# liuyuan-pal/NeRO

Hardware: NVIDIA B200
Metric: train rays/sec (128 samples/ray) (higher is better)
Workload: dtype f32 (split-bf16 x3 tensor-core MMAs, fp32 accumulate)

## Files before the change

### include/nero_b200.h

```cpp
#ifndef NERO_B200_H_
#define NERO_B200_H_
#include <stdint.h>

#ifdef __cplusplus
extern "C" {
#endif

#define NERO_ACT_NONE 0
#define NERO_ACT_SOFTPLUS100 1
#define NERO_ACT_RELU 2
#define NERO_ACT_SIGMOID 3
#define NERO_ACT_EXPCLAMP 4
#define NERO_EPI_BIAS_ACT 0
#define NERO_EPI_MUL_DACT 1
#define NERO_EPI_TANGENT 2

int nero_version(void);

int nero_prep_weight(const float* v, const float* g, int K, int row0, int nrows, const int* kmap, float in_scale,
                     void* img_f, int rows_pad_f, void* img_t, int rows_pad_t, int t_c0, int t_ncols, float* w_eff, int ld_weff,
                     void* stream);

int nero_linear(const float* A, int lda, int k_valid, const void* wimg, int n_pad, int k_chunks, const float* bias, int n_bias,
                float* out, int ldo, int ncol_out, float oscale, int mode, int act, float act_param,
                const float* H, int ldh, float hscale, int dact, const float* V, int ldv, float* out2, int ldo2,
                const float* addend, int ldadd, int ncol_main, float* tail, int ldt,
                const int* m_ptr, int m_cap, void* stream);

typedef struct nero_chain_layer {
  const void* wimg; const float* bias;
  float* save; const float* H; const float* addend; const float* V; float* out2; float* tail;
  int n_pad, k_chunks, n_bias, ncol_out, ncol_main, kind, act;
  int ld_save, ldh, ldadd, ldv, ldo2, ldt;
  float oscale, hscale, act_param;
  int write_a, a_blocks;
  const float* csrc; int ld_csrc;
  int pad_;
} nero_chain_layer;
typedef struct nero_chain_params {
  const float* A0; int lda0; int k_valid0;
  int n_layers; const int* m_ptr; int m_cap;
  nero_chain_layer L[10];
} nero_chain_params;
int nero_chain(const void* chain_params_host, void* stream);
int nero_row_axpy(const float* a, int lda, const float* X, int ldx, float* Y, int ldy, int ncol, const int* m_ptr, int m_cap, void* stream);

int nero_wgrad(const float* dY, int ldy, int n_valid, const float* X, int ldx, int k_valid,
               const float* dY2, int ldy2, const float* X2, int ldx2,
               float* partial, int ld_partial, int rows_partial, float* bias_partial,
               int n_rows_pad, int k_pad, int P, const int* m_ptr, int m_cap, void* stream);
int nero_wgrad_finish(const float* partial, int P, int rows_partial, int ld_partial, const float* bias_partial, int K,
                      int row0, int nrows, const int* kmap, float in_scale, const float* v, const float* g,
                      float* grad_w, float* grad_g, float* grad_b, const float* extra_row, float extra_scale, void* stream);
int nero_colsum(const float* X, int ldx, int ncol, const float* w, int ldw, const int* m_ptr, int m_cap, float* out,
                void* stream);

int nero_pe(const float* x, int d, int ldx, int M, int L, float scale, float* out, int ldo, void* stream);
int nero_ide(const float* dirs, int ldd, const float* kappa_inv, int kstride, float kappa_scalar, int M, float* out, int ldo, void* stream);

int nero_set_ide_table(const float* mat17x36_host);

int nero_ray_prepare(const float* rays_o, const float* rays_d, const float* z_vals, int R, int S, int* cnt_in, int* cnt_out,
                     int* off_in, int* off_out, int* n_in, int* n_out, void* stream);
int nero_ray_fill(const float* rays_o, const float* rays_d, const float* z_vals, int R, int S, const int* off_in, const int* off_out,
                  int* slot, float* pts, int* ray_in, float* X0, int ld_x0, float* Y8, int ld_y8, float* H4, int ld_h4,
                  float* XN, int ld_xn, float* H5, int ld_h5, float* FV, int ld_fv, float* dist_out, int* ray_out, void* stream);

int nero_reg_prepare(const float* rays_o, const float* rays_d, const float* z_vals, int R, int S, float radius, int* cnt, int* cnt_dummy,
                     int* off, int* off_dummy, int* n, int* n_dummy, void* stream);
int nero_reg_fill(const float* rays_o, const float* rays_d, const float* z_vals, int R, int S, float radius, const int* off, float* pts,
                  float* X0, int ldx, float* H4, int ldh, void* stream);

int nero_points_fill(const float* pts3, int N, float* pts, int* ray_in, float* X0, int ldx, float* Y8, int ldy, float* H4, int ldh, void* stream);

int nero_dact_times_row(const float* H, int ldh, const float* row, float* V, int ldv, int ncol, const int* m_ptr, int m_cap, void* stream);
int nero_pe_grad(const float* X0, int ldx, const float* U0, int ldu, const float* US, int lds, float* G, const int* m_ptr, int m_cap, void* stream);
int nero_pe_tangent(const float* X0, int ldx, const float* DG, float* UB0, int ld0, float* UB4, int ld4, const int* m_ptr, int m_cap, void* stream);

int nero_sdf_alpha_fwd(const float* Y8, int ldy, int sdf_col, const float* G, const float* pts, const int* ray_in, const float* rays_d,
                       const float* variance, const float* car, float* alpha, float* gerr, const int* m_ptr, int m_cap, void* stream);
int nero_sdf_alpha_bwd(const float* Y8, int ldy, int sdf_col, const float* G, const float* pts, const int* ray_in, const float* rays_d,
                       const float* variance, const float* car, const float* dalpha, const float* dgerr, float* dY8, int lddy, float* DG,
                       float* d_inv_s, const int* m_ptr, int m_cap, void* stream);

int nero_nerf_post_fwd(const float* dens, int ldd, const float* rgb, int ldr, const float* dist, float* alpha, float* color,
                       const int* m_ptr, int m_cap, void* stream);
int nero_nerf_post_bwd(const float* dens, int ldd, const float* rgb, int ldr, const float* dist, const float* dalpha, const float* dcolor,
                       float* ddens, int lddd, float* drgb, int lddr, const int* m_ptr, int m_cap, void* stream);

int nero_composite_fwd(const int* slot, int R, int S, const float* a_in, const float* c_in, const float* a_out, const float* c_out,
                       float* rgb, float* weights, void* stream);
int nero_composite_bwd(const int* slot, int R, int S, const float* a_in, const float* c_in, const float* a_out, const float* c_out,
                       const float* drgb, float* da_in, float* dc_in, float* da_out, float* dc_out, void* stream);

int nero_shade_prep_fwd(const float* G, const float* pts, const int* ray_in, const float* rays_d, const float* OUTS, float* E, int lde,
                        float* GEO, const float* human_poses, float* EH, int ldeh, int pos_freq, const int* m_ptr, int m_cap, int sphere, void* stream);
int nero_shade_prep_bwd(const float* G, const float* pts, const int* ray_in, const float* rays_d, const float* OUTS, const float* GEO,
                        const float* dE_dir, int ld_dir, const float* dE_inn, int ld_inn, const float* dE_dif, int ld_dif,
                        const float* dEH, int ld_eh, const float* human_poses, const float* dNoV, float* DOUTS, float* DG,
                        const int* m_ptr, int m_cap, int sphere, void* stream);
int nero_shade_combine_fwd(const float* OUTS, const float* GEO, const float* lut, float exp_max, int human, float* color,
                           float* occ_prob, float* refl, const int* m_ptr, int m_cap, void* stream);
int nero_shade_combine_bwd(const float* OUTS, const float* GEO, const float* lut, float exp_max, int human, const float* dcolor,
                           const float* docc, float* DOUTS, float* dNoV, const int* m_ptr, int m_cap, void* stream);

int nero_sample_init(const float* rays_o, const float* rays_d, const float* near, const float* far, int R, int n, int nb,
                     const float* lin_inner, const float* bg_base, const float* bg_lower, const float* bg_upper,
                     const float* rand_inner, const float* rand_bg, float* z, int ldz, float* z_bg, int ldzb,
                     float* X0, int ldx, float* HC, int ldh, void* stream);
int nero_upsample(const float* rays_o, const float* rays_d, int R, const float* z, int ldz, const float* sdf, int lds, int n, int n_new,
                  const float* variance, float inv_s_cap, int clip, int surface_variant, float* new_z, int ldn,
                  float* X0, int ldx, float* HC, int ldh, float* wsum, void* stream);
int nero_merge_samples(const float* z, int ldz, const float* sdf, int lds, int n, const float* nz, int ldn, const float* nsdf, int ldns,
                       int m, float* oz, int ldoz, float* osdf, int ldos, int R, void* stream);
int nero_occ_init(const float* pts, const float* refl, const int* sel, const int* p_ptr, int p_cap, int sn0, const float* lin,
                  float* o_out, float* d_out, float* z, int ldz, float* X0, int ldx, float* HC, int ldh, void* stream);
int nero_occ_select(const float* pts, const float* Y8, int ldy, int sdf_col, const float* G, const int* ray_in, const float* rays_d,
                    float sdf_thresh, const int* m_ptr, int m_cap, int* sel, int* count, void* stream);
int nero_occ_loss(const float* occ_prob, const float* gt, const int* sel, const int* p_ptr, int p_cap, float* loss_sum, float* docc_sign,
                  void* stream);

int nero_bvh_build_host(const float* verts, int V, const int* tris, int T, void* nodes_out, float* tri_out, int* tri_id_out, int* n_nodes);
int nero_bvh_trace(const void* nodes, const float* tris, int n_rays, const float* org, int ldo, const float* dir, int ldd,
                   float* pos_depth, float* nrm_hit, float miss_depth, int flip, void* stream);

typedef struct nero_mc_params {
  const float* pts; const float* normals; const float* view; const float* rough;
  const float* poses;
  const float* rand_d; const float* rand_s;
  const float* tab_d; const float* tab_s;
  int P, Sd, Ss;
  int ggx_smith, sphere_dir, human;
  float* org; float* dir;
  const float* pos_depth; const float* nrm_hit;
  int* slot;
  int* blk_cnt; int* blk_off; int* counts;
  float* EO; int ldeo; float* EH; int ldeh; float* hhit; float* EI; int ldei;
  const float* OUT_O; const float* OUT_H; const float* OUT_I;
  float exp_max_o, exp_max_i;
  float* LD; float* LS; float* LSF;
  const float* dLD; const float* dLS; const float* dLSF;
  float* DPRE_O; float* DPRE_H; float* DPRE_I;
  float* dA;
  const float* dEO; const float* dEH; const float* dEI;
  float* dA2;
} nero_mc_params;
int nero_mc_sample(const nero_mc_params* q, void* stream);
int nero_mc_classify(const nero_mc_params* q, void* stream);
int nero_mc_fill(const nero_mc_params* q, void* stream);
int nero_mc_combine_fwd(const nero_mc_params* q, void* stream);
int nero_mc_combine_bwd(const nero_mc_params* q, void* stream);
int nero_mc_dir_bwd(const nero_mc_params* q, void* stream);
int nero_mat_prep(const float* pts, int M, float* X, int ldx, float* CAT, int ldc, float* Y, int ldy, void* stream);

int nero_abi_sizeof(int which);

int nero_prep_weight_batch(const void* jobs_dev, int n_jobs, int max_rows, void* stream);

int nero_wgrad_finish_batch(const void* jobs_dev, int n_jobs, int max_rows, int max_k, void* stream);

int nero_adam_flat(float* p, const float* g, float* m, float* v, long long n, float lr_over_bc1, float b1, float b2, float eps,
                   float inv_sqrt_bc2, float weight_decay, void* stream);

#ifdef __cplusplus
}
#endif
#endif
```

### nero_b200/csrc/api.cu

```cuda
#include "common.cuh"
#include "../../include/nero_b200.h"

namespace nero {
struct LinearParams {
  const float* A; int lda; int k_valid;
  const uint8_t* wimg; int n_pad; int k_chunks;
  const float* bias; int n_bias;
  float* out; int ldo; int ncol_out; float oscale;
  int mode; int act; float act_param;
  const float* H; int ldh; float hscale; int dact;
  const float* V; int ldv;
  float* out2; int ldo2;
  const float* addend; int ldadd;
  int ncol_main; float* tail; int ldt;
  const int* m_ptr; int m_cap;
};
struct WgradParams {
  const float* dY; int ldy; const float* X; int ldx;
  const float* dY2; int ldy2; const float* X2; int ldx2;
  int n0; int n_valid; int k0; int k_valid;
  float* partial; int ld_partial; int rows_partial;
  float* bias_partial;
  const int* m_ptr; int m_cap;
};
int linear_dispatch(const LinearParams& p, cudaStream_t stream);
int wgrad_dispatch(WgradParams p, int n_rows_pad, int k_pad, int P, cudaStream_t stream);
int prep_weight(const float* v, const float* g, int K, int row0, int nrows, const int* kmap, float in_scale,
                uint8_t* img_f, int rows_pad_f, uint8_t* img_t, int rows_pad_t, int t_c0, int t_ncols, float* w_eff, int ld_weff,
                cudaStream_t stream);
int wgrad_finish(const float* partial, int P, int rows_partial, int ld_partial, const float* bias_partial, int K,
                 int row0, int nrows, const int* kmap, float in_scale, const float* v, const float* g, float* grad_w,
                 float* grad_g, float* grad_b, const float* extra_row, float extra_scale, cudaStream_t stream);
int colsum(const float* X, int ldx, int ncol, const float* w, int ldw, const int* m_ptr, int m_cap, float* out, cudaStream_t stream);
int wgrad_finish_batch(const void* jobs_dev, int n_jobs, int max_rows, int max_k, cudaStream_t stream);
int prep_weight_batch(const void* jobs_dev, int n_jobs, int max_rows, cudaStream_t stream);
int adam_flat(float* p, const float* g, float* m, float* v, long n, float lr_over_bc1, float b1, float b2, float eps, float inv_sqrt_bc2,
              float wd, cudaStream_t st);
}


namespace nero {
struct IdeTable;
int set_ide_table(const float* mat17x36_host);
int ray_prepare(const float* rays_o, const float* rays_d, const float* z_vals, int R, int S, int* cnt_in, int* cnt_out,
                int* off_in, int* off_out, int* n_in, int* n_out, cudaStream_t st);
struct FillParams {
  const float* rays_o; const float* rays_d; const float* z_vals; int R; int S;
  const int* off_in; const int* off_out;
  int* slot; float* pts; int* ray_in;
  float* X0; int ld_x0; float* Y8; int ld_y8; float* H4; int ld_h4;
  float* XN; int ld_xn; float* H5; int ld_h5; float* FV; int ld_fv;
  float* dist_out; int* ray_out;
};
int ray_fill(const FillParams& q, cudaStream_t st);
int dact_times_row(const float* H, int ldh, const float* row, float* V, int ldv, int ncol, const int* m_ptr, int m_cap, cudaStream_t st);
int pe_grad(const float* X0, int ldx, const float* U0, int ldu, const float* US, int lds, float* G, const int* m_ptr, int m_cap, cudaStream_t st);
int pe_tangent_launch(const float* X0, int ldx, const float* DG, float* UB0, int ld0, float* UB4, int ld4, const int* m_ptr, int m_cap, cudaStream_t st);
int sdf_alpha_forward(const float* Y8, int ldy, int sdf_col, const float* G, const float* pts, const int* ray_in, const float* rays_d,
                      const float* variance, const float* car, float* alpha, float* gerr, const int* m_ptr, int m_cap, cudaStream_t st);
int sdf_alpha_backward(const float* Y8, int ldy, int sdf_col, const float* G, const float* pts, const int* ray_in, const float* rays_d,
                       const float* variance, const float* car, const float* dalpha, const float* dgerr, float* dY8, int lddy, float* DG,
                       float* d_inv_s, const int* m_ptr, int m_cap, cudaStream_t st);
int nerf_post_forward(const float* dens, int ldd, const float* rgb, int ldr, const float* dist, float* alpha, float* color, const int* m_ptr, int m_cap, cudaStream_t st);
int nerf_post_backward(const float* dens, int ldd, const float* rgb, int ldr, const float* dist, const float* dalpha, const float* dcolor,
                       float* ddens, int lddd, float* drgb, int lddr, const int* m_ptr, int m_cap, cudaStream_t st);
int composite_forward(const int* slot, int R, int S, const float* a_in, const float* c_in, const float* a_out, const float* c_out,
                      float* rgb, float* weights, cudaStream_t st);
int composite_backward(const int* slot, int R, int S, const float* a_in, const float* c_in, const float* a_out, const float* c_out,
                       const float* drgb, float* da_in, float* dc_in, float* da_out, float* dc_out, cudaStream_t st);
struct ShadePrepParams {
  const float* G; const float* pts; const int* ray_in; const float* rays_d;
  const float* OUTS; float* E; int lde; float* GEO;
  const float* human_poses; float* EH; int ldeh;
  int pos_freq;
  const int* m_ptr; int m_cap;
  int sphere;
};
struct ShadePrepBwdParams {
  const float* G; const float* pts; const int* ray_in; const float* rays_d; const float* OUTS; const float* GEO;
  const float* dE_dir; int ld_dir; const float* dE_inn; int ld_inn; const float* dE_dif; int ld_dif;
  const float* dEH; int ld_eh; const float* human_poses; const float* dNoV;
  float* DOUTS; float* DG;
  const int* m_ptr; int m_cap;
  int sphere;
};
struct ShadeCombineParams {
  const float* OUTS; const float* GEO; const float* lut; float exp_max; int human;
  float* color; float* occ_prob; float* refl;
  const float* dcolor; const float* docc; float* DOUTS; float* dNoV;
  const int* m_ptr; int m_cap;
};
int shade_prep_forward(const ShadePrepParams& q, cudaStream_t st);
int shade_prep_backward(const ShadePrepBwdParams& q, cudaStream_t st);
int shade_combine_forward(const ShadeCombineParams& q, cudaStream_t st);
int shade_combine_backward(const ShadeCombineParams& q, cudaStream_t st);
struct SampleInitParams {
  const float* rays_o; const float* rays_d; const float* near; const float* far; int R;
  int n; int nb;
  const float* lin_inner; const float* bg_base; const float* bg_lower; const float* bg_upper;
  const float* rand_inner; const float* rand_bg;
  float* z; int ldz; float* z_bg; int ldzb;
  float* X0; int ldx; float* HC; int ldh;
};
struct UpsampleParams {
  const float* rays_o; const float* rays_d; int R;
  const float* z; int ldz; const float* sdf; int lds; int n;
  int n_new;
  const float* variance; float inv_s_cap; int clip;
  int surface_variant;
  float* new_z; int ldn;
  float* X0; int ldx; float* HC; int ldh;
  float* wsum;
  const float* origins;
};
int sample_init(const SampleInitParams& q, cudaStream_t st);
int upsample(const UpsampleParams& q, cudaStream_t st);
int merge_samples(const float* z, int ldz, const float* sdf, int lds, int n, const float* nz, int ldn, const float* nsdf, int ldns,
                  int m, float* oz, int ldoz, float* osdf, int ldos, int R, cudaStream_t st);
int occ_init(const float* pts, const float* refl, const int* sel, const int* p_ptr, int p_cap, int sn0, const float* lin,
             float* o_out, float* d_out, float* z, int ldz, float* X0, int ldx, float* HC, int ldh, cudaStream_t st);
int occ_select(const float* pts, const float* Y8, int ldy, int sdf_col, const float* G, const int* ray_in, const float* rays_d,
               float sdf_thresh, const int* m_ptr, int m_cap, int* sel, int* count, cudaStream_t st);
int row_axpy(const float* a, int lda, const float* X, int ldx, float* Y, int ldy, int ncol, const int* m_ptr, int m_cap, cudaStream_t st);
int reg_prepare(const float* rays_o, const float* rays_d, const float* z_vals, int R, int S, float radius, int* cnt, int* cnt_dummy,
                int* off, int* off_dummy, int* n, int* n_dummy, cudaStream_t st);
int reg_fill(const float* rays_o, const float* rays_d, const float* z_vals, int R, int S, float radius, const int* off, float* pts,
             float* X0, int ldx, float* H4, int ldh, cudaStream_t st);
int points_fill(const float* pts3, int N, float* pts, int* ray_in, float* X0, int ldx, float* Y8, int ldy, float* H4, int ldh, cudaStream_t st);
struct ChainParams;
int set_ide_table_mc(const float* mat17x36_host);
int bvh_build_host(const float* verts, int V, const int* tris, int T, void* nodes_out, float* tri_out, int* tri_id_out, int* n_nodes);
struct BvhNode;
struct TraceParams {
  const BvhNode* nodes; const float4* tris; int n_rays;
  const float* org; int ldo; const float* dir; int ldd;
  float4* pos_depth; float4* nrm_hit;
  float miss_depth; int flip;
};
int bvh_trace(const TraceParams& q, cudaStream_t st);
int mc_sample(const ::nero_mc_params& q, cudaStream_t st);
int mc_classify(const ::nero_mc_params& q, cudaStream_t st);
int mc_fill(const ::nero_mc_params& q, cudaStream_t st);
int mc_combine_fwd(const ::nero_mc_params& q, cudaStream_t st);
int mc_combine_bwd(const ::nero_mc_params& q, cudaStream_t st);
int mc_dir_bwd(const ::nero_mc_params& q, cudaStream_t st);
int mat_prep(const float* pts, int M, float* X, int ldx, float* CAT, int ldc, float* Y, int ldy, cudaStream_t st);
int chain_dispatch(const ChainParams& p, cudaStream_t stream);
int pe_standalone(const float* x, int d, int ldx, int M, int L, float scale, float* out, int ldo, cudaStream_t st);
int ide_standalone(const float* dirs, int ldd, const float* kappa, int kstride, float kappa_scalar, int M, float* out, int ldo, cudaStream_t st);
int occ_loss(const float* occ_prob, const float* gt, const int* sel, const int* p_ptr, int p_cap, float* loss_sum, float* docc_sign,
             cudaStream_t st);
}

using namespace nero;

extern "C" {

int nero_version(void) { return 100; }

int nero_prep_weight(const float* v, const float* g, int K, int row0, int nrows, const int* kmap, float in_scale,
                     void* img_f, int rows_pad_f, void* img_t, int rows_pad_t, int t_c0, int t_ncols, float* w_eff, int ld_weff,
                     void* stream) {
  return prep_weight(v, g, K, row0, nrows, kmap, in_scale, (uint8_t*)img_f, rows_pad_f, (uint8_t*)img_t, rows_pad_t, t_c0, t_ncols,
                     w_eff, ld_weff, (cudaStream_t)stream);
}

int nero_linear(const float* A, int lda, int k_valid, const void* wimg, int n_pad, int k_chunks, const float* bias, int n_bias,
                float* out, int ldo, int ncol_out, float oscale, int mode, int act, float act_param,
                const float* H, int ldh, float hscale, int dact, const float* V, int ldv, float* out2, int ldo2,
                const float* addend, int ldadd, int ncol_main, float* tail, int ldt,
                const int* m_ptr, int m_cap, void* stream) {
  LinearParams p{A, lda, k_valid, (const uint8_t*)wimg, n_pad, k_chunks, bias, n_bias, out, ldo, ncol_out, oscale, mode, act, act_param,
                 H, ldh, hscale, dact, V, ldv, out2, ldo2, addend, ldadd, ncol_main, tail, ldt, m_ptr, m_cap};
  if (!A || !wimg || !out || ncol_out > n_pad) return NERO_ERR_ARG;
  return linear_dispatch(p, (cudaStream_t)stream);
}

int nero_wgrad(const float* dY, int ldy, int n_valid, const float* X, int ldx, int k_valid,
               const float* dY2, int ldy2, const float* X2, int ldx2,
               float* partial, int ld_partial, int rows_partial, float* bias_partial,
               int n_rows_pad, int k_pad, int P, const int* m_ptr, int m_cap, void* stream) {
  WgradParams p{dY, ldy, X, ldx, dY2, ldy2, X2, ldx2, 0, n_valid, 0, k_valid, partial, ld_partial, rows_partial, bias_partial,
                m_ptr, m_cap};
  if (!dY || !X || !partial || (dY2 && !X2)) return NERO_ERR_ARG;
  return wgrad_dispatch(p, n_rows_pad, k_pad, P, (cudaStream_t)stream);
}

int nero_wgrad_finish(const float* partial, int P, int rows_partial, int ld_partial, const float* bias_partial, int K,
                      int row0, int nrows, const int* kmap, float in_scale, const float* v, const float* g,
                      float* grad_w, float* grad_g, float* grad_b, const float* extra_row, float extra_scale, void* stream) {
  return wgrad_finish(partial, P, rows_partial, ld_partial, bias_partial, K, row0, nrows, kmap, in_scale, v, g, grad_w, grad_g,
                      grad_b, extra_row, extra_scale, (cudaStream_t)stream);
}

int nero_colsum(const float* X, int ldx, int ncol, const float* w, int ldw, const int* m_ptr, int m_cap, float* out,
                void* stream) {
  return colsum(X, ldx, ncol, w, ldw, m_ptr, m_cap, out, (cudaStream_t)stream);
}

int nero_set_ide_table(const float* mat17x36_host) {
  const int rc = set_ide_table(mat17x36_host);
  return rc != NERO_OK ? rc : set_ide_table_mc(mat17x36_host);
}
int nero_bvh_build_host(const float* verts, int V, const int* tris, int T, void* nodes_out, float* tri_out, int* tri_id_out, int* n_nodes) {
  if (!verts || !tris || !nodes_out || !tri_out || !tri_id_out || !n_nodes) return NERO_ERR_ARG;
  return bvh_build_host(verts, V, tris, T, nodes_out, tri_out, tri_id_out, n_nodes);
}
int nero_bvh_trace(const void* nodes, const float* tris, int n_rays, const float* org, int ldo, const float* dir, int ldd,
                   float* pos_depth, float* nrm_hit, float miss_depth, int flip, void* stream) {
  if (!nodes || !tris || (n_rays > 0 && (!org || !dir || !pos_depth || !nrm_hit))) return NERO_ERR_ARG;
  TraceParams q{reinterpret_cast<const BvhNode*>(nodes), reinterpret_cast<const float4*>(tris), n_rays, org, ldo, dir, ldd,
                reinterpret_cast<float4*>(pos_depth), reinterpret_cast<float4*>(nrm_hit), miss_depth, flip};
  return bvh_trace(q, (cudaStream_t)stream);
}
int nero_mc_sample(const nero_mc_params* q, void* stream) { return q ? mc_sample(*q, (cudaStream_t)stream) : NERO_ERR_ARG; }
int nero_mc_classify(const nero_mc_params* q, void* stream) { return q ? mc_classify(*q, (cudaStream_t)stream) : NERO_ERR_ARG; }
int nero_mc_fill(const nero_mc_params* q, void* stream) { return q ? mc_fill(*q, (cudaStream_t)stream) : NERO_ERR_ARG; }
int nero_mc_combine_fwd(const nero_mc_params* q, void* stream) { return q ? mc_combine_fwd(*q, (cudaStream_t)stream) : NERO_ERR_ARG; }
int nero_mc_combine_bwd(const nero_mc_params* q, void* stream) { return q ? mc_combine_bwd(*q, (cudaStream_t)stream) : NERO_ERR_ARG; }
int nero_mc_dir_bwd(const nero_mc_params* q, void* stream) { return q ? mc_dir_bwd(*q, (cudaStream_t)stream) : NERO_ERR_ARG; }
int nero_abi_sizeof(int which) {
  switch (which) {
    case 0: return int(sizeof(nero_chain_layer));
    case 1: return int(sizeof(nero_chain_params));
    case 2: return int(sizeof(nero_mc_params));
    case 3: return 104;
    case 4: return 88;
    default: return -1;
  }
}
int nero_prep_weight_batch(const void* jobs_dev, int n_jobs, int max_rows, void* stream) {
  return prep_weight_batch(jobs_dev, n_jobs, max_rows, (cudaStream_t)stream);
}
int nero_wgrad_finish_batch(const void* jobs_dev, int n_jobs, int max_rows, int max_k, void* stream) {
  return wgrad_finish_batch(jobs_dev, n_jobs, max_rows, max_k, (cudaStream_t)stream);
}
int nero_adam_flat(float* p, const float* g, float* m, float* v, long long n, float lr_over_bc1, float b1, float b2, float eps,
                   float inv_sqrt_bc2, float weight_decay, void* stream) {
  if (!p || !g || !m || !v) return NERO_ERR_ARG;
  return adam_flat(p, g, m, v, long(n), lr_over_bc1, b1, b2, eps, inv_sqrt_bc2, weight_decay, (cudaStream_t)stream);
}
int nero_mat_prep(const float* pts, int M, float* X, int ldx, float* CAT, int ldc, float* Y, int ldy, void* stream) {
  return mat_prep(pts, M, X, ldx, CAT, ldc, Y, ldy, (cudaStream_t)stream);
}

int nero_pe(const float* x, int d, int ldx, int M, int L, float scale, float* out, int ldo, void* stream) {
  return pe_standalone(x, d, ldx, M, L, scale, out, ldo, (cudaStream_t)stream);
}
int nero_ide(const float* dirs, int ldd, const float* kappa_inv, int kstride, float kappa_scalar, int M, float* out, int ldo, void* stream) {
  return ide_standalone(dirs, ldd, kappa_inv, kstride, kappa_scalar, M, out, ldo, (cudaStream_t)stream);
}

int nero_chain(const void* chain_params_host, void* stream) {
  if (!chain_params_host) return NERO_ERR_ARG;
  return chain_dispatch(*reinterpret_cast<const ChainParams*>(chain_params_host), (cudaStream_t)stream);
}
int nero_reg_prepare(const float* rays_o, const float* rays_d, const float* z_vals, int R, int S, float radius, int* cnt, int* cnt_dummy,
                     int* off, int* off_dummy, int* n, int* n_dummy, void* stream) {
  return reg_prepare(rays_o, rays_d, z_vals, R, S, radius, cnt, cnt_dummy, off, off_dummy, n, n_dummy, (cudaStream_t)stream);
}
int nero_reg_fill(const float* rays_o, const float* rays_d, const float* z_vals, int R, int S, float radius, const int* off, float* pts,
                  float* X0, int ldx, float* H4, int ldh, void* stream) {
  return reg_fill(rays_o, rays_d, z_vals, R, S, radius, off, pts, X0, ldx, H4, ldh, (cudaStream_t)stream);
}
int nero_points_fill(const float* pts3, int N, float* pts, int* ray_in, float* X0, int ldx, float* Y8, int ldy, float* H4, int ldh, void* stream) {
  return points_fill(pts3, N, pts, ray_in, X0, ldx, Y8, ldy, H4, ldh, (cudaStream_t)stream);
}
int nero_row_axpy(const float* a, int lda, const float* X, int ldx, float* Y, int ldy, int ncol, const int* m_ptr, int m_cap, void* stream) {
  return row_axpy(a, lda, X, ldx, Y, ldy, ncol, m_ptr, m_cap, (cudaStream_t)stream);
}

int nero_ray_prepare(const float* rays_o, const float* rays_d, const float* z_vals, int R, int S, int* cnt_in, int* cnt_out,
                     int* off_in, int* off_out, int* n_in, int* n_out, void* stream) {
  return ray_prepare(rays_o, rays_d, z_vals, R, S, cnt_in, cnt_out, off_in, off_out, n_in, n_out, (cudaStream_t)stream);
}
int nero_ray_fill(const float* rays_o, const float* rays_d, const float* z_vals, int R, int S, const int* off_in, const int* off_out,
                  int* slot, float* pts, int* ray_in, float* X0, int ld_x0, float* Y8, int ld_y8, float* H4, int ld_h4,
                  float* XN, int ld_xn, float* H5, int ld_h5, float* FV, int ld_fv, float* dist_out, int* ray_out, void* stream) {
  FillParams q{rays_o, rays_d, z_vals, R, S, off_in, off_out, slot, pts, ray_in, X0, ld_x0, Y8, ld_y8, H4, ld_h4, XN, ld_xn, H5, ld_h5,
               FV, ld_fv, dist_out, ray_out};
  return ray_fill(q, (cudaStream_t)stream);
}
int nero_dact_times_row(const float* H, int ldh, const float* row, float* V, int ldv, int ncol, const int* m_ptr, int m_cap, void* stream) {
  return dact_times_row(H, ldh, row, V, ldv, ncol, m_ptr, m_cap, (cudaStream_t)stream);
}
int nero_pe_grad(const float* X0, int ldx, const float* U0, int ldu, const float* US, int lds, float* G, const int* m_ptr, int m_cap, void* stream) {
  return pe_grad(X0, ldx, U0, ldu, US, lds, G, m_ptr, m_cap, (cudaStream_t)stream);
}
int nero_pe_tangent(const float* X0, int ldx, const float* DG, float* UB0, int ld0, float* UB4, int ld4, const int* m_ptr, int m_cap, void* stream) {
  return pe_tangent_launch(X0, ldx, DG, UB0, ld0, UB4, ld4, m_ptr, m_cap, (cudaStream_t)stream);
}
int nero_sdf_alpha_fwd(const float* Y8, int ldy, int sdf_col, const float* G, const float* pts, const int* ray_in, const float* rays_d,
                       const float* variance, const float* car, float* alpha, float* gerr, const int* m_ptr, int m_cap, void* stream) {
  return sdf_alpha_forward(Y8, ldy, sdf_col, G, pts, ray_in, rays_d, variance, car, alpha, gerr, m_ptr, m_cap, (cudaStream_t)stream);
}
int nero_sdf_alpha_bwd(const float* Y8, int ldy, int sdf_col, const float* G, const float* pts, const int* ray_in, const float* rays_d,
                       const float* variance, const float* car, const float* dalpha, const float* dgerr, float* dY8, int lddy, float* DG,
                       float* d_inv_s, const int* m_ptr, int m_cap, void* stream) {
  return sdf_alpha_backward(Y8, ldy, sdf_col, G, pts, ray_in, rays_d, variance, car, dalpha, dgerr, dY8, lddy, DG, d_inv_s, m_ptr, m_cap,
                            (cudaStream_t)stream);
}
int nero_nerf_post_fwd(const float* dens, int ldd, const float* rgb, int ldr, const float* dist, float* alpha, float* color,
                       const int* m_ptr, int m_cap, void* stream) {
  return nerf_post_forward(dens, ldd, rgb, ldr, dist, alpha, color, m_ptr, m_cap, (cudaStream_t)stream);
}
int nero_nerf_post_bwd(const float* dens, int ldd, const float* rgb, int ldr, const float* dist, const float* dalpha, const float* dcolor,
                       float* ddens, int lddd, float* drgb, int lddr, const int* m_ptr, int m_cap, void* stream) {
  return nerf_post_backward(dens, ldd, rgb, ldr, dist, dalpha, dcolor, ddens, lddd, drgb, lddr, m_ptr, m_cap, (cudaStream_t)stream);
}
int nero_composite_fwd(const int* slot, int R, int S, const float* a_in, const float* c_in, const float* a_out, const float* c_out,
                       float* rgb, float* weights, void* stream) {
  return composite_forward(slot, R, S, a_in, c_in, a_out, c_out, rgb, weights, (cudaStream_t)stream);
}
int nero_composite_bwd(const int* slot, int R, int S, const float* a_in, const float* c_in, const float* a_out, const float* c_out,
                       const float* drgb, float* da_in, float* dc_in, float* da_out, float* dc_out, void* stream) {
  return composite_backward(slot, R, S, a_in, c_in, a_out, c_out, drgb, da_in, dc_in, da_out, dc_out, (cudaStream_t)stream);
}
int nero_shade_prep_fwd(const float* G, const float* pts, const int* ray_in, const float* rays_d, const float* OUTS, float* E, int lde,
                        float* GEO, const float* human_poses, float* EH, int ldeh, int pos_freq, const int* m_ptr, int m_cap, int sphere, void* stream) {
  ShadePrepParams q{G, pts, ray_in, rays_d, OUTS, E, lde, GEO, human_poses, EH, ldeh, pos_freq, m_ptr, m_cap, sphere};
  return shade_prep_forward(q, (cudaStream_t)stream);
}
int nero_shade_prep_bwd(const float* G, const float* pts, const int* ray_in, const float* rays_d, const float* OUTS, const float* GEO,
                        const float* dE_dir, int ld_dir, const float* dE_inn, int ld_inn, const float* dE_dif, int ld_dif,
                        const float* dEH, int ld_eh, const float* human_poses, const float* dNoV, float* DOUTS, float* DG,
                        const int* m_ptr, int m_cap, int sphere, void* stream) {
  ShadePrepBwdParams q{G, pts, ray_in, rays_d, OUTS, GEO, dE_dir, ld_dir, dE_inn, ld_inn, dE_dif, ld_dif, dEH, ld_eh, human_poses, dNoV,
                       DOUTS, DG, m_ptr, m_cap, sphere};
  return shade_prep_backward(q, (cudaStream_t)stream);
}
int nero_shade_combine_fwd(const float* OUTS, const float* GEO, const float* lut, float exp_max, int human, float* color,
                           float* occ_prob, float* refl, const int* m_ptr, int m_cap, void* stream) {
  ShadeCombineParams q{OUTS, GEO, lut, exp_max, human, color, occ_prob, refl, nullptr, nullptr, nullptr, nullptr, m_ptr, m_cap};
  return shade_combine_forward(q, (cudaStream_t)stream);
}
int nero_shade_combine_bwd(const float* OUTS, const float* GEO, const float* lut, float exp_max, int human, const float* dcolor,
                           const float* docc, float* DOUTS, float* dNoV, const int* m_ptr, int m_cap, void* stream) {
  ShadeCombineParams q{OUTS, GEO, lut, exp_max, human, nullptr, nullptr, nullptr, dcolor, docc, DOUTS, dNoV, m_ptr, m_cap};
  return shade_combine_backward(q, (cudaStream_t)stream);
}
int nero_sample_init(const float* rays_o, const float* rays_d, const float* near, const float* far, int R, int n, int nb,
                     const float* lin_inner, const float* bg_base, const float* bg_lower, const float* bg_upper,
                     const float* rand_inner, const float* rand_bg, float* z, int ldz, float* z_bg, int ldzb,
                     float* X0, int ldx, float* HC, int ldh, void* stream) {
  SampleInitParams q{rays_o, rays_d, near, far, R, n, nb, lin_inner, bg_base, bg_lower, bg_upper, rand_inner, rand_bg, z, ldz, z_bg, ldzb,
                     X0, ldx, HC, ldh};
  return sample_init(q, (cudaStream_t)stream);
}
int nero_upsample(const float* rays_o, const float* rays_d, int R, const float* z, int ldz, const float* sdf, int lds, int n, int n_new,
                  const float* variance, float inv_s_cap, int clip, int surface_variant, float* new_z, int ldn,
                  float* X0, int ldx, float* HC, int ldh, float* wsum, void* stream) {
  UpsampleParams q{rays_o, rays_d, R, z, ldz, sdf, lds, n, n_new, variance, inv_s_cap, clip, surface_variant, new_z, ldn, X0, ldx, HC, ldh,
                   wsum, nullptr};
  return upsample(q, (cudaStream_t)stream);
}
int nero_merge_samples(const float* z, int ldz, const float* sdf, int lds, int n, const float* nz, int ldn, const float* nsdf, int ldns,
                       int m, float* oz, int ldoz, float* osdf, int ldos, int R, void* stream) {
  return merge_samples(z, ldz, sdf, lds, n, nz, ldn, nsdf, ldns, m, oz, ldoz, osdf, ldos, R, (cudaStream_t)stream);
}
int nero_occ_init(const float* pts, const float* refl, const int* sel, const int* p_ptr, int p_cap, int sn0, const float* lin,
                  float* o_out, float* d_out, float* z, int ldz, float* X0, int ldx, float* HC, int ldh, void* stream) {
  return occ_init(pts, refl, sel, p_ptr, p_cap, sn0, lin, o_out, d_out, z, ldz, X0, ldx, HC, ldh, (cudaStream_t)stream);
}
int nero_occ_select(const float* pts, const float* Y8, int ldy, int sdf_col, const float* G, const int* ray_in, const float* rays_d,
                    float sdf_thresh, const int* m_ptr, int m_cap, int* sel, int* count, void* stream) {
  return occ_select(pts, Y8, ldy, sdf_col, G, ray_in, rays_d, sdf_thresh, m_ptr, m_cap, sel, count, (cudaStream_t)stream);
}
int nero_occ_loss(const float* occ_prob, const float* gt, const int* sel, const int* p_ptr, int p_cap, float* loss_sum, float* docc_sign,
                  void* stream) {
  return occ_loss(occ_prob, gt, sel, p_ptr, p_cap, loss_sum, docc_sign, (cudaStream_t)stream);
}

}
```

### nero_b200/csrc/k_umma_wgrad.cu

```cuda

#include "common.cuh"
#include "ptx.cuh"
#include "umma_common.cuh"

namespace nero {

struct WgradParams {
  const float* dY; int ldy; const float* X; int ldx;
  const float* dY2; int ldy2; const float* X2; int ldx2;
  int n0; int n_valid;
  int k0; int k_valid;
  float* partial; int ld_partial; int rows_partial;
  float* bias_partial;
  const int* m_ptr; int m_cap;
};

constexpr int WG_BM = 128, WG_BK = 64;
constexpr int kWgProdWarps = 16;
constexpr int kWgThreads = (kWgProdWarps + 1) * 32;
constexpr uint32_t kWgABytes = WG_BM * 128;

template <int NW> struct WgCfg {
  static constexpr uint32_t b_plane = NW * 128;
  static constexpr uint32_t stage_bytes = 2 * kWgABytes + 2 * b_plane;
  static constexpr int stages = (stage_bytes * 3 <= 200 * 1024) ? 3 : 2;
  static constexpr uint32_t smem_bytes = stages * stage_bytes + 1024 + 256 + 512;
};

__device__ __forceinline__ void wg_split2(float x0, float x1, uint32_t& hi, uint32_t& lo) {
  __nv_bfloat162 h = __floats2bfloat162_rn(x0, x1);
  const uint32_t hb = *reinterpret_cast<uint32_t*>(&h);
  const float h0 = __uint_as_float(hb << 16), h1 = __uint_as_float(hb & 0xffff0000u);
  __nv_bfloat162 l = __floats2bfloat162_rn(x0 - h0, x1 - h1);
  hi = hb;
  lo = *reinterpret_cast<uint32_t*>(&l);
}

template <int NOCT>
__device__ __forceinline__ void load_octets(const float* __restrict__ src, int ld, int col, bool col_ok, int s0, int M, uint32_t oct0,
                                            float (&x)[NOCT][8]) {
#pragma unroll
  for (int o = 0; o < NOCT; ++o)
#pragma unroll
    for (int i = 0; i < 8; ++i) {
      const int s = s0 + (oct0 + o) * 8 + i;
      x[o][i] = (col_ok && s < M) ? __ldg(src + size_t(s) * ld + col) : 0.0f;
    }
}
template <int NOCT>
__device__ __forceinline__ float store_octets(const float (&x)[NOCT][8], uint8_t* plane_hi, uint8_t* plane_lo, uint32_t row, uint32_t oct0) {
  float sum = 0.0f;
#pragma unroll
  for (int o = 0; o < NOCT; ++o) {
    uint32_t hw[4], lw[4];
#pragma unroll
    for (int i = 0; i < 4; ++i) {
      wg_split2(x[o][2 * i], x[o][2 * i + 1], hw[i], lw[i]);
      sum += x[o][2 * i] + x[o][2 * i + 1];
    }
    const uint32_t off = row * 128u + (((oct0 + o) ^ (row & 7u)) << 4);
    *reinterpret_cast<uint4*>(plane_hi + off) = make_uint4(hw[0], hw[1], hw[2], hw[3]);
    *reinterpret_cast<uint4*>(plane_lo + off) = make_uint4(lw[0], lw[1], lw[2], lw[3]);
  }
  return sum;
}

__device__ __forceinline__ void red_add_v4(float* addr, float a, float b, float c, float d) {
  asm volatile("red.global.add.v4.f32 [%0], {%1, %2, %3, %4};" ::"l"(addr), "f"(a), "f"(b), "f"(c), "f"(d) : "memory");
}

template <int NW>
__device__ __forceinline__ void wg_epilogue(const WgradParams& p, uint32_t tmem_base, int pw, int lane, int n0, bool any, const float* s_bias) {
  const int orow = n0 + pw * 32 + lane;
  float* prow = p.partial + size_t(orow) * p.ld_partial + p.k0;
  const uint32_t taddr = tmem_base + (uint32_t(pw * 32) << 16);
  if (any) {
#pragma unroll 1
    for (int cc = 0; cc < (NW + 31) / 32; ++cc) {
      float v[32];
      tmem_ld32(taddr + cc * 32, v);
      tmem_ld_wait();
      if (orow < p.rows_partial) {
#pragma unroll
        for (int j = 0; j < 32; j += 4)
          if (cc * 32 + j < NW) red_add_v4(prow + cc * 32 + j, v[j], v[j + 1], v[j + 2], v[j + 3]);
      }
    }
    if (p.bias_partial && p.k0 == 0 && orow < p.rows_partial) atomicAdd(&p.bias_partial[orow], s_bias[pw * 32 + lane]);
  }
}

template <int NW>
__global__ void __launch_bounds__(kWgThreads, 1) umma_wgrad_kernel(const WgradParams p) {
  using Cfg = WgCfg<NW>;
  constexpr int STAGES = Cfg::stages;
  extern __shared__ uint8_t smem_raw[];
  uint8_t* smem = reinterpret_cast<uint8_t*>((reinterpret_cast<uintptr_t>(smem_raw) + 1023) & ~uintptr_t(1023));
  uint64_t* bars = reinterpret_cast<uint64_t*>(smem + STAGES * Cfg::stage_bytes);
  uint64_t* full = bars;
  uint64_t* empty = bars + STAGES;
  uint64_t* tfull = bars + 2 * STAGES;
  uint32_t* tmem_slot = reinterpret_cast<uint32_t*>(bars + 2 * STAGES + 1);
  float* s_bias = reinterpret_cast<float*>(smem + STAGES * Cfg::stage_bytes + 256);

  const int warp = threadIdx.x >> 5, lane = threadIdx.x & 31;
  int M = p.m_ptr ? *p.m_ptr : p.m_cap;
  if (M > p.m_cap) M = p.m_cap;
  const int P = gridDim.x;
  const int n0 = p.n0 + int(blockIdx.y) * WG_BM;
  const int total_chunks = (M + WG_BK - 1) / WG_BK;
  const int cpp = (total_chunks + P - 1) / P;
  const int c_begin = min(total_chunks, int(blockIdx.x) * cpp), c_end = min(total_chunks, c_begin + cpp);
  const int npairs = p.dY2 ? 2 : 1;
  const int nc1 = c_end - c_begin;
  const int nchunks = nc1 * npairs;

  if (threadIdx.x == 0) {
    for (int s = 0; s < STAGES; ++s) { mbar_init(&full[s], kWgProdWarps); mbar_init(&empty[s], 1); }
    mbar_init(tfull, 1);
    fence_mbar_init();
  }
  if (threadIdx.x < 128) s_bias[threadIdx.x] = 0.0f;
  if (warp == kWgProdWarps) tmem_alloc<256>(tmem_slot);
  tcgen05_fence_before();
  __syncthreads();
  tcgen05_fence_after();
  const uint32_t tmem_base = *tmem_slot;

  if (warp < kWgProdWarps) {
    const bool is_a = warp < 8;
    const int pw = warp & 3;
    const int oh = (warp >> 2) & 1;
    float bias_acc = 0.0f;
    for (int g = 0; g < nchunks; ++g) {
      const int s = g % STAGES;
      const int pair = g / nc1;
      const int chunk = c_begin + g % nc1;
      const int s0 = chunk * WG_BK;
      uint8_t* st = smem + s * Cfg::stage_bytes;
      if (is_a) {
        const float* src = pair ? p.dY2 : p.dY;
        const int ld = pair ? p.ldy2 : p.ldy;
        const uint32_t row = pw * 32 + lane;
        const int col = n0 + int(row);
        const bool ok = col < p.n_valid;
        float x[4][8];
        load_octets<4>(src, ld, col, ok, s0, M, oh * 4, x);
        mbar_wait(&empty[s], ((g / STAGES) & 1) ^ 1);
        const float sacc = store_octets<4>(x, st, st + kWgABytes, row, oh * 4);
        if (pair == 0) bias_acc += sacc;
      } else {
        const float* src = pair ? p.X2 : p.X;
        const int ld = pair ? p.ldx2 : p.ldx;
        uint8_t* bh = st + 2 * kWgABytes;
        constexpr int NJ = (NW + 127) / 128;
        float x[NJ][4][8];
#pragma unroll
        for (int j = 0; j < NJ; ++j) {
          const uint32_t row = j * 128 + pw * 32 + lane;
          const int col = p.k0 + int(row);
          load_octets<4>(src, ld, col, row < NW && col < p.k_valid, s0, M, oh * 4, x[j]);
        }
        mbar_wait(&empty[s], ((g / STAGES) & 1) ^ 1);
#pragma unroll
        for (int j = 0; j < NJ; ++j) {
          const uint32_t row = j * 128 + pw * 32 + lane;
          if (row < NW) store_octets<4>(x[j], bh, bh + Cfg::b_plane, row, oh * 4);
        }
      }
      fence_proxy_async_smem();
      __syncwarp();
      if (lane == 0) mbar_arrive(&full[s]);
    }
    if (is_a) atomicAdd(&s_bias[pw * 32 + lane], bias_acc);
    asm volatile("bar.sync 1, %0;" ::"n"(kWgProdWarps * 32));
    if (warp < 4) {
      mbar_wait(tfull, 0);
      tcgen05_fence_after();
      wg_epilogue<NW>(p, tmem_base, pw, lane, n0, nchunks > 0, s_bias);
    }
  } else {
    constexpr uint32_t idesc = make_idesc_bf16(WG_BM, NW);
    for (int g = 0; g < nchunks; ++g) {
      const int s = g % STAGES;
      mbar_wait(&full[s], (g / STAGES) & 1);
      tcgen05_fence_after();
      if (elect_one()) {
        const uint32_t a_hi = smem_u32(smem + s * Cfg::stage_bytes);
        const uint32_t a_lo = a_hi + kWgABytes;
        const uint32_t b_hi = a_hi + 2 * kWgABytes;
        const uint32_t b_lo = b_hi + Cfg::b_plane;
#pragma unroll
        for (int k = 0; k < WG_BK / 16; ++k) {
          const uint64_t dah = make_desc_k_sw128(a_hi + k * 32), dal = make_desc_k_sw128(a_lo + k * 32);
          const uint64_t dbh = make_desc_k_sw128(b_hi + k * 32), dbl = make_desc_k_sw128(b_lo + k * 32);
          umma_bf16(tmem_base, dal, dbh, idesc, (g | k) != 0);
          umma_bf16(tmem_base, dah, dbl, idesc, 1);
          umma_bf16(tmem_base, dah, dbh, idesc, 1);
        }
        umma_commit(&empty[s]);
        if (g == nchunks - 1) umma_commit(tfull);
      }
      __syncwarp();
    }
    if (nchunks == 0 && elect_one()) mbar_arrive(tfull);
    __syncwarp();
  }
  tcgen05_fence_before();
  __syncthreads();
  if (warp == kWgProdWarps) tmem_dealloc<256>(tmem_base);
}


constexpr int MN_BK = 32, kMnGroupWarps = kWgProdWarps / 2;
constexpr uint32_t kMnSbo = 1024, kMnLbo = (MN_BK / 8) * 1024;
template <int NW> struct WgMnCfg {
  static constexpr uint32_t a_plane = WG_BM * MN_BK * 2, b_plane = NW * MN_BK * 2;
  static constexpr uint32_t stage_bytes = 2 * a_plane + 2 * b_plane;
  static constexpr int stages = 4;
  static constexpr uint32_t smem_bytes = stages * stage_bytes + 1024 + 256 + 512;
};

__device__ __forceinline__ uint32_t mn_chunk_offset(uint32_t chunk, uint32_t s) {
  const uint32_t r = s & 7u;
  return (chunk >> 3) * kMnLbo + (s >> 3) * kMnSbo + r * 128u + (((chunk & 7u) ^ r) << 4);
}

template <int NW>
__device__ __forceinline__ void wg_epilogue_rows(const WgradParams& p, uint32_t tmem_base, float* tile, int warp, int lane, int n0,
                                                 const float* s_bias) {
  constexpr int LD = NW + 4;
  constexpr int SLICE = NW / 4;
  const int quarter = warp & 3, slice = warp >> 2;
  {
    const int row = quarter * 32 + lane;
    const uint32_t taddr = tmem_base + (uint32_t(quarter * 32) << 16) + uint32_t(slice * SLICE);
    float* dst = tile + row * LD + slice * SLICE;
#pragma unroll
    for (int c = 0; c < SLICE; c += 16) {
      float v[16];
      tmem_ld16(taddr + c, v);
      tmem_ld_wait();
#pragma unroll
      for (int j = 0; j < 16; j += 4) *reinterpret_cast<float4*>(dst + c + j) = make_float4(v[j], v[j + 1], v[j + 2], v[j + 3]);
    }
  }
  asm volatile("bar.sync 1, %0;" ::"n"(kWgProdWarps * 32));
  const int r_first = (int(blockIdx.x) * 5) & 127;
  for (int i = warp; i < WG_BM; i += kWgProdWarps) {
    const int r = (i + r_first) & 127;
    const int orow = n0 + r;
    if (orow >= p.rows_partial) continue;
    float* prow = p.partial + size_t(orow) * p.ld_partial + p.k0;
#pragma unroll
    for (int c = lane * 4; c < NW; c += 128) {
      const float4 v = *reinterpret_cast<const float4*>(tile + r * LD + c);
      red_add_v4(prow + c, v.x, v.y, v.z, v.w);
    }
    if (lane == 0 && p.bias_partial && p.k0 == 0) atomicAdd(&p.bias_partial[orow], s_bias[r]);
  }
}

template <int NW>
__global__ void __launch_bounds__(kWgThreads, 1) umma_wgrad_mn_kernel(const WgradParams p) {
  using Cfg = WgMnCfg<NW>;
  constexpr int STAGES = Cfg::stages;
  constexpr int CB = NW / 8;
  constexpr int SPW = 32 / CB;
  constexpr int ATASKS = MN_BK / 2;
  constexpr int TASKS = ATASKS + MN_BK / SPW;
  constexpr int TPW = TASKS / kMnGroupWarps;
  static_assert(TASKS % kMnGroupWarps == 0 && TPW >= 2 && STAGES % 2 == 0, "task split");
  extern __shared__ uint8_t smem_raw[];
  uint8_t* smem = reinterpret_cast<uint8_t*>((reinterpret_cast<uintptr_t>(smem_raw) + 1023) & ~uintptr_t(1023));
  uint64_t* bars = reinterpret_cast<uint64_t*>(smem + STAGES * Cfg::stage_bytes);
  uint64_t* full = bars;
  uint64_t* empty = bars + STAGES;
  uint64_t* tfull = bars + 2 * STAGES;
  uint32_t* tmem_slot = reinterpret_cast<uint32_t*>(bars + 2 * STAGES + 1);
  float* s_bias = reinterpret_cast<float*>(smem + STAGES * Cfg::stage_bytes + 256);

  const int warp = threadIdx.x >> 5, lane = threadIdx.x & 31;
  int M = p.m_ptr ? *p.m_ptr : p.m_cap;
  if (M > p.m_cap) M = p.m_cap;
  const int P = gridDim.x;
  const int n0 = p.n0 + int(blockIdx.y) * WG_BM;
  const int total_chunks = (M + MN_BK - 1) / MN_BK;
  const int cpp = (total_chunks + P - 1) / P;
  const int c_begin = min(total_chunks, int(blockIdx.x) * cpp), c_end = min(total_chunks, c_begin + cpp);
  const int npairs = p.dY2 ? 2 : 1;
  const int nc1 = c_end - c_begin;
  const int nchunks = nc1 * npairs;

  if (threadIdx.x == 0) {
    for (int s = 0; s < STAGES; ++s) { mbar_init(&full[s], kMnGroupWarps); mbar_init(&empty[s], 1); }
    mbar_init(tfull, 1);
    fence_mbar_init();
  }
  if (threadIdx.x < 128) s_bias[threadIdx.x] = 0.0f;
  if (warp == kWgProdWarps) tmem_alloc<256>(tmem_slot);
  tcgen05_fence_before();
  __syncthreads();
  tcgen05_fence_after();
  const uint32_t tmem_base = *tmem_slot;

  if (warp < kWgProdWarps) {
    float bsum[8] = {0.f, 0.f, 0.f, 0.f, 0.f, 0.f, 0.f, 0.f};
    const uint32_t a_chunk = lane & 15, a_sub = lane >> 4;
    const uint32_t b_chunk = lane % CB, b_sub = lane / CB;
    const int a_col = n0 + int(a_chunk) * 8, b_col = p.k0 + int(b_chunk) * 8;
    const int group = warp / kMnGroupWarps, wi = warp % kMnGroupWarps;
    for (int g = group; g < nchunks; g += 2) {
      const int s = g % STAGES;
      const int pair = g / nc1;
      const int chunk = c_begin + g % nc1;
      const int s0 = chunk * MN_BK;
      uint8_t* st = smem + s * Cfg::stage_bytes;
      const float* srcA = pair ? p.dY2 : p.dY;
      const int ldA = pair ? p.ldy2 : p.ldy;
      const float* srcB = pair ? p.X2 : p.X;
      const int ldB = pair ? p.ldx2 : p.ldx;
      float4 v[TPW][2];
#pragma unroll
      for (int i = 0; i < TPW; ++i) {
        const int t = wi + kMnGroupWarps * i;
        const bool isA = t < ATASKS;
        const int sl = isA ? 2 * t + int(a_sub) : (t - ATASKS) * SPW + int(b_sub);
        const int srow = s0 + sl;
        const int col = isA ? a_col : b_col;
        const int lim = isA ? p.n_valid : p.k_valid;
        const float* rp = (isA ? srcA : srcB) + size_t(srow) * (isA ? ldA : ldB) + col;
        const bool rok = srow < M;
        v[i][0] = (rok && col < lim) ? __ldg(reinterpret_cast<const float4*>(rp)) : make_float4(0.f, 0.f, 0.f, 0.f);
        v[i][1] = (rok && col + 4 < lim) ? __ldg(reinterpret_cast<const float4*>(rp + 4)) : make_float4(0.f, 0.f, 0.f, 0.f);
      }
      mbar_wait(&empty[s], ((g / STAGES) & 1) ^ 1);
#pragma unroll
      for (int i = 0; i < TPW; ++i) {
        const int t = wi + kMnGroupWarps * i;
        const bool isA = t < ATASKS;
        const int sl = isA ? 2 * t + int(a_sub) : (t - ATASKS) * SPW + int(b_sub);
        const int col = isA ? a_col : b_col;
        const int lim = isA ? p.n_valid : p.k_valid;
        float x[8] = {v[i][0].x, v[i][0].y, v[i][0].z, v[i][0].w, v[i][1].x, v[i][1].y, v[i][1].z, v[i][1].w};
#pragma unroll
        for (int j = 0; j < 8; ++j) if (col + j >= lim) x[j] = 0.f;
        uint32_t hw[4], lw[4];
#pragma unroll
        for (int j = 0; j < 4; ++j) wg_split2(x[2 * j], x[2 * j + 1], hw[j], lw[j]);
        uint8_t* hi = isA ? st : st + 2 * Cfg::a_plane;
        uint8_t* lo = isA ? st + Cfg::a_plane : st + 2 * Cfg::a_plane + Cfg::b_plane;
        const uint32_t off = mn_chunk_offset(isA ? a_chunk : b_chunk, uint32_t(sl));
        *reinterpret_cast<uint4*>(hi + off) = make_uint4(hw[0], hw[1], hw[2], hw[3]);
        *reinterpret_cast<uint4*>(lo + off) = make_uint4(lw[0], lw[1], lw[2], lw[3]);
        if (isA && pair == 0) {
#pragma unroll
          for (int j = 0; j < 8; ++j) bsum[j] += x[j];
        }
      }
      fence_proxy_async_smem();
      __syncwarp();
      if (lane == 0) mbar_arrive(&full[s]);
    }
#pragma unroll
    for (int j = 0; j < 8; ++j) {
      bsum[j] += __shfl_xor_sync(0xffffffffu, bsum[j], 16);
      if (lane < 16) atomicAdd(&s_bias[a_chunk * 8 + j], bsum[j]);
    }
    asm volatile("bar.sync 1, %0;" ::"n"(kWgProdWarps * 32));
    mbar_wait(tfull, 0);
    tcgen05_fence_after();
    if (nchunks > 0) wg_epilogue_rows<NW>(p, tmem_base, reinterpret_cast<float*>(smem), warp, lane, n0, s_bias);
  } else {
    constexpr uint32_t idesc = make_idesc_bf16_mn(WG_BM, NW);
    for (int g = 0; g < nchunks; ++g) {
      const int s = g % STAGES;
      mbar_wait(&full[s], (g / STAGES) & 1);
      tcgen05_fence_after();
      if (elect_one()) {
        const uint32_t a_hi = smem_u32(smem + s * Cfg::stage_bytes);
        const uint32_t a_lo = a_hi + Cfg::a_plane;
        const uint32_t b_hi = a_hi + 2 * Cfg::a_plane;
        const uint32_t b_lo = b_hi + Cfg::b_plane;
#pragma unroll
        for (int k = 0; k < MN_BK / 16; ++k) {
          const uint32_t ko = k * 2 * kMnSbo;
          const uint64_t dah = make_desc_mn_sw128(a_hi + ko, kMnLbo, kMnSbo), dal = make_desc_mn_sw128(a_lo + ko, kMnLbo, kMnSbo);
          const uint64_t dbh = make_desc_mn_sw128(b_hi + ko, kMnLbo, kMnSbo), dbl = make_desc_mn_sw128(b_lo + ko, kMnLbo, kMnSbo);
          umma_bf16(tmem_base, dal, dbh, idesc, (g | k) != 0);
          umma_bf16(tmem_base, dah, dbl, idesc, 1);
          umma_bf16(tmem_base, dah, dbh, idesc, 1);
        }
        umma_commit(&empty[s]);
        if (g == nchunks - 1) umma_commit(tfull);
      }
      __syncwarp();
    }
    if (nchunks == 0 && elect_one()) mbar_arrive(tfull);
    __syncwarp();
  }
  tcgen05_fence_before();
  __syncthreads();
  if (warp == kWgProdWarps) tmem_dealloc<256>(tmem_base);
}

template <int NW>
static int launch_wgrad_mn(const WgradParams& p, int P, int n_tiles, cudaStream_t stream) {
  using Cfg = WgMnCfg<NW>;
  static bool attr_set = false;
  if (!attr_set) {
    if (cudaFuncSetAttribute(umma_wgrad_mn_kernel<NW>, cudaFuncAttributeMaxDynamicSharedMemorySize, Cfg::smem_bytes) != cudaSuccess)
      return NERO_ERR_CUDA;
    attr_set = true;
  }
  umma_wgrad_mn_kernel<NW><<<dim3(P, n_tiles), kWgThreads, Cfg::smem_bytes, stream>>>(p);
  NERO_LAUNCH_CHECK();
  return NERO_OK;
}

template <int NW>
static int launch_wgrad(const WgradParams& p, int P, int n_tiles, cudaStream_t stream) {
  using Cfg = WgCfg<NW>;
  static bool attr_set = false;
  if (!attr_set) {
    if (cudaFuncSetAttribute(umma_wgrad_kernel<NW>, cudaFuncAttributeMaxDynamicSharedMemorySize, Cfg::smem_bytes) != cudaSuccess)
      return NERO_ERR_CUDA;
    attr_set = true;
  }
  umma_wgrad_kernel<NW><<<dim3(P, n_tiles), kWgThreads, Cfg::smem_bytes, stream>>>(p);
  NERO_LAUNCH_CHECK();
  return NERO_OK;
}

int wgrad_dispatch(WgradParams p, int n_rows_pad, int k_pad, int P, cudaStream_t stream) {
  if ((p.ld_partial & 3) || k_pad % 64 || n_rows_pad % 16 || P <= 0) return NERO_ERR_ARG;
  const int n_tiles = (n_rows_pad + 127) / 128;
  p.n0 = 0;
  auto al = [](const float* q, int ld) { return q == nullptr || ((reinterpret_cast<uintptr_t>(q) & 15) == 0 && (ld & 3) == 0); };
  const bool mn = al(p.dY, p.ldy) && al(p.X, p.ldx) && al(p.dY2, p.ldy2) && al(p.X2, p.ldx2);
  int k0 = 0;
  while (k0 < k_pad) {
    const int rem = k_pad - k0;
    p.k0 = k0;
    int rc;
    if (rem >= 256) { rc = mn ? launch_wgrad_mn<256>(p, P, n_tiles, stream) : launch_wgrad<256>(p, P, n_tiles, stream); k0 += 256; }
    else if (rem >= 128) { rc = mn ? launch_wgrad_mn<128>(p, P, n_tiles, stream) : launch_wgrad<128>(p, P, n_tiles, stream); k0 += 128; }
    else { rc = mn ? launch_wgrad_mn<64>(p, P, n_tiles, stream) : launch_wgrad<64>(p, P, n_tiles, stream); k0 += 64; }
    if (rc != NERO_OK) return rc;
  }
  return NERO_OK;
}

}
```

### nero_b200/engine.py

```python
import math

import numpy as np
import torch

from . import ops
from .ops import Mat, K, linear, wgrad, chain, chain_layer as CL, ACT_NONE, ACT_SOFTPLUS100, ACT_RELU, ACT_SIGMOID, ACT_EXPCLAMP, EPI_MUL_DACT, EPI_TANGENT
from .ops import EK_BIAS_SOFTPLUS, EK_BIAS_RELU, EK_BIAS_GENERIC, EK_DACT_SOFTPLUS, EK_DACT_RELU, EK_DACT_NONE, EK_TANGENT

USE_CHAIN = True

INV_SQRT2 = 0.7071067811865476
SQRT2 = 1.4142135623730951
E_PE6R, E_PE8X, E_IDER, E_IDEN, E_LD = 0, 40, 92, 164, 240
O_MET, O_ROUGH, O_ALB, O_LD, O_LDIR, O_LI, O_IW, O_HUM, O_LDIM = 0, 4, 8, 12, 16, 20, 24, 28, 32
Y8_LD, Y8_X, Y8_SDF = 320, 256, 260


def ide_coefficient_table():
    def gbc(a, k):
        return np.prod(a - np.arange(k)) / math.factorial(k)

    def alc(l, m, k):
        return ((-1) ** m * 2 ** l * math.factorial(l) / math.factorial(k) / math.factorial(l - k - m) *
                gbc(0.5 * (l + k + m - 1.0), l))

    def shc(l, m, k):
        return np.sqrt((2.0 * l + 1.0) * math.factorial(l - m) / (4.0 * np.pi * math.factorial(l + m))) * alc(l, m, k)

    cols = [(m, 2 ** e) for e in range(5) for m in range(2 ** e + 1)]
    mat = np.zeros((17, len(cols)))
    for i, (m, l) in enumerate(cols):
        for k in range(l - m + 1):
            mat[k, i] = shc(l, m, k)
    return np.ascontiguousarray(mat.astype(np.float32))


_ide_uploaded = False


def upload_ide_table():
    global _ide_uploaded
    if not _ide_uploaded:
        mat = ide_coefficient_table()
        rc = ops.lib.nero_set_ide_table(mat.ctypes.data_as(ops.ctypes.c_void_p))
        ops._check(rc, 'nero_set_ide_table')
        _ide_uploaded = True


def _linear_to_srgb_torch(x):
    eps = torch.finfo(torch.float32).eps
    return torch.where(x <= 0.0031308, 323 / 25 * x, (211 * torch.clamp(x, min=eps) ** (5 / 12) - 11) / 200)


def _fg_lookup_torch(lut, uv):
    H, W = lut.shape[0], lut.shape[1]
    fx, fy = uv[:, 0] * W - 0.5, uv[:, 1] * H - 0.5
    x0f, y0f = torch.floor(fx), torch.floor(fy)
    tx, ty = (fx - x0f)[:, None], (fy - y0f)[:, None]
    x0, x1 = x0f.long().clamp(0, W - 1), (x0f.long() + 1).clamp(0, W - 1)
    y0, y1 = y0f.long().clamp(0, H - 1), (y0f.long() + 1).clamp(0, H - 1)
    a = lut[y0, x0] * (1 - tx) + lut[y0, x1] * tx
    b = lut[y1, x0] * (1 - tx) + lut[y1, x1] * tx
    return a * (1 - ty) + b * ty


class Grads:

    def __init__(self, params):
        self.params = [p for p in params]
        self.total = sum(p.numel() for p in self.params)
        self.flat = None
        self.views = None

    def ensure(self, strict=False):
        if self.flat is None:
            self.flat = torch.zeros(self.total, dtype=torch.float32, device=self.params[0].device)
            off = 0
            self.views = []
            for p in self.params:
                n = p.numel()
                self.views.append(self.flat[off:off + n].view_as(p))
                off += n
        missing = [i for i, p in enumerate(self.params) if p.grad is None]
        if len(missing) == len(self.params):
            self.flat.zero_()
        else:
            for i in missing:
                self.views[i].zero_()
        for i in missing:
            self.params[i].grad = self.views[i]
        if strict:
            for p, v in zip(self.params, self.views):
                if p.grad.data_ptr() != v.data_ptr():
                    v.copy_(p.grad)
                    p.grad = v
        return self.flat


class Predictor:

    def __init__(self, pp, dev, n_out, act, act_param=0.0, kmap=None, k_layout=None, t_cols=None):
        ls = pp.layers()
        self.n_out, self.act, self.act_param = n_out, act, act_param
        self.layers = [ops.PreparedLayer(ls[0].weight_v, ls[0].weight_g, ls[0].bias, dev, kmap=kmap, k_layout=k_layout, t_cols=t_cols)]
        for l in ls[1:]:
            self.layers.append(ops.PreparedLayer(l.weight_v, l.weight_g, l.bias, dev, t_cols=(0, 256)))
        self.pl = ls

    def prep(self):
        for l in self.layers:
            l.prep()

    def forward(self, A, acts, out, m_ptr, m_cap):
        L = self.layers
        if USE_CHAIN:
            tail = [CL(L[1], EK_BIAS_RELU, 256, save=Mat(acts[1])), CL(L[2], EK_BIAS_RELU, 256, save=Mat(acts[2])),
                    CL(L[3], EK_BIAS_GENERIC, self.n_out, save=out, act=self.act, act_param=self.act_param)]
            if L[0].k_chunks <= 4:
                chain(A, L[0].k_valid, [CL(L[0], EK_BIAS_RELU, 256, save=Mat(acts[0]))] + tail, m_ptr, m_cap)
            else:
                linear(A, L[0], Mat(acts[0]), 256, act=ACT_RELU, m_ptr=m_ptr, m_cap=m_cap)
                chain(Mat(acts[0]), 256, tail, m_ptr, m_cap)
            return
        linear(A, L[0], Mat(acts[0]), 256, act=ACT_RELU, m_ptr=m_ptr, m_cap=m_cap)
        linear(Mat(acts[0]), L[1], Mat(acts[1]), 256, act=ACT_RELU, m_ptr=m_ptr, m_cap=m_cap)
        linear(Mat(acts[1]), L[2], Mat(acts[2]), 256, act=ACT_RELU, m_ptr=m_ptr, m_cap=m_cap)
        linear(Mat(acts[2]), L[3], out, self.n_out, act=self.act, act_param=self.act_param, m_ptr=m_ptr, m_cap=m_cap)

    def backward(self, ws, dpre, A, acts, dHa, dHb, m_ptr, m_cap, dX=None, dx_ncol=0, dx_addend=None, dHc=None):
        L, P = self.layers, self.pl
        g = lambda i: (P[i].weight_v.grad, P[i].weight_g.grad, P[i].bias.grad)
        kw = dict(m_ptr=m_ptr, m_cap=m_cap)
        if USE_CHAIN and dHc is not None:
            ls = [CL(L[3], EK_DACT_RELU, 256, transposed=True, H=Mat(acts[2]), save=Mat(dHa)),
                  CL(L[2], EK_DACT_RELU, 256, transposed=True, H=Mat(acts[1]), save=Mat(dHb)),
                  CL(L[1], EK_DACT_RELU, 256, transposed=True, H=Mat(acts[0]), save=Mat(dHc))]
            if dX is not None:
                ls.append(CL(L[0], EK_DACT_NONE, dx_ncol, transposed=True, addend=dx_addend, save=dX))
            chain(dpre, self.n_out, ls, m_ptr, m_cap)
            wgrad(ws, dpre, self.n_out, Mat(acts[2]), 256, L[3], *g(3), **kw)
            wgrad(ws, Mat(dHa), 256, Mat(acts[1]), 256, L[2], *g(2), **kw)
            wgrad(ws, Mat(dHb), 256, Mat(acts[0]), 256, L[1], *g(1), **kw)
            wgrad(ws, Mat(dHc), 256, A, L[0].k_valid, L[0], *g(0), **kw)
            return
        linear(dpre, L[3], Mat(dHa), 256, transposed=True, mode=EPI_MUL_DACT, H=Mat(acts[2]), dact=ACT_RELU, **kw)
        wgrad(ws, dpre, self.n_out, Mat(acts[2]), 256, L[3], *g(3), **kw)
        linear(Mat(dHa), L[2], Mat(dHb), 256, transposed=True, mode=EPI_MUL_DACT, H=Mat(acts[1]), dact=ACT_RELU, **kw)
        wgrad(ws, Mat(dHa), 256, Mat(acts[1]), 256, L[2], *g(2), **kw)
        linear(Mat(dHb), L[1], Mat(dHa), 256, transposed=True, mode=EPI_MUL_DACT, H=Mat(acts[0]), dact=ACT_RELU, **kw)
        wgrad(ws, Mat(dHb), 256, Mat(acts[0]), 256, L[1], *g(1), **kw)
        if dX is not None:
            linear(Mat(dHa), L[0], dX, dx_ncol, transposed=True, mode=EPI_MUL_DACT, addend=dx_addend, **kw)
        wgrad(ws, Mat(dHa), 256, A, L[0].k_valid, L[0], *g(0), **kw)


class SdfNet:

    def __init__(self, sp, dev):
        self.sp = sp
        ls = sp.layers()
        assert len(ls) == 9 and sp.multires == 6 and tuple(sp.skip_in) == (4,), 'kernels are laid out for the default SDF network'
        self.L = []
        for k, l in enumerate(ls[:8]):
            tc = (0, 39) if k == 0 else (0, 256)
            self.L.append(ops.PreparedLayer(l.weight_v, l.weight_g, l.bias, dev, t_cols=tc))
        l8 = ls[8]
        self.L8f = ops.PreparedLayer(l8.weight_v, l8.weight_g, l8.bias, dev, row0=1, nrows=256, t_cols=(0, 256))
        self.L8s = ops.PreparedLayer(l8.weight_v, l8.weight_g, l8.bias, dev, row0=0, nrows=1, t_cols=(0, 256))
        self.nout = [256, 256, 256, 217, 256, 256, 256, 256]
        self.tmp_row = torch.zeros(256, device=dev)
        self.tmp_b = torch.zeros(4, device=dev)

    def prep(self):
        for l in self.L + [self.L8f, self.L8s]:
            l.prep()

    def hidden_forward(self, X0, Hs, H4buf, m_ptr, m_cap, save=True, heads=None):
        kw = dict(act=ACT_SOFTPLUS100, m_ptr=m_ptr, m_cap=m_cap)
        if USE_CHAIN:
            sv = (lambda t: Mat(t)) if save else (lambda t: None)
            ls = [CL(self.L[0], EK_BIAS_SOFTPLUS, 256, save=sv(Hs[0])), CL(self.L[1], EK_BIAS_SOFTPLUS, 256, save=sv(Hs[1])),
                  CL(self.L[2], EK_BIAS_SOFTPLUS, 256, save=sv(Hs[2])),
                  CL(self.L[3], EK_BIAS_SOFTPLUS, 217, oscale=INV_SQRT2, save=sv(H4buf), csrc=Mat(H4buf)),
                  CL(self.L[4], EK_BIAS_SOFTPLUS, 256, save=sv(Hs[4])), CL(self.L[5], EK_BIAS_SOFTPLUS, 256, save=sv(Hs[5])),
                  CL(self.L[6], EK_BIAS_SOFTPLUS, 256, save=sv(Hs[6])), CL(self.L[7], EK_BIAS_SOFTPLUS, 256, save=sv(Hs[7]))]
            chain(Mat(X0), self.L[0].k_valid, ls + (heads or []), m_ptr, m_cap, tag='sdf_forward' if save else 'sdf_forward_nosave')
            return
        linear(Mat(X0), self.L[0], Mat(Hs[0]), 256, **kw)
        linear(Mat(Hs[0]), self.L[1], Mat(Hs[1]), 256, **kw)
        linear(Mat(Hs[1]), self.L[2], Mat(Hs[2]), 256, **kw)
        linear(Mat(Hs[2]), self.L[3], Mat(H4buf), 217, oscale=INV_SQRT2, **kw)
        linear(Mat(H4buf), self.L[4], Mat(Hs[4]), 256, **kw)
        linear(Mat(Hs[4]), self.L[5], Mat(Hs[5]), 256, **kw)
        linear(Mat(Hs[5]), self.L[6], Mat(Hs[6]), 256, **kw)
        linear(Mat(Hs[6]), self.L[7], Mat(Hs[7]), 256, **kw)

    def sdf_only(self, X0, SA, SB, SC, out, m_ptr, m_cap):
        Hs = [SA, SB, SA, SC, SA, SB, SA, SB]
        if USE_CHAIN:
            self.hidden_forward(X0, Hs, SC, m_ptr, m_cap, save=False,
                                heads=[CL(self.L8s, EK_BIAS_GENERIC, 1, save=Mat(out), write_a=False)])
            return
        self.hidden_forward(X0, Hs, SC, m_ptr, m_cap)
        linear(Mat(SB), self.L8s, Mat(out), 1, m_ptr=m_ptr, m_cap=m_cap)

    def forward_with_gradient(self, w, m_ptr, m_cap):
        H = w['H']
        Hs = [H[1], H[2], H[3], H[4], H[5], H[6], H[7], H[8]]
        kw = dict(m_ptr=m_ptr, m_cap=m_cap)
        V = w['V']
        if USE_CHAIN:
            self.hidden_forward(w['X0'], Hs, H[4], m_ptr, m_cap,
                                heads=[CL(self.L8f, EK_BIAS_GENERIC, 256, save=Mat(w['Y8']), write_a=False),
                                       CL(self.L8s, EK_BIAS_GENERIC, 1, save=Mat(w['Y8'], Y8_SDF), write_a=False)])
            K('nero_dact_times_row', H[8], 256, self.L8s.w_eff, V[7], 256, 256, m_ptr, m_cap)
            ls = []
            for k in range(7, 0, -1):
                if k == 4:
                    ls.append(CL(self.L[4], EK_DACT_SOFTPLUS, 256, transposed=True, oscale=INV_SQRT2, H=Mat(H[4]), hscale=SQRT2,
                                 ncol_main=217, tail=Mat(w['USKIP']), save=Mat(V[3])))
                else:
                    ls.append(CL(self.L[k], EK_DACT_SOFTPLUS, 256, transposed=True, H=Mat(H[k]), save=Mat(V[k - 1])))
            ls.append(CL(self.L[0], EK_DACT_NONE, 39, transposed=True, save=Mat(w['U0'])))
            chain(Mat(V[7]), 256, ls, m_ptr, m_cap, tag='sdf_reverse_sweep')
            K('nero_pe_grad', w['X0'], 64, w['U0'], 64, w['USKIP'], 64, w['G'], m_ptr, m_cap)
            return
        self.hidden_forward(w['X0'], Hs, H[4], m_ptr, m_cap)
        linear(Mat(H[8]), self.L8f, Mat(w['Y8']), 256, **kw)
        linear(Mat(H[8]), self.L8s, Mat(w['Y8'], Y8_SDF), 1, **kw)
        K('nero_dact_times_row', H[8], 256, self.L8s.w_eff, V[7], 256, 256, m_ptr, m_cap)
        for k in range(7, 0, -1):
            if k == 4:
                linear(Mat(V[4]), self.L[4], Mat(V[3]), 256, transposed=True, mode=EPI_MUL_DACT, oscale=INV_SQRT2, H=Mat(H[4]),
                       hscale=SQRT2, dact=ACT_SOFTPLUS100, ncol_main=217, tail=Mat(w['USKIP']), **kw)
            else:
                linear(Mat(V[k]), self.L[k], Mat(V[k - 1]), 256, transposed=True, mode=EPI_MUL_DACT, H=Mat(H[k]),
                       dact=ACT_SOFTPLUS100, **kw)
        linear(Mat(V[0]), self.L[0], Mat(w['U0']), 39, transposed=True, mode=EPI_MUL_DACT, **kw)
        K('nero_pe_grad', w['X0'], 64, w['U0'], 64, w['USKIP'], 64, w['G'], m_ptr, m_cap)

    def backward(self, ws, w, m_ptr, m_cap, grads_of):
        H, V, UB, AB = w['H'], w['V'], w['UB'], w['ABAR']
        kw = dict(m_ptr=m_ptr, m_cap=m_cap)
        dY8 = w['dY8']
        K('nero_pe_tangent', w['X0'], 64, w['DG'], UB[0], 64, UB[4], 256, m_ptr, m_cap)
        if USE_CHAIN:
            ls = []
            for k in range(8):
                if k == 3:
                    ls.append(CL(self.L[3], EK_TANGENT, 217, use_bias=False, oscale=INV_SQRT2, H=Mat(H[4]), hscale=SQRT2, V=Mat(V[3]),
                                 out2=Mat(AB[3]), save=Mat(UB[4]), csrc=Mat(UB[4])))
                else:
                    ls.append(CL(self.L[k], EK_TANGENT, 256, use_bias=False, H=Mat(H[k + 1]), V=Mat(V[k]), out2=Mat(AB[k]), save=Mat(UB[k + 1])))
            chain(Mat(UB[0]), self.L[0].k_valid, ls, m_ptr, m_cap, tag='sdf_tangent_sweep')
            K('nero_row_axpy', Mat(dY8, Y8_SDF), Y8_LD, V[7], 256, AB[7], 256, 256, m_ptr, m_cap)
            ls = [CL(self.L8f, EK_DACT_SOFTPLUS, 256, transposed=True, H=Mat(H[8]), addend=Mat(AB[7]), save=Mat(AB[7]))]
            for k in range(7, 0, -1):
                if k == 4:
                    ls.append(CL(self.L[4], EK_DACT_SOFTPLUS, 217, transposed=True, oscale=INV_SQRT2, H=Mat(H[4]), hscale=SQRT2,
                                 addend=Mat(AB[3]), save=Mat(AB[3])))
                else:
                    ls.append(CL(self.L[k], EK_DACT_SOFTPLUS, 256, transposed=True, H=Mat(H[k]), addend=Mat(AB[k - 1]), save=Mat(AB[k - 1])))
            chain(Mat(dY8), 256, ls, m_ptr, m_cap, tag='sdf_value_backward')
        else:
            for k in range(8):
                A = Mat(UB[k])
                if k == 3:
                    linear(A, self.L[3], Mat(UB[4]), 217, use_bias=False, mode=EPI_TANGENT, oscale=INV_SQRT2, H=Mat(H[4]), hscale=SQRT2,
                           dact=ACT_SOFTPLUS100, V=Mat(V[3]), out2=Mat(AB[3]), **kw)
                else:
                    linear(A, self.L[k], Mat(UB[k + 1]), 256, use_bias=False, mode=EPI_TANGENT, H=Mat(H[k + 1]), dact=ACT_SOFTPLUS100,
                           V=Mat(V[k]), out2=Mat(AB[k]), **kw)
            linear(Mat(dY8), self.L8f, Mat(AB[7]), 256, transposed=True, mode=EPI_MUL_DACT, H=Mat(H[8]), dact=ACT_SOFTPLUS100,
                   addend=Mat(AB[7]), **kw)
            linear(Mat(dY8, Y8_SDF), self.L8s, Mat(AB[7]), 256, transposed=True, mode=EPI_MUL_DACT, H=Mat(H[8]), dact=ACT_SOFTPLUS100,
                   addend=Mat(AB[7]), **kw)
            for k in range(7, 0, -1):
                if k == 4:
                    linear(Mat(AB[4]), self.L[4], Mat(AB[3]), 217, transposed=True, mode=EPI_MUL_DACT, oscale=INV_SQRT2, H=Mat(H[4]),
                           hscale=SQRT2, dact=ACT_SOFTPLUS100, addend=Mat(AB[3]), **kw)
                else:
                    linear(Mat(AB[k]), self.L[k], Mat(AB[k - 1]), 256, transposed=True, mode=EPI_MUL_DACT, H=Mat(H[k]),
                           dact=ACT_SOFTPLUS100, addend=Mat(AB[k - 1]), **kw)
        ls = self.sp.layers()
        for k in range(8):
            Hin = Mat(w['X0']) if k == 0 else Mat(H[k])
            wgrad(ws, Mat(AB[k]), self.nout[k], Hin, self.L[k].k_valid, self.L[k], ls[k].weight_v.grad, ls[k].weight_g.grad,
                  ls[k].bias.grad, dY2=Mat(V[k]), X2=Mat(UB[k]), **kw)
        l8 = ls[8]
        wgrad(ws, Mat(dY8), 256, Mat(H[8]), 256, self.L8f, l8.weight_v.grad, l8.weight_g.grad, l8.bias.grad, **kw)
        self.tmp_row.zero_()
        self.tmp_b.zero_()
        ops.colsum(Mat(H[8]), 256, self.tmp_row, w=Mat(dY8, Y8_SDF), m_ptr=m_ptr, m_cap=m_cap)
        ops.colsum(Mat(UB[8]), 256, self.tmp_row, m_ptr=m_ptr, m_cap=m_cap)
        ops.colsum(Mat(dY8, Y8_SDF), 1, self.tmp_b, m_ptr=m_ptr, m_cap=m_cap)
        K('nero_wgrad_finish', self.tmp_row, 1, 1, 256, self.tmp_b, 256, 0, 1, None, 1.0, l8.weight_v.detach(), l8.weight_g.detach(),
          l8.weight_v.grad, l8.weight_g.grad, l8.bias.grad, None, 0.0)

    def value_forward(self, X0, H, out, m_ptr, m_cap):
        Hs = [H[1], H[2], H[3], H[4], H[5], H[6], H[7], H[8]]
        if USE_CHAIN:
            self.hidden_forward(X0, Hs, H[4], m_ptr, m_cap, heads=[CL(self.L8s, EK_BIAS_GENERIC, 1, save=Mat(out), write_a=False)])
        else:
            self.hidden_forward(X0, Hs, H[4], m_ptr, m_cap)
            linear(Mat(H[8]), self.L8s, Mat(out), 1, m_ptr=m_ptr, m_cap=m_cap)

    def value_backward(self, ws, X0, H, dsdf, AB, scratch, m_ptr, m_cap):
        kw = dict(m_ptr=m_ptr, m_cap=m_cap)
        K('nero_dact_times_row', H[8], 256, self.L8s.w_eff, scratch, 256, 256, m_ptr, m_cap)
        AB[7].zero_()
        K('nero_row_axpy', dsdf, dsdf.stride(0), scratch, 256, AB[7], 256, 256, m_ptr, m_cap)
        ls = []
        for k in range(7, 0, -1):
            if k == 4:
                ls.append(CL(self.L[4], EK_DACT_SOFTPLUS, 217, transposed=True, oscale=INV_SQRT2, H=Mat(H[4]), hscale=SQRT2, save=Mat(AB[3])))
            else:
                ls.append(CL(self.L[k], EK_DACT_SOFTPLUS, 256, transposed=True, H=Mat(H[k]), save=Mat(AB[k - 1])))
        if USE_CHAIN:
            chain(Mat(AB[7]), 256, ls, m_ptr, m_cap)
        else:
            for k in range(7, 0, -1):
                if k == 4:
                    linear(Mat(AB[4]), self.L[4], Mat(AB[3]), 217, transposed=True, mode=EPI_MUL_DACT, oscale=INV_SQRT2, H=Mat(H[4]),
                           hscale=SQRT2, dact=ACT_SOFTPLUS100, **kw)
                else:
                    linear(Mat(AB[k]), self.L[k], Mat(AB[k - 1]), 256, transposed=True, mode=EPI_MUL_DACT, H=Mat(H[k]),
                           dact=ACT_SOFTPLUS100, **kw)
        ls_ = self.sp.layers()
        for k in range(8):
            Hin = Mat(X0) if k == 0 else Mat(H[k])
            wgrad(ws, Mat(AB[k]), self.nout[k], Hin, self.L[k].k_valid, self.L[k], ls_[k].weight_v.grad, ls_[k].weight_g.grad,
                  ls_[k].bias.grad, **kw)
        l8 = ls_[8]
        self.tmp_row.zero_()
        self.tmp_b.zero_()
        ops.colsum(Mat(H[8]), 256, self.tmp_row, w=Mat(dsdf), m_ptr=m_ptr, m_cap=m_cap)
        ops.colsum(Mat(dsdf), 1, self.tmp_b, m_ptr=m_ptr, m_cap=m_cap)
        K('nero_wgrad_finish', self.tmp_row, 1, 1, 256, self.tmp_b, 256, 0, 1, None, 1.0, l8.weight_v.detach(), l8.weight_g.detach(),
          l8.weight_v.grad, l8.weight_g.grad, l8.bias.grad, None, 0.0)


class NerfNet:

    def __init__(self, npar, dev):
        self.np = npar
        pl = npar.pts_linears
        mk = lambda l, **kw: ops.PreparedLayer(l.weight, None, l.bias, dev, **kw)
        self.P = [mk(pl[0])] + [mk(pl[i], t_cols=(0, 256)) for i in range(1, 5)] + [mk(pl[5], t_cols=(84, 256))] + \
                 [mk(pl[i], t_cols=(0, 256)) for i in (6, 7)]
        self.alpha = mk(npar.alpha_linear, t_cols=(0, 256))
        self.feature = mk(npar.feature_linear, t_cols=(0, 256))
        self.views = mk(npar.views_linears[0], t_cols=(0, 256))
        self.rgb = mk(npar.rgb_linear, t_cols=(0, 128))

    def all_layers(self):
        return self.P + [self.alpha, self.feature, self.views, self.rgb]

    def prep(self):
        for l in self.all_layers():
            l.prep()

    def forward(self, w, m_ptr, m_cap):
        kw = dict(m_ptr=m_ptr, m_cap=m_cap)
        N = w['NH']
        if USE_CHAIN:
            chain(Mat(w['XN']), self.P[0].k_valid,
                  [CL(self.P[0], EK_BIAS_RELU, 256, save=Mat(N[1])), CL(self.P[1], EK_BIAS_RELU, 256, save=Mat(N[2])),
                   CL(self.P[2], EK_BIAS_RELU, 256, save=Mat(N[3])), CL(self.P[3], EK_BIAS_RELU, 256, save=Mat(N[4])),
                   CL(self.P[4], EK_BIAS_RELU, 256, save=Mat(w['H5'], 84), write_a=False)], m_ptr, m_cap, tag='nerf_fwd_a')
            linear(Mat(w['H5']), self.P[5], Mat(N[6]), 256, act=ACT_RELU, **kw)
            chain(Mat(N[6]), 256,
                  [CL(self.P[6], EK_BIAS_RELU, 256, save=Mat(N[7])), CL(self.P[7], EK_BIAS_RELU, 256, save=Mat(N[8])),
                   CL(self.alpha, EK_BIAS_GENERIC, 1, save=Mat(w['DENS']), write_a=False),
                   CL(self.feature, EK_BIAS_GENERIC, 256, save=Mat(w['FV']), write_a=False)], m_ptr, m_cap, tag='nerf_fwd_b')
            linear(Mat(w['FV']), self.views, Mat(w['HV']), 128, act=ACT_RELU, **kw)
            linear(Mat(w['HV']), self.rgb, Mat(w['RGBRAW']), 3, **kw)
            return
        linear(Mat(w['XN']), self.P[0], Mat(N[1]), 256, act=ACT_RELU, **kw)
        linear(Mat(N[1]), self.P[1], Mat(N[2]), 256, act=ACT_RELU, **kw)
        linear(Mat(N[2]), self.P[2], Mat(N[3]), 256, act=ACT_RELU, **kw)
        linear(Mat(N[3]), self.P[3], Mat(N[4]), 256, act=ACT_RELU, **kw)
        linear(Mat(N[4]), self.P[4], Mat(w['H5'], 84), 256, act=ACT_RELU, **kw)
        linear(Mat(w['H5']), self.P[5], Mat(N[6]), 256, act=ACT_RELU, **kw)
        linear(Mat(N[6]), self.P[6], Mat(N[7]), 256, act=ACT_RELU, **kw)
        linear(Mat(N[7]), self.P[7], Mat(N[8]), 256, act=ACT_RELU, **kw)
        linear(Mat(N[8]), self.alpha, Mat(w['DENS']), 1, **kw)
        linear(Mat(N[8]), self.feature, Mat(w['FV']), 256, **kw)
        linear(Mat(w['FV']), self.views, Mat(w['HV']), 128, act=ACT_RELU, **kw)
        linear(Mat(w['HV']), self.rgb, Mat(w['RGBRAW']), 3, **kw)

    def backward(self, ws, w, m_ptr, m_cap):
        kw = dict(m_ptr=m_ptr, m_cap=m_cap)
        N, dA, dB = w['NH'], w['dNa'], w['dNb']
        n = self.np
        gp = lambda l: (l.weight.grad, None, l.bias.grad)
        R = dict(transposed=True, mode=EPI_MUL_DACT, dact=ACT_RELU)
        linear(Mat(w['dRGBRAW']), self.rgb, Mat(w['dHV']), 128, H=Mat(w['HV']), **R, **kw)
        wgrad(ws, Mat(w['dRGBRAW']), 3, Mat(w['HV']), 128, self.rgb, *gp(n.rgb_linear), **kw)
        linear(Mat(w['dHV']), self.views, Mat(w['dFV']), 256, transposed=True, mode=EPI_MUL_DACT, **kw)
        wgrad(ws, Mat(w['dHV']), 128, Mat(w['FV']), self.views.k_valid, self.views, *gp(n.views_linears[0]), **kw)
        linear(Mat(w['dFV']), self.feature, Mat(dA), 256, H=Mat(N[8]), **R, **kw)
        linear(Mat(w['dDENS']), self.alpha, Mat(dA), 256, H=Mat(N[8]), addend=Mat(dA), **R, **kw)
        wgrad(ws, Mat(w['dFV']), 256, Mat(N[8]), 256, self.feature, *gp(n.feature_linear), **kw)
        wgrad(ws, Mat(w['dDENS']), 1, Mat(N[8]), 256, self.alpha, *gp(n.alpha_linear), **kw)
        pl = n.pts_linears
        if USE_CHAIN:
            G = w['dNG']
            chain(Mat(dA), 256,
                  [CL(self.P[7], EK_DACT_RELU, 256, transposed=True, H=Mat(N[7]), save=Mat(G[6])),
                   CL(self.P[6], EK_DACT_RELU, 256, transposed=True, H=Mat(N[6]), save=Mat(G[5])),
                   CL(self.P[5], EK_DACT_RELU, 256, transposed=True, H=Mat(w['H5'], 84), save=Mat(G[4])),
                   CL(self.P[4], EK_DACT_RELU, 256, transposed=True, H=Mat(N[4]), save=Mat(G[3])),
                   CL(self.P[3], EK_DACT_RELU, 256, transposed=True, H=Mat(N[3]), save=Mat(G[2])),
                   CL(self.P[2], EK_DACT_RELU, 256, transposed=True, H=Mat(N[2]), save=Mat(G[1])),
                   CL(self.P[1], EK_DACT_RELU, 256, transposed=True, H=Mat(N[1]), save=Mat(G[0]))], m_ptr, m_cap, tag='nerf_bwd')
            wgrad(ws, Mat(dA), 256, Mat(N[7]), 256, self.P[7], *gp(pl[7]), **kw)
            wgrad(ws, Mat(G[6]), 256, Mat(N[6]), 256, self.P[6], *gp(pl[6]), **kw)
            wgrad(ws, Mat(G[5]), 256, Mat(w['H5']), self.P[5].k_valid, self.P[5], *gp(pl[5]), **kw)
            wgrad(ws, Mat(G[4]), 256, Mat(N[4]), 256, self.P[4], *gp(pl[4]), **kw)
            wgrad(ws, Mat(G[3]), 256, Mat(N[3]), 256, self.P[3], *gp(pl[3]), **kw)
            wgrad(ws, Mat(G[2]), 256, Mat(N[2]), 256, self.P[2], *gp(pl[2]), **kw)
            wgrad(ws, Mat(G[1]), 256, Mat(N[1]), 256, self.P[1], *gp(pl[1]), **kw)
            wgrad(ws, Mat(G[0]), 256, Mat(w['XN']), self.P[0].k_valid, self.P[0], *gp(pl[0]), **kw)
            return
        linear(Mat(dA), self.P[7], Mat(dB), 256, H=Mat(N[7]), **R, **kw)
        wgrad(ws, Mat(dA), 256, Mat(N[7]), 256, self.P[7], *gp(pl[7]), **kw)
        linear(Mat(dB), self.P[6], Mat(dA), 256, H=Mat(N[6]), **R, **kw)
        wgrad(ws, Mat(dB), 256, Mat(N[6]), 256, self.P[6], *gp(pl[6]), **kw)
        linear(Mat(dA), self.P[5], Mat(dB), 256, H=Mat(w['H5'], 84), **R, **kw)
        wgrad(ws, Mat(dA), 256, Mat(w['H5']), self.P[5].k_valid, self.P[5], *gp(pl[5]), **kw)
        linear(Mat(dB), self.P[4], Mat(dA), 256, H=Mat(N[4]), **R, **kw)
        wgrad(ws, Mat(dB), 256, Mat(N[4]), 256, self.P[4], *gp(pl[4]), **kw)
        linear(Mat(dA), self.P[3], Mat(dB), 256, H=Mat(N[3]), **R, **kw)
        wgrad(ws, Mat(dA), 256, Mat(N[3]), 256, self.P[3], *gp(pl[3]), **kw)
        linear(Mat(dB), self.P[2], Mat(dA), 256, H=Mat(N[2]), **R, **kw)
        wgrad(ws, Mat(dB), 256, Mat(N[2]), 256, self.P[2], *gp(pl[2]), **kw)
        linear(Mat(dA), self.P[1], Mat(dB), 256, H=Mat(N[1]), **R, **kw)
        wgrad(ws, Mat(dA), 256, Mat(N[1]), 256, self.P[1], *gp(pl[1]), **kw)
        wgrad(ws, Mat(dB), 256, Mat(w['XN']), self.P[0].k_valid, self.P[0], *gp(pl[0]), **kw)


class ShapeEngine:
    def __init__(self, params, cfg):
        self.p = params
        self.cfg = cfg
        self.scfg = params.color_network.cfg
        dev = params.deviation_network.variance.device
        ops.require_cuda(dev)
        self.dev = dev
        if self.scfg['light_pos_freq'] != 8:
            raise NotImplementedError('light_pos_freq != 8')
        upload_ide_table()
        self.human = bool(self.scfg['human_light'])
        self.exp_max = float(self.scfg['light_exp_max'])
        c = params.color_network
        self.sdf = SdfNet(params.sdf_network, dev)
        self.nerf = NerfNet(params.outer_nerf, dev)
        self.m_met = Predictor(c.metallic_predictor, dev, 1, ACT_SIGMOID, k_layout=259, t_cols=(0, 256))
        self.m_rough = Predictor(c.roughness_predictor, dev, 1, ACT_SIGMOID, k_layout=259, t_cols=(0, 256))
        self.m_alb = Predictor(c.albedo_predictor, dev, 3, ACT_SIGMOID, k_layout=259, t_cols=(0, 256))
        self.sphere = bool(self.scfg['sphere_direction'])
        self.e_iden, self.e_ld = (236, 384) if self.sphere else (E_IDEN, E_LD)
        ko = 144 if self.sphere else 72
        self.m_outer = Predictor(c.outer_light, dev, 3, ACT_EXPCLAMP, self.exp_max, k_layout=ko, t_cols=(0, ko))
        self.m_inner = Predictor(c.inner_light, dev, 3, ACT_EXPCLAMP, self.exp_max,
                                 kmap=list(range(51)) + [52 + i for i in range(72)], k_layout=124, t_cols=(52, 72))
        self.m_iw = Predictor(c.inner_weight, dev, 1, ACT_NONE, kmap=[40 + i for i in range(51)] + list(range(39)), k_layout=91)
        self.m_human = Predictor(c.human_light_predictor, dev, 4, ACT_EXPCLAMP, 0.0, k_layout=24, t_cols=(0, 24)) if self.human else None
        self.lut = c.FG_LUT
        self.grads = Grads(list(params.parameters()))
        self.ws = ops.WgradWorkspace(dev)
        self.ws.defer = True
        self.w = None
        self.cap = (0, 0)
        n, nb = cfg['n_samples'], cfg['n_bg_samples']
        zo = torch.linspace(1e-3, 1.0 - 1.0 / (nb + 1.0), nb)
        mids = .5 * (zo[1:] + zo[:-1])
        self.t_lin = torch.linspace(0.0, 1.0, n).to(dev)
        self.t_bg = zo.to(dev)
        self.t_bg_lo = torch.cat([zo[:1], mids]).to(dev)
        self.t_bg_hi = torch.cat([mids, zo[-1:]]).to(dev)
        self.t_lin64 = torch.linspace(0, 1, 64).to(dev)
        self.prepared_version = None
        self.car_dev = torch.zeros(1, device=dev)

    def predictors(self):
        ps = [self.m_met, self.m_rough, self.m_alb, self.m_outer, self.m_inner, self.m_iw]
        return ps + ([self.m_human] if self.human else [])

    def prepare_weights(self):
        if getattr(self, '_all_layers', None) is None:
            ls = self.sdf.L + [self.sdf.L8f, self.sdf.L8s] + self.nerf.all_layers()
            for m in self.predictors():
                ls += m.layers
            self._all_layers = ops.PrepBatch(ls)
        self._all_layers.run()

    def _alloc(self, R, S):
        if R <= self.cap[0] and S <= self.cap[1]:
            return
        R, S = max(R, self.cap[0]), max(S, self.cap[1])
        self.w = None
        dev = self.dev
        cap = R * S
        z = lambda *s, dt=torch.float32: torch.zeros(*s, dtype=dt, device=dev)
        w = {}
        ns = self.cfg['n_samples']
        caps = max(R * ns, self.cfg['occ_loss_max_pn'] * 64)
        w.update(SX0=z(caps, 64), SA=z(caps, 256), SB=z(caps, 256), SC=z(caps, 256), SSDF=z(caps, 1), SSDF0=z(R * ns, 1),
                 ZA=z(R, 128), ZB=z(R, 128), SDFA=z(R, 128), SDFB=z(R, 128), NEWZ=z(R, 32))
        w.update(cnt_in=z(R, dt=torch.int32), cnt_out=z(R, dt=torch.int32), off_in=z(R, dt=torch.int32), off_out=z(R, dt=torch.int32),
                 n_in=z(1, dt=torch.int32), n_out=z(1, dt=torch.int32), slot=z(R, S, dt=torch.int32))
        w.update(X0=z(cap, 64), PTS=z(cap, 4), RAY_IN=z(cap, dt=torch.int32), Y8=z(cap, Y8_LD), U0=z(cap, 64), USKIP=z(cap, 64),
                 G=z(cap, 4), OUTS=z(cap, O_LDIM), E=z(cap, self.e_ld), GEO=z(cap, 8), EH=z(cap, 64), COLOR_IN=z(cap, 4), OCCP=z(cap),
                 REFL=z(cap, 4), ALPHA_IN=z(cap), GERR=z(cap))
        w['H'] = [None] + [z(cap, 256) for _ in range(8)]
        w['V'] = [z(cap, 256) for _ in range(8)]
        names = ['met', 'rough', 'alb', 'odir', 'odif', 'inner', 'iw'] + (['human'] if self.human else [])
        w['ACT'] = {k: [z(cap, 256) for _ in range(3)] for k in names}
        w.update(XN=z(cap, 128), H5=z(cap, 384), DENS=z(cap, 4), FV=z(cap, 320), HV=z(cap, 128), RGBRAW=z(cap, 4), DIST_OUT=z(cap),
                 RAY_OUT=z(cap, dt=torch.int32), ALPHA_OUT=z(cap), COLOR_OUT=z(cap, 4))
        w['NH'] = [None] + [z(cap, 256) for _ in range(4)] + [None] + [z(cap, 256) for _ in range(3)]
        P = self.cfg['occ_loss_max_pn']
        w.update(SEL=z(cap, dt=torch.int32), OCC_COUNT=z(1, dt=torch.int32), OCC_O=z(P, 3), OCC_D=z(P, 3), OCC_Z=z(P, 64),
                 OCC_NEWZ=z(P, 16), OCC_GT=z(P), OCC_LOSS=z(1), DOCC=z(cap))
        self.w = w
        self.cap = (R, S)
        self.bw_ready = False

    def _alloc_reg(self):
        if 'REG_H' in self.w:
            return
        R, S = self.cap
        cap = R * S
        z = lambda *s, dt=torch.float32: torch.zeros(*s, dtype=dt, device=self.dev)
        self.w.update(REG_CNT=z(R, dt=torch.int32), REG_OFF=z(R, dt=torch.int32), REG_N=z(1, dt=torch.int32), REG_DUMMY=z(R, dt=torch.int32),
                      REG_DUMMY1=z(1, dt=torch.int32), REG_PTS=z(cap, 4), REG_X0=z(cap, 64), REG_SDF=z(cap, 1), REG_DSDF=z(cap, 1))
        self.w['REG_H'] = [None] + [z(cap, 256) for _ in range(8)]

    def reg_forward(self, rays_o, rays_d, z_vals):
        R, S = z_vals.shape
        self._alloc_reg()
        w = self.w
        K('nero_reg_prepare', rays_o, rays_d, z_vals, R, S, 1.2, w['REG_CNT'], w['REG_DUMMY'], w['REG_OFF'], w['REG_DUMMY'], w['REG_N'],
          w['REG_DUMMY1'])
        K('nero_reg_fill', rays_o, rays_d, z_vals, R, S, 1.2, w['REG_OFF'], w['REG_PTS'], w['REG_X0'], 64, w['REG_H'][4], 256)
        self.sdf.value_forward(w['REG_X0'], w['REG_H'], w['REG_SDF'], w['REG_N'], R * S)

    def reg_backward(self, d_sdf_vals):
        self._alloc_backward()
        self.grads.ensure()
        w = self.w
        k = d_sdf_vals.shape[0]
        w['REG_DSDF'][:k, 0].copy_(d_sdf_vals)
        cap = self.cap[0] * self.cap[1]
        self.sdf.value_backward(self.ws, w['REG_X0'], w['REG_H'], w['REG_DSDF'], w['ABAR'], w['dHa'], w['REG_N'], cap)
        self.ws.flush()

    def _alloc_backward(self):
        if self.bw_ready:
            return
        R, S = self.cap
        cap = R * S
        z = lambda *s: torch.zeros(*s, dtype=torch.float32, device=self.dev)
        w = self.w
        w.update(dALPHA_IN=z(cap), dCOLOR_IN=z(cap, 4), DOUTS=z(cap, O_LDIM), DNOV=z(cap), dE_dir=z(cap, 160), dE_inn=z(cap, 128),
                 dE_dif=z(cap, 160), dEH=z(cap, 64), DG=z(cap, 4), dY8=z(cap, Y8_LD), dHa=z(cap, 256), dHb=z(cap, 256), dHc=z(cap, 256),
                 D_INV_S=z(1))
        w['UB'] = [z(cap, 64)] + [z(cap, 256) for _ in range(8)]
        w['ABAR'] = [z(cap, 256) for _ in range(8)]
        w.update(dALPHA_OUT=z(cap), dCOLOR_OUT=z(cap, 4), dDENS=z(cap, 4), dRGBRAW=z(cap, 4), dHV=z(cap, 128), dFV=z(cap, 256),
                 dNa=z(cap, 256), dNb=z(cap, 256))
        w['dNG'] = [z(cap, 256) for _ in range(7)]
        self.bw_ready = True

    def sample_ray(self, rays_o, rays_d, near, far, rand_inner=None, rand_bg=None):
        cfg = self.cfg
        R = rays_o.shape[0]
        n, nb, nimp, steps = cfg['n_samples'], cfg['n_bg_samples'], cfg['n_importance'], cfg['up_sample_steps']
        S = n + nimp + nb
        nn_ = nimp // steps
        assert nimp % steps == 0 and nn_ <= 32 and n + nimp <= 128 and nb <= n, 'sampling kernels: <=32 new samples / step, <=128 inner samples'
        self._alloc(R, S)
        w = self.w
        z_vals = torch.empty(R, S, device=self.dev)
        var = self.p.deviation_network.variance.detach()
        K('nero_sample_init', rays_o, rays_d, near, far, R, n, nb, self.t_lin, self.t_bg, self.t_bg_lo, self.t_bg_hi,
          rand_inner, rand_bg, w['ZA'], 128, Mat(z_vals, n + nimp), S, w['SX0'], 64, w['SC'], 256)
        self.sdf.sdf_only(w['SX0'], w['SA'], w['SB'], w['SC'], w['SSDF0'], None, R * n)
        cur_z, cur_sdf, lds = w['ZA'], w['SSDF0'], n
        nxt_z, nxt_sdf = w['ZB'], w['SDFB']
        cur_n = n
        for i in range(steps):
            last = i + 1 == steps
            K('nero_upsample', rays_o, rays_d, R, cur_z, 128, cur_sdf, lds, cur_n, nn_, var, float(64 * 2 ** i),
              1 if cfg['clip_sample_variance'] else 0, 0, w['NEWZ'], 32, None if last else w['SX0'], 64,
              None if last else w['SC'], 256, None)
            if last:
                K('nero_merge_samples', cur_z, 128, None, 0, cur_n, w['NEWZ'], 32, None, 0, nn_, z_vals, S, None, 0, R)
            else:
                self.sdf.sdf_only(w['SX0'], w['SA'], w['SB'], w['SC'], w['SSDF'], None, R * nn_)
                K('nero_merge_samples', cur_z, 128, cur_sdf, lds, cur_n, w['NEWZ'], 32, w['SSDF'], nn_, nn_, nxt_z, 128, nxt_sdf, 128, R)
                cur_z, nxt_z = nxt_z, (w['ZA'] if nxt_z is w['ZB'] else w['ZB'])
                cur_sdf, nxt_sdf = nxt_sdf, (w['SDFA'] if nxt_sdf is w['SDFB'] else w['SDFB'])
                lds = 128
            cur_n += nn_
        return z_vals

    def render_core_forward(self, rays_o, rays_d, z_vals, human_poses, cos_anneal_ratio, step, perm=None, static=None):
        cfg = self.cfg
        R, S = z_vals.shape
        self._alloc(R, S)
        w = self.w
        cap = R * S
        if static is None:
            self.car_dev.fill_(float(cos_anneal_ratio))
        var = self.p.deviation_network.variance.detach()
        K('nero_ray_prepare', rays_o, rays_d, z_vals, R, S, w['cnt_in'], w['cnt_out'], w['off_in'], w['off_out'], w['n_in'], w['n_out'])
        K('nero_ray_fill', rays_o, rays_d, z_vals, R, S, w['off_in'], w['off_out'], w['slot'], w['PTS'], w['RAY_IN'],
          w['X0'], 64, w['Y8'], Y8_LD, w['H'][4], 256, w['XN'], 128, w['H5'], 384, w['FV'], 320, w['DIST_OUT'], w['RAY_OUT'])
        n_in, n_out = w['n_in'], w['n_out']
        self.sdf.forward_with_gradient(w, n_in, cap)
        self._shade_forward(rays_d, human_poses, n_in, cap)
        K('nero_sdf_alpha_fwd', w['Y8'], Y8_LD, Y8_SDF, w['G'], w['PTS'], w['RAY_IN'], rays_d, var, self.car_dev, w['ALPHA_IN'],
          w['GERR'], n_in, cap)
        self.nerf.forward(w, n_out, cap)
        K('nero_nerf_post_fwd', w['DENS'], 4, w['RGBRAW'], 4, w['DIST_OUT'], w['ALPHA_OUT'], w['COLOR_OUT'], n_out, cap)
        rgb = torch.empty(R, 3, device=self.dev)
        K('nero_composite_fwd', w['slot'], R, S, w['ALPHA_IN'], w['COLOR_IN'], w['ALPHA_OUT'], w['COLOR_OUT'], rgb, None)
        occ_on = cfg['apply_occ_loss'] and step >= cfg['occ_loss_step']
        P = 0
        if occ_on:
            K('nero_occ_select', w['PTS'], w['Y8'], Y8_LD, Y8_SDF, w['G'], w['RAY_IN'], rays_d, float(cfg['occ_sdf_thresh']), n_in, cap,
              w['SEL'], w['OCC_COUNT'])
        with_reg = step < 1000
        if static is not None:
            assert not with_reg, 'the SDF-initialisation phase (step < 1000) runs eagerly'
            P = self._occ_forward_static(static) if occ_on else 0
            self.n_reg = 0
            self.state = dict(R=R, S=S, N_in=None, P=P, rays_d=rays_d, hp=self._hp, step=step)
            return rgb
        if with_reg:
            self.reg_forward(rays_o, rays_d, z_vals)
            w = self.w
        counts = torch.cat([w['n_in'], w['OCC_COUNT'], w['REG_N'] if with_reg else w['n_out']]).tolist()
        N_in = counts[0]
        self.n_reg = counts[2] if with_reg else 0
        if occ_on:
            P = self._occ_forward(counts[1], perm)
        self.state = dict(R=R, S=S, N_in=N_in, P=P, rays_d=rays_d, hp=self._hp, step=step)
        return rgb, N_in, P

    def _occ_forward(self, cnt, perm):
        cfg, w = self.cfg, self.w
        maxp = cfg['occ_loss_max_pn']
        if cnt == 0:
            return 0
        sel = w['SEL']
        if cnt > maxp:
            idx = perm if perm is not None else torch.randperm(cnt, device=self.dev)
            sel = torch.sort(sel[:cnt])[0][idx[:maxp].to(self.dev)].contiguous()
            cnt = maxp
            w['SEL_SUB'] = sel
        return self._occ_march(sel, None, cnt)

    def _occ_forward_static(self, static):
        w = self.w
        maxp = self.cfg['occ_loss_max_pn']
        cnt = w['OCC_COUNT']
        keys = torch.where(static.ar < cnt, static.occ_keys, 2.0)
        maxp = min(maxp, keys.shape[0])
        vals, idx = torch.topk(keys, maxp, largest=False)
        static.P_dev = (vals < 1.5).sum(dtype=torch.int32).reshape(1)
        sel = w['SEL'][idx].contiguous()
        return self._occ_march(sel, static.P_dev, maxp)

    def _occ_march(self, sel, p_ptr, P):
        w = self.w
        var = self.p.deviation_network.variance.detach()
        K('nero_occ_init', w['PTS'], w['REFL'], sel, p_ptr, P, 64, self.t_lin64, w['OCC_O'], w['OCC_D'], w['OCC_Z'], 64, w['SX0'], 64,
          w['SC'], 256)
        self.sdf.sdf_only(w['SX0'], w['SA'], w['SB'], w['SC'], w['SSDF'], None, P * 64)
        K('nero_upsample', w['OCC_O'], w['OCC_D'], P, w['OCC_Z'], 64, w['SSDF'], 64, 64, 16, var, 3.0e38, 1, 1, w['OCC_NEWZ'], 16,
          w['SX0'], 64, w['SC'], 256, None)
        self.sdf.sdf_only(w['SX0'], w['SA'], w['SB'], w['SC'], w['SSDF'], None, P * 16)
        K('nero_upsample', w['OCC_O'], w['OCC_D'], P, w['OCC_NEWZ'], 16, w['SSDF'], 16, 16, 16, var, 3.0e38, 1, 1, None, 0, None, 0, None, 0,
          w['OCC_GT'])
        w['OCC_LOSS'].zero_()
        w['DOCC'].zero_()
        K('nero_occ_loss', w['OCCP'], w['OCC_GT'], sel, p_ptr, P, w['OCC_LOSS'], w['DOCC'])
        self.occ_sel = sel
        return P

    def _shade_forward(self, rays_d, human_poses, n_in, cap):
        w = self.w
        A = w['ACT']
        matin = Mat(w['Y8'])
        self.m_met.forward(matin, A['met'], Mat(w['OUTS'], O_MET), n_in, cap)
        self.m_rough.forward(matin, A['rough'], Mat(w['OUTS'], O_ROUGH), n_in, cap)
        self.m_alb.forward(matin, A['alb'], Mat(w['OUTS'], O_ALB), n_in, cap)
        hp = human_poses.contiguous() if self.human else None
        self._hp = hp
        K('nero_shade_prep_fwd', w['G'], w['PTS'], w['RAY_IN'], rays_d, w['OUTS'], w['E'], self.e_ld, w['GEO'], hp, w['EH'] if self.human else None,
          64, 8, n_in, cap, 1 if self.sphere else 0)
        self.m_outer.forward(Mat(w['E'], E_IDER), A['odir'], Mat(w['OUTS'], O_LDIR), n_in, cap)
        self.m_outer.forward(Mat(w['E'], self.e_iden), A['odif'], Mat(w['OUTS'], O_LD), n_in, cap)
        self.m_inner.forward(Mat(w['E'], E_PE8X), A['inner'], Mat(w['OUTS'], O_LI), n_in, cap)
        self.m_iw.forward(Mat(w['E'], 0), A['iw'], Mat(w['OUTS'], O_IW), n_in, cap)
        if self.human:
            self.m_human.forward(Mat(w['EH']), A['human'], Mat(w['OUTS'], O_HUM), n_in, cap)
        K('nero_shade_combine_fwd', w['OUTS'], w['GEO'], self.lut, self.exp_max, 1 if self.human else 0, w['COLOR_IN'], w['OCCP'], w['REFL'],
          n_in, cap)

    QUERY_CHUNK = 131072

    def sdf_query(self, x):
        shape = x.shape[:-1]
        x = x.reshape(-1, 3).to(self.dev, torch.float32).contiguous()
        M = x.shape[0]
        out = torch.empty(M, 1, device=self.dev)
        if M == 0:
            return out.reshape(*shape, 1)
        q = getattr(self, '_qws', None)
        if q is None:
            c = self.QUERY_CHUNK
            z = lambda *s: torch.zeros(*s, device=self.dev)
            q = self._qws = dict(X0=z(c, 64), SA=z(c, 256), SB=z(c, 256), SC=z(c, 256), OUT=z(c, 1))
        self.sdf.prep()
        for c0 in range(0, M, self.QUERY_CHUNK):
            n = min(self.QUERY_CHUNK, M - c0)
            K('nero_points_fill', x[c0:c0 + n], n, None, None, q['X0'], 64, None, 0, q['SC'], 256)
            self.sdf.sdf_only(q['X0'], q['SA'], q['SB'], q['SC'], q['OUT'], None, n)
            out[c0:c0 + n] = q['OUT'][:n]
        return out.reshape(*shape, 1)

    def materials_query(self, x):
        x = x.reshape(-1, 3).to(self.dev, torch.float32).contiguous()
        M = x.shape[0]
        if self.w is None:
            self._alloc(self.cfg['test_ray_num'], self.cfg['n_samples'] + self.cfg['n_importance'] + self.cfg['n_bg_samples'])
        w = self.w
        chunk = w['X0'].shape[0]
        out = torch.empty(M, 5, device=self.dev)
        A = w['ACT']
        for c0 in range(0, M, chunk):
            n = min(chunk, M - c0)
            K('nero_points_fill', x[c0:c0 + n], n, w['PTS'], w['RAY_IN'], w['X0'], 64, w['Y8'], Y8_LD, w['H'][4], 256)
            H = w['H']
            self.sdf.hidden_forward(w['X0'], [H[1], H[2], H[3], H[4], H[5], H[6], H[7], H[8]], H[4], None, n, save=False,
                                    heads=[CL(self.sdf.L8f, EK_BIAS_GENERIC, 256, save=Mat(w['Y8']), write_a=False)])
            matin = Mat(w['Y8'])
            self.m_met.forward(matin, A['met'], Mat(w['OUTS'], O_MET), None, n)
            self.m_rough.forward(matin, A['rough'], Mat(w['OUTS'], O_ROUGH), None, n)
            self.m_alb.forward(matin, A['alb'], Mat(w['OUTS'], O_ALB), None, n)
            o = w['OUTS'][:n]
            out[c0:c0 + n, 0] = o[:, O_MET]
            out[c0:c0 + n, 1] = o[:, O_ROUGH]
            out[c0:c0 + n, 2:5] = o[:, O_ALB:O_ALB + 3]
        return out[:, 0:1], out[:, 1:2], out[:, 2:5]

    def validation_info(self, rays_o, rays_d, z_vals, human_poses):
        R, S = z_vals.shape
        w, dev = self.w, self.dev
        weights = torch.empty(R, S, device=dev)
        rgb = torch.empty(R, 3, device=dev)
        K('nero_composite_fwd', w['slot'], R, S, w['ALPHA_IN'], w['COLOR_IN'], w['ALPHA_OUT'], w['COLOR_OUT'], rgb, weights)
        depth = torch.sum(weights * z_vals, -1, keepdim=True)
        points = (depth * rays_d + rays_o).contiguous()
        K('nero_points_fill', points, R, w['PTS'], w['RAY_IN'], w['X0'], 64, w['Y8'], Y8_LD, w['H'][4], 256)
        self.sdf.forward_with_gradient(w, None, R)
        self._shade_forward(rays_d, human_poses, None, R)
        O = w['OUTS'][:R]
        geo = w['GEO'][:R]
        grads = w['G'][:R, :3]
        inner = (torch.norm(points, dim=-1, keepdim=True) <= 1.0).float()
        met, rough, alb = O[:, O_MET:O_MET + 1], O[:, O_ROUGH:O_ROUGH + 1], O[:, O_ALB:O_ALB + 3]
        Ld, Ldir, Li, iw = O[:, O_LD:O_LD + 3], O[:, O_LDIR:O_LDIR + 3], O[:, O_LI:O_LI + 3], O[:, O_IW:O_IW + 1]
        occ = iw * 0.5 + 0.5
        occ_ = occ.clamp(0, 1)
        if self.human:
            hit = geo[:, 7:8]
            hl = O[:, O_HUM:O_HUM + 4] * hit
            Lh, wh = hl[:, :3], hl[:, 3:].clamp(0, 1)
        else:
            Lh, wh = 0.0, 0.0
        spec_light = Li * occ_ + (Lh * wh + Ldir * (1 - wh)) * (1 - occ_)
        uv = torch.cat([geo[:, 3:4].clamp(0, 1), rough.clamp(0, 1)], -1)
        fg = _fg_lookup_torch(self.lut[0], uv)
        diff_alb = (1 - met) * alb
        spec_alb = 0.04 * (1 - met) + met * alb
        spec_ref = spec_alb * fg[:, 0:1] + fg[:, 1:2]
        srgb = _linear_to_srgb_torch
        out = {'depth': depth, 'normal': ((torch.nn.functional.normalize(grads, dim=-1) + 1.0) * 0.5) * inner}
        inter = {'specular_albedo': spec_alb, 'specular_ref': spec_ref.clamp(0, 1), 'specular_light': srgb(spec_light).clamp(0, 1),
                 'specular_color': srgb(spec_ref * spec_light).clamp(0, 1), 'diffuse_albedo': diff_alb,
                 'diffuse_light': srgb(Ld).clamp(0, 1), 'diffuse_color': srgb(diff_alb * Ld).clamp(0, 1), 'metallic': met.clone(),
                 'roughness': rough.clone(), 'occ_prob': occ.clamp(0, 1), 'indirect_light': Li * occ_}
        if self.human:
            inter['human_light'] = srgb(Lh * wh)
        sel = torch.nonzero(torch.norm(points, dim=-1) < 0.999)[:, 0].to(torch.int32).contiguous()
        P = int(sel.shape[0])
        gt = torch.zeros(R, 1, device=dev)
        if P > 0:
            var = self.p.deviation_network.variance.detach()
            if not hasattr(self, 't_lin128'):
                self.t_lin128 = torch.linspace(0, 1, 128).to(dev)
            chunk = w['SX0'].shape[0] // 128
            oo, dd = torch.empty(chunk, 3, device=dev), torch.empty(chunk, 3, device=dev)
            zz, nz, g_ = torch.empty(chunk, 128, device=dev), torch.empty(chunk, 16, device=dev), torch.empty(chunk, device=dev)
            for c0 in range(0, P, chunk):
                sl = sel[c0:c0 + chunk]
                pc = int(sl.shape[0])
                K('nero_occ_init', w['PTS'], w['REFL'], sl, None, pc, 128, self.t_lin128, oo, dd, zz, 128, w['SX0'], 64, w['SC'], 256)
                self.sdf.sdf_only(w['SX0'], w['SA'], w['SB'], w['SC'], w['SSDF'], None, pc * 128)
                K('nero_upsample', oo, dd, pc, zz, 128, w['SSDF'], 128, 128, 9, var, 3.0e38, 1, 1, nz, 16, w['SX0'], 64, w['SC'], 256, None)
                self.sdf.sdf_only(w['SX0'], w['SA'], w['SB'], w['SC'], w['SSDF'], None, pc * 9)
                K('nero_upsample', oo, dd, pc, nz, 16, w['SSDF'], 9, 9, 9, var, 3.0e38, 1, 1, None, 0, None, 0, None, 0, g_)
                gt[sl.long(), 0] = g_[:pc]
        out['occ_prob_gt'] = gt
        out.update({k: v * inner for k, v in inter.items()})
        return out

    def render_core_backward(self, d_rgb, d_gerr, d_occ_scale, static=None):
        self._alloc_backward()
        if static is None:
            self.grads.ensure()
        st, w, cfg = self.state, self.w, self.cfg
        R, S, cap = st['R'], st['S'], st['R'] * st['S']
        rays_d = st['rays_d']
        n_in, n_out = w['n_in'], w['n_out']
        var_p = self.p.deviation_network.variance
        var = var_p.detach()
        ws = self.ws
        K('nero_composite_bwd', w['slot'], R, S, w['ALPHA_IN'], w['COLOR_IN'], w['ALPHA_OUT'], w['COLOR_OUT'], d_rgb.contiguous(),
          w['dALPHA_IN'], w['dCOLOR_IN'], w['dALPHA_OUT'], w['dCOLOR_OUT'])
        K('nero_nerf_post_bwd', w['DENS'], 4, w['RGBRAW'], 4, w['DIST_OUT'], w['dALPHA_OUT'], w['dCOLOR_OUT'], w['dDENS'], 4, w['dRGBRAW'], 4,
          n_out, cap)
        self.nerf.backward(ws, w, n_out, cap)
        docc = None
        if d_occ_scale is not None and st['P'] > 0:
            docc = w['DOCC'] * d_occ_scale
        K('nero_shade_combine_bwd', w['OUTS'], w['GEO'], self.lut, self.exp_max, 1 if self.human else 0, w['dCOLOR_IN'], docc, w['DOUTS'],
          w['DNOV'], n_in, cap)
        A = w['ACT']
        dHa, dHb, dHc = w['dHa'], w['dHb'], w['dHc']
        ko = 144 if self.sphere else 72
        self.m_outer.backward(ws, Mat(w['DOUTS'], O_LDIR), Mat(w['E'], E_IDER), A['odir'], dHa, dHb, n_in, cap, dX=Mat(w['dE_dir']), dx_ncol=ko, dHc=dHc)
        self.m_outer.backward(ws, Mat(w['DOUTS'], O_LD), Mat(w['E'], self.e_iden), A['odif'], dHa, dHb, n_in, cap, dX=Mat(w['dE_dif']), dx_ncol=ko, dHc=dHc)
        self.m_inner.backward(ws, Mat(w['DOUTS'], O_LI), Mat(w['E'], E_PE8X), A['inner'], dHa, dHb, n_in, cap, dX=Mat(w['dE_inn']), dx_ncol=72, dHc=dHc)
        self.m_iw.backward(ws, Mat(w['DOUTS'], O_IW), Mat(w['E'], 0), A['iw'], dHa, dHb, n_in, cap, dHc=dHc)
        if self.human:
            self.m_human.backward(ws, Mat(w['DOUTS'], O_HUM), Mat(w['EH']), A['human'], dHa, dHb, n_in, cap, dX=Mat(w['dEH']), dx_ncol=24, dHc=dHc)
        K('nero_shade_prep_bwd', w['G'], w['PTS'], w['RAY_IN'], rays_d, w['OUTS'], w['GEO'], w['dE_dir'], 160, w['dE_inn'], 128, w['dE_dif'], 160,
          w['dEH'] if self.human else None, 64, st['hp'], w['DNOV'], w['DOUTS'], w['DG'], n_in, cap, 1 if self.sphere else 0)
        matin = Mat(w['Y8'])
        self.m_rough.backward(ws, Mat(w['DOUTS'], O_ROUGH), matin, A['rough'], dHa, dHb, n_in, cap, dX=Mat(w['dY8']), dx_ncol=256, dHc=dHc)
        self.m_met.backward(ws, Mat(w['DOUTS'], O_MET), matin, A['met'], dHa, dHb, n_in, cap, dX=Mat(w['dY8']), dx_ncol=256, dx_addend=Mat(w['dY8']), dHc=dHc)
        self.m_alb.backward(ws, Mat(w['DOUTS'], O_ALB), matin, A['alb'], dHa, dHb, n_in, cap, dX=Mat(w['dY8']), dx_ncol=256, dx_addend=Mat(w['dY8']), dHc=dHc)
        w['D_INV_S'].zero_()
        dg = None if d_gerr is None else d_gerr.contiguous()
        K('nero_sdf_alpha_bwd', w['Y8'], Y8_LD, Y8_SDF, w['G'], w['PTS'], w['RAY_IN'], rays_d, var, self.car_dev, w['dALPHA_IN'], dg,
          w['dY8'], Y8_LD, w['DG'], w['D_INV_S'], n_in, cap)
        frozen = cfg['freeze_inv_s_step'] is not None and st['step'] < cfg['freeze_inv_s_step']
        if not frozen:
            inv_s = torch.exp(var * 10.0)
            inr = ((inv_s >= 1e-6) & (inv_s <= 1e6)).float()
            var_p.grad.add_((w['D_INV_S'][0] * 10.0 * inv_s * inr).reshape(var_p.shape))
        self.sdf.backward(ws, w, n_in, cap, None)
        ws.flush()
```

### nero_b200/ops.py

```python
import ctypes
import os

import torch

_HERE = os.path.dirname(os.path.abspath(__file__))
_LIB_PATH = os.environ.get('NERO_LIB') or os.path.join(_HERE, 'libnero_b200.so')

ACT_NONE, ACT_SOFTPLUS100, ACT_RELU, ACT_SIGMOID, ACT_EXPCLAMP = 0, 1, 2, 3, 4
EPI_BIAS_ACT, EPI_MUL_DACT, EPI_TANGENT = 0, 1, 2
_NPADS = (16, 64, 128, 224, 256)

if not os.path.exists(_LIB_PATH):
    raise ImportError(f'{_LIB_PATH} is missing: run `python -c "import __graft_entry__ as g; g.build()"` '
                      '(nero_b200 has no CPU or PyTorch fallback)')
lib = ctypes.CDLL(_LIB_PATH)

launch_count = 0


def require_cuda(dev, what='nero_b200'):
    if torch.device(dev).type != 'cuda':
        raise RuntimeError(f'{what} runs on a CUDA device only (move the module with .cuda(); there is no CPU fallback)')


def _ptr(t):
    if t is None:
        return ctypes.c_void_p(0)
    return ctypes.c_void_p(t.data_ptr())


def _stream():
    return ctypes.c_void_p(torch.cuda.current_stream().cuda_stream)


def _check(rc, name):
    if rc != 0:
        raise RuntimeError(f'{name} failed with code {rc}')


def npad_for(n):
    for c in _NPADS:
        if n <= c:
            return c
    raise ValueError(f'width {n} > 256 not supported by one UMMA tile')


def ceil_div(a, b):
    return (a + b - 1) // b


class PreparedLayer:

    def __init__(self, weight, g, bias, device, row0=0, nrows=None, kmap=None, k_layout=None, t_cols=None):
        self.weight, self.g, self.bias = weight, g, bias
        N, K = weight.shape
        self.K = K
        self.row0 = row0
        self.nrows = N - row0 if nrows is None else nrows
        self.k_layout = k_layout if k_layout is not None else K
        self.kmap_host = kmap
        self.kmap = None if kmap is None else torch.tensor(kmap, dtype=torch.int32, device=device)
        self.n_pad = npad_for(self.nrows)
        self.k_chunks = ceil_div(self.k_layout, 64)
        self.k_valid = ceil_div(self.k_layout, 4) * 4
        self.img_f = torch.zeros(self.k_chunks * 2 * self.n_pad * 128, dtype=torch.uint8, device=device)
        self.t_cols = t_cols
        if t_cols is not None:
            self.t_npad = npad_for(t_cols[1])
            self.t_chunks = ceil_div(self.nrows, 64)
            self.img_t = torch.zeros(self.t_chunks * 2 * self.t_npad * 128, dtype=torch.uint8, device=device)
        else:
            self.img_t = None
        self.w_eff = torch.zeros(N, K, dtype=torch.float32, device=device)

    def prep(self):
        global launch_count
        w = self.weight.detach()
        g = None if self.g is None else self.g.detach()
        rc = lib.nero_prep_weight(_ptr(w), _ptr(g), self.K, self.row0, self.nrows, _ptr(self.kmap), ctypes.c_float(1.0),
                                  _ptr(self.img_f), self.n_pad, _ptr(self.img_t), self.t_npad if self.img_t is not None else 0,
                                  self.t_cols[0] if self.t_cols else 0, self.t_cols[1] if self.t_cols else 0,
                                  _ptr(self.w_eff), self.K, _stream())
        _check(rc, 'nero_prep_weight')
        launch_count += 1

    def bias_view(self):
        return None if self.bias is None else self.bias.detach()[self.row0:self.row0 + self.nrows]


_PREP_JOB = None


class PrepBatch:

    def __init__(self, layers):
        self.layers = list(layers)
        self.key, self.tab, self.max_rows = None, None, 0

    @staticmethod
    def _ptrs(l):
        p = lambda t: 0 if t is None else t.data_ptr()
        return (p(l.weight), p(l.g), p(l.kmap), p(l.img_f), p(l.img_t), p(l.w_eff))

    def run(self):
        global _PREP_JOB, launch_count
        if not self.layers:
            return
        import numpy as np
        if _PREP_JOB is None:
            _PREP_JOB = np.dtype([('v', 'u8'), ('g', 'u8'), ('kmap', 'u8'), ('img_f', 'u8'), ('img_t', 'u8'), ('w_eff', 'u8'), ('K', 'i4'),
                                  ('row0', 'i4'), ('nrows', 'i4'), ('rows_pad_f', 'i4'), ('rows_pad_t', 'i4'), ('t_c0', 'i4'),
                                  ('t_ncols', 'i4'), ('ld_weff', 'i4'), ('in_scale', 'f4'), ('pad', 'i4')])
            assert _PREP_JOB.itemsize == 88
        key = tuple(self._ptrs(l) for l in self.layers)
        if key != self.key:
            arr = np.zeros(len(self.layers), dtype=_PREP_JOB)
            for i, (l, pt) in enumerate(zip(self.layers, key)):
                arr[i] = pt + (l.K, l.row0, l.nrows, l.n_pad, l.t_npad if l.img_t is not None else 0, l.t_cols[0] if l.t_cols else 0,
                               l.t_cols[1] if l.t_cols else 0, l.K, 1.0, 0)
            self.tab = torch.from_numpy(arr.view(np.uint8).copy()).to(self.layers[0].img_f.device)
            self.key, self.max_rows = key, int(arr['nrows'].max())
        rc = lib.nero_prep_weight_batch(_ptr(self.tab), len(self.layers), self.max_rows, _stream())
        _check(rc, 'nero_prep_weight_batch')
        launch_count += 1


class Mat:
    __slots__ = ('t', 'c0', 'ncol')

    def __init__(self, t, c0=0, ncol=None):
        self.t, self.c0 = t, c0
        self.ncol = t.shape[1] - c0 if ncol is None else ncol

    @property
    def ld(self):
        return self.t.stride(0)

    def ptr(self):
        return ctypes.c_void_p(self.t.data_ptr() + 4 * self.c0)

    def view(self, m=None):
        v = self.t[:, self.c0:self.c0 + self.ncol]
        return v if m is None else v[:m]


def linear(A: Mat, layer: PreparedLayer, out: Mat, ncol_out, *, transposed=False, mode=EPI_BIAS_ACT, act=ACT_NONE,
           act_param=0.0, oscale=1.0, H: Mat = None, hscale=1.0, dact=ACT_NONE, V: Mat = None, out2: Mat = None,
           addend: Mat = None, ncol_main=None, tail: Mat = None, m_ptr=None, m_cap=None, use_bias=True):
    global launch_count
    if ncol_main is None:
        ncol_main = ncol_out
    if transposed:
        img, n_pad, k_chunks, k_valid = layer.img_t, layer.t_npad, layer.t_chunks, ceil_div(layer.nrows, 4) * 4
        bias = None
    else:
        img, n_pad, k_chunks, k_valid = layer.img_f, layer.n_pad, layer.k_chunks, layer.k_valid
        bias = layer.bias_view() if use_bias else None
    if m_cap is None:
        m_cap = A.t.shape[0]
    rc = lib.nero_linear(A.ptr(), A.ld, k_valid, _ptr(img), n_pad, k_chunks, _ptr(bias), 0 if bias is None else bias.numel(), out.ptr(), out.ld, ncol_out,
                         ctypes.c_float(oscale), mode, act, ctypes.c_float(act_param),
                         H.ptr() if H else None, H.ld if H else 0, ctypes.c_float(hscale), dact,
                         V.ptr() if V else None, V.ld if V else 0, out2.ptr() if out2 else None, out2.ld if out2 else 0,
                         addend.ptr() if addend else None, addend.ld if addend else 0, ncol_main,
                         tail.ptr() if tail else None, tail.ld if tail else 0, _ptr(m_ptr), m_cap, _stream())
    _check(rc, 'nero_linear')
    launch_count += 1


_FINISH_JOB = None


def _finish_job_dtype():
    global _FINISH_JOB
    if _FINISH_JOB is None:
        import numpy as np
        _FINISH_JOB = np.dtype([('partial', 'u8'), ('bias_partial', 'u8'), ('kmap', 'u8'), ('v', 'u8'), ('g', 'u8'), ('grad_w', 'u8'),
                                ('grad_g', 'u8'), ('grad_b', 'u8'), ('extra_row', 'u8'), ('P', 'i4'), ('rows_partial', 'i4'),
                                ('ld_partial', 'i4'), ('K', 'i4'), ('row0', 'i4'), ('nrows', 'i4'), ('in_scale', 'f4'),
                                ('extra_scale', 'f4')])
        assert _FINISH_JOB.itemsize == 104
    return _FINISH_JOB


class WgradWorkspace:

    def __init__(self, device, P=74, rows=256, ld=384, max_slots=48):
        self.P, self.rows, self.ld = P, rows, ld
        self.device, self.max_slots = device, max_slots
        self.pool = torch.zeros(max_slots, rows * ld + rows, dtype=torch.float32, device=device)
        self.jobs, self.dest, self.keep = [], set(), []
        self.defer = False
        self._tabs = {}

    def _slot(self):
        i = len(self.jobs)
        row = self.pool[i]
        return row[:self.rows * self.ld].view(1, self.rows, self.ld), row[self.rows * self.ld:].view(1, self.rows)

    @property
    def partial(self):
        return self._slot()[0]

    @property
    def bias_partial(self):
        return self._slot()[1]

    def enqueue(self, job, dest_key, keep):
        self.jobs.append(job)
        self.dest.add(dest_key)
        self.keep.append(keep)
        if len(self.jobs) >= self.max_slots:
            self.flush()

    def flush(self):
        global launch_count
        if not self.jobs:
            return
        key = tuple(self.jobs)
        hit = self._tabs.get(key)
        if hit is None:
            import numpy as np
            arr = np.zeros(len(self.jobs), dtype=_finish_job_dtype())
            for i, j in enumerate(self.jobs):
                arr[i] = j
            if len(self._tabs) >= 64:
                self._tabs.clear()
            hit = self._tabs[key] = (torch.from_numpy(arr.view(np.uint8).copy()).to(self.device), int(arr['nrows'].max()),
                                     int(arr['K'].max()))
        tab, max_rows, max_k = hit
        rc = lib.nero_wgrad_finish_batch(_ptr(tab), len(self.jobs), max_rows, max_k, _stream())
        _check(rc, 'nero_wgrad_finish_batch')
        launch_count += 1
        self.pool[:len(self.jobs)].zero_()
        self.jobs, self.dest, self.keep = [], set(), []


def wgrad(ws: WgradWorkspace, dY: Mat, n_valid, X: Mat, k_valid, layer: PreparedLayer, grad_w, grad_g, grad_b,
          dY2: Mat = None, X2: Mat = None, m_ptr=None, m_cap=None, with_bias=True):
    global launch_count
    if m_cap is None:
        m_cap = dY.t.shape[0]
    n_rows_pad = ceil_div(n_valid, 16) * 16
    k_pad = ceil_div(layer.k_layout, 64) * 64
    assert k_pad <= ws.ld and n_rows_pad <= ws.rows
    if ws.defer and grad_w is not None and (grad_w.data_ptr(), layer.row0) in ws.dest:
        ws.flush()
    partial_t, bias_t = ws.partial, ws.bias_partial
    P = ws.P * 2 // ceil_div(n_rows_pad, 128) if n_rows_pad <= 128 else ws.P
    if not ws.defer:
        partial_t.zero_()
        bias_t.zero_()
    rc = lib.nero_wgrad(dY.ptr(), dY.ld, n_valid, X.ptr(), X.ld, k_valid,
                        dY2.ptr() if dY2 else None, dY2.ld if dY2 else 0, X2.ptr() if X2 else None, X2.ld if X2 else 0,
                        _ptr(partial_t), ws.ld, ws.rows, _ptr(bias_t), n_rows_pad, k_pad, P, _ptr(m_ptr),
                        m_cap, _stream())
    _check(rc, 'nero_wgrad')
    launch_count += ceil_div(n_rows_pad, 128) * max(1, ceil_div(k_pad, 256))
    g = None if layer.g is None else layer.g.detach()
    w_ = layer.weight.detach()
    if ws.defer:
        ptr = lambda t: 0 if t is None else t.data_ptr()
        job = (ptr(partial_t), ptr(bias_t) if with_bias else 0, ptr(layer.kmap), ptr(w_), ptr(g), ptr(grad_w), ptr(grad_g),
               ptr(grad_b) if with_bias else 0, 0, 1, ws.rows, ws.ld, layer.K, layer.row0, layer.nrows, 1.0, 0.0)
        ws.enqueue(job, (grad_w.data_ptr(), layer.row0), (w_, g))
        return
    rc = lib.nero_wgrad_finish(_ptr(partial_t), 1, ws.rows, ws.ld, _ptr(bias_t) if with_bias else None,
                               layer.K, layer.row0, layer.nrows, _ptr(layer.kmap), ctypes.c_float(1.0),
                               _ptr(w_), _ptr(g), _ptr(grad_w), _ptr(grad_g),
                               _ptr(grad_b) if with_bias else None, None, ctypes.c_float(0.0), _stream())
    _check(rc, 'nero_wgrad_finish')
    launch_count += 1


def colsum(X: Mat, ncol, out, w: Mat = None, m_ptr=None, m_cap=None):
    global launch_count
    if m_cap is None:
        m_cap = X.t.shape[0]
    rc = lib.nero_colsum(X.ptr(), X.ld, ncol, w.ptr() if w else None, w.ld if w else 0, _ptr(m_ptr), m_cap, _ptr(out),
                         _stream())
    _check(rc, 'nero_colsum')
    launch_count += 1


def K(name, *args):
    global launch_count
    conv = []
    for a in args:
        if a is None:
            conv.append(ctypes.c_void_p(0))
        elif isinstance(a, torch.Tensor):
            conv.append(ctypes.c_void_p(a.data_ptr()))
        elif isinstance(a, Mat):
            conv.append(a.ptr())
        elif isinstance(a, float):
            conv.append(ctypes.c_float(a))
        elif isinstance(a, ctypes._SimpleCData):
            conv.append(a)
        else:
            conv.append(int(a))
    rc = getattr(lib, name)(*conv, _stream())
    _check(rc, name)
    launch_count += 1


def positional_encoding(x, L, scale=1.0):
    global launch_count
    x = x.contiguous().float()
    M, d = x.shape
    out = torch.empty(M, d * (1 + 2 * L), device=x.device)
    rc = lib.nero_pe(_ptr(x), d, d, M, L, ctypes.c_float(scale), _ptr(out), out.shape[1], _stream())
    _check(rc, 'nero_pe')
    launch_count += 1
    return out


def integrated_dir_enc(dirs, kappa_inv):
    global launch_count
    from .engine import upload_ide_table
    upload_ide_table()
    dirs = dirs.contiguous().float()
    M = dirs.shape[0]
    out = torch.empty(M, 72, device=dirs.device)
    if torch.is_tensor(kappa_inv):
        k = kappa_inv.reshape(-1).contiguous().float()
        rc = lib.nero_ide(_ptr(dirs), 3, _ptr(k), 1, ctypes.c_float(0.0), M, _ptr(out), 72, _stream())
    else:
        rc = lib.nero_ide(_ptr(dirs), 3, None, 0, ctypes.c_float(float(kappa_inv)), M, _ptr(out), 72, _stream())
    _check(rc, 'nero_ide')
    launch_count += 1
    return out


EK_BIAS_SOFTPLUS, EK_BIAS_RELU, EK_BIAS_GENERIC, EK_DACT_SOFTPLUS, EK_DACT_RELU, EK_DACT_NONE, EK_TANGENT = range(7)


class _ChainLayer(ctypes.Structure):
    _fields_ = [('wimg', ctypes.c_void_p), ('bias', ctypes.c_void_p),
                ('save', ctypes.c_void_p), ('H', ctypes.c_void_p), ('addend', ctypes.c_void_p), ('V', ctypes.c_void_p),
                ('out2', ctypes.c_void_p), ('tail', ctypes.c_void_p),
                ('n_pad', ctypes.c_int), ('k_chunks', ctypes.c_int), ('n_bias', ctypes.c_int), ('ncol_out', ctypes.c_int),
                ('ncol_main', ctypes.c_int), ('kind', ctypes.c_int), ('act', ctypes.c_int),
                ('ld_save', ctypes.c_int), ('ldh', ctypes.c_int), ('ldadd', ctypes.c_int), ('ldv', ctypes.c_int),
                ('ldo2', ctypes.c_int), ('ldt', ctypes.c_int),
                ('oscale', ctypes.c_float), ('hscale', ctypes.c_float), ('act_param', ctypes.c_float),
                ('write_a', ctypes.c_int), ('a_blocks', ctypes.c_int),
                ('csrc', ctypes.c_void_p), ('ld_csrc', ctypes.c_int), ('pad_', ctypes.c_int)]


class _ChainParams(ctypes.Structure):
    _fields_ = [('A0', ctypes.c_void_p), ('lda0', ctypes.c_int), ('k_valid0', ctypes.c_int),
                ('n_layers', ctypes.c_int), ('m_ptr', ctypes.c_void_p), ('m_cap', ctypes.c_int),
                ('L', _ChainLayer * 10)]


def _p(m):
    if m is None:
        return None
    if isinstance(m, Mat):
        return m.t.data_ptr() + 4 * m.c0
    return m.data_ptr()


def chain_layer(layer: PreparedLayer, kind, ncol_out, *, transposed=False, save: Mat = None, act=ACT_NONE, act_param=0.0, oscale=1.0,
                H: Mat = None, hscale=1.0, V: Mat = None, out2: Mat = None, addend: Mat = None, ncol_main=None, tail: Mat = None,
                write_a=True, csrc: Mat = None, use_bias=True):
    return dict(layer=layer, kind=kind, ncol_out=ncol_out, transposed=transposed, save=save, act=act, act_param=act_param, oscale=oscale,
                H=H, hscale=hscale, V=V, out2=out2, addend=addend, ncol_main=ncol_out if ncol_main is None else ncol_main, tail=tail,
                write_a=write_a, csrc=csrc, use_bias=use_bias)


PROFILE = None


def chain(A0: Mat, k_valid0, layers, m_ptr=None, m_cap=None, tag=''):
    global launch_count
    assert 1 <= len(layers) <= 10
    if m_cap is None:
        m_cap = A0.t.shape[0]
    P = _ChainParams()
    P.A0, P.lda0, P.k_valid0 = _p(A0), A0.ld, ceil_div(k_valid0, 4) * 4
    P.n_layers, P.m_ptr, P.m_cap = len(layers), _p(m_ptr), m_cap
    keep = []
    for i, d in enumerate(layers):
        lay, L = d['layer'], P.L[i]
        if d['transposed']:
            img, n_pad, k_chunks, bias = lay.img_t, lay.t_npad, lay.t_chunks, None
        else:
            img, n_pad, k_chunks = lay.img_f, lay.n_pad, lay.k_chunks
            bias = lay.bias_view() if d['use_bias'] else None
        assert k_chunks <= 4 and d['ncol_out'] <= n_pad
        keep.append(bias)
        L.wimg, L.bias, L.n_bias = _p(img), _p(bias), 0 if bias is None else bias.numel()
        L.n_pad, L.k_chunks, L.ncol_out, L.ncol_main, L.kind, L.act = n_pad, k_chunks, d['ncol_out'], d['ncol_main'], d['kind'], d['act']
        for name, key, ldname in (('save', 'save', 'ld_save'), ('H', 'H', 'ldh'), ('addend', 'addend', 'ldadd'), ('V', 'V', 'ldv'),
                                  ('out2', 'out2', 'ldo2'), ('tail', 'tail', 'ldt'), ('csrc', 'csrc', 'ld_csrc')):
            m = d[key]
            setattr(L, name, _p(m))
            setattr(L, ldname, m.ld if m is not None else 0)
        L.oscale, L.hscale, L.act_param = d['oscale'], d['hscale'], d['act_param']
        L.write_a = 1 if (d['write_a'] and i + 1 < len(layers)) else 0
        nxt = layers[i + 1]['layer'] if i + 1 < len(layers) else None
        if nxt is not None:
            nk = nxt.t_chunks if layers[i + 1]['transposed'] else nxt.k_chunks
            L.a_blocks = 4 * nk
    if PROFILE is not None:
        fl = 0.0
        for d in layers:
            lay = d['layer']
            kdim = lay.nrows if d['transposed'] else lay.K
            fl += 2.0 * kdim * d['ncol_out']
        e0, e1 = torch.cuda.Event(enable_timing=True), torch.cuda.Event(enable_timing=True)
        e0.record()
    rc = lib.nero_chain(ctypes.byref(P), _stream())
    _check(rc, 'nero_chain')
    launch_count += 1
    if PROFILE is not None:
        e1.record()
        PROFILE.append((tag, e0, e1, fl, None if m_ptr is None else m_ptr.data_ptr(), m_cap))


_vp, _ci, _cf = ctypes.c_void_p, ctypes.c_int, ctypes.c_float


class McParams(ctypes.Structure):
    _fields_ = [('pts', _vp), ('normals', _vp), ('view', _vp), ('rough', _vp), ('poses', _vp), ('rand_d', _vp), ('rand_s', _vp),
                ('tab_d', _vp), ('tab_s', _vp), ('P', _ci), ('Sd', _ci), ('Ss', _ci), ('ggx_smith', _ci), ('sphere_dir', _ci),
                ('human', _ci), ('org', _vp), ('dir', _vp), ('pos_depth', _vp), ('nrm_hit', _vp), ('slot', _vp), ('blk_cnt', _vp),
                ('blk_off', _vp), ('counts', _vp), ('EO', _vp), ('ldeo', _ci), ('EH', _vp), ('ldeh', _ci), ('hhit', _vp), ('EI', _vp),
                ('ldei', _ci), ('OUT_O', _vp), ('OUT_H', _vp), ('OUT_I', _vp), ('exp_max_o', _cf), ('exp_max_i', _cf), ('LD', _vp),
                ('LS', _vp), ('LSF', _vp), ('dLD', _vp), ('dLS', _vp), ('dLSF', _vp), ('DPRE_O', _vp), ('DPRE_H', _vp), ('DPRE_I', _vp),
                ('dA', _vp), ('dEO', _vp), ('dEH', _vp), ('dEI', _vp), ('dA2', _vp)]

    def set(self, **kw):
        for k, v in kw.items():
            if isinstance(v, torch.Tensor):
                v = v.data_ptr()
            elif isinstance(v, Mat):
                v = v.t.data_ptr() + 4 * v.c0
            setattr(self, k, v)
        return self


def mc(name, params: McParams):
    global launch_count
    rc = getattr(lib, name)(ctypes.byref(params), _stream())
    _check(rc, name)
    launch_count += 1


def bvh_build(verts, tris):
    import numpy as np
    verts = np.ascontiguousarray(verts, np.float32)
    tris = np.ascontiguousarray(tris, np.int32)
    T = tris.shape[0]
    nodes = np.zeros((2 * T, 32), np.uint8)
    tri = np.zeros((T, 12), np.float32)
    ids = np.zeros(T, np.int32)
    n = ctypes.c_int(0)
    rc = lib.nero_bvh_build_host(verts.ctypes.data_as(_vp), verts.shape[0], tris.ctypes.data_as(_vp), T, nodes.ctypes.data_as(_vp),
                                 tri.ctypes.data_as(_vp), ids.ctypes.data_as(_vp), ctypes.byref(n))
    _check(rc, 'nero_bvh_build_host')
    return nodes[:n.value].copy(), tri, ids
```

Before: 80930.

## Group wgrad GEMMs into one persistent kernel with MN-major tiles and double-buffered TMEM

Replaces the per-layer templated wgrad kernel launches with a single persistent grouped kernel. It walks a job table of work units (n-tile, k-slice, M-slice) across a fixed CTA count. The new kernel uses 32-row MN-major K chunks with float4 loads, 4 smem stages, 512 TMEM columns double-buffered between MMA and dedicated epilogue warps, and register rebalancing via setmaxnreg. This is meant to cut launch overhead and overlap epilogue reductions with the next unit's MMAs. In exchange it adds host-side job packing and a 16-byte alignment requirement on operands.

```diff
diff --git a/include/nero_b200.h b/include/nero_b200.h
--- a/include/nero_b200.h
+++ b/include/nero_b200.h
@@ -45,10 +45,10 @@
 int nero_chain(const void* chain_params_host, void* stream);
 int nero_row_axpy(const float* a, int lda, const float* X, int ldx, float* Y, int ldy, int ncol, const int* m_ptr, int m_cap, void* stream);
 
-int nero_wgrad(const float* dY, int ldy, int n_valid, const float* X, int ldx, int k_valid,
-               const float* dY2, int ldy2, const float* X2, int ldx2,
-               float* partial, int ld_partial, int rows_partial, float* bias_partial,
-               int n_rows_pad, int k_pad, int P, const int* m_ptr, int m_cap, void* stream);
+int nero_wgrad_job(void* rec, const float* dY, int ldy, const float* X, int ldx, const float* dY2, int ldy2, const float* X2, int ldx2,
+                   int n_valid, int k_valid, float* partial, int ld_partial, int rows_partial, float* bias_partial, const int* m_ptr,
+                   int m_cap, int k_pad, int n_ctas, int* units);
+int nero_wgrad_group(const void* jobs_dev, int n_jobs, int n_units, int n_ctas, void* stream);
 int nero_wgrad_finish(const float* partial, int P, int rows_partial, int ld_partial, const float* bias_partial, int K,
                       int row0, int nrows, const int* kmap, float in_scale, const float* v, const float* g,
                       float* grad_w, float* grad_g, float* grad_b, const float* extra_row, float extra_scale, void* stream);
diff --git a/nero_b200/csrc/api.cu b/nero_b200/csrc/api.cu
--- a/nero_b200/csrc/api.cu
+++ b/nero_b200/csrc/api.cu
@@ -15,16 +15,11 @@
   int ncol_main; float* tail; int ldt;
   const int* m_ptr; int m_cap;
 };
-struct WgradParams {
-  const float* dY; int ldy; const float* X; int ldx;
-  const float* dY2; int ldy2; const float* X2; int ldx2;
-  int n0; int n_valid; int k0; int k_valid;
-  float* partial; int ld_partial; int rows_partial;
-  float* bias_partial;
-  const int* m_ptr; int m_cap;
-};
 int linear_dispatch(const LinearParams& p, cudaStream_t stream);
-int wgrad_dispatch(WgradParams p, int n_rows_pad, int k_pad, int P, cudaStream_t stream);
+int wgrad_group(const void* jobs_dev, int n_jobs, int n_units, int n_ctas, cudaStream_t stream);
+int wgrad_job(void* rec, const float* dY, int ldy, const float* X, int ldx, const float* dY2, int ldy2, const float* X2, int ldx2,
+              int n_valid, int k_valid, float* partial, int ld_partial, int rows_partial, float* bias_partial, const int* m_ptr,
+              int m_cap, int k_pad, int n_ctas, int* units);
 int prep_weight(const float* v, const float* g, int K, int row0, int nrows, const int* kmap, float in_scale,
                 uint8_t* img_f, int rows_pad_f, uint8_t* img_t, int rows_pad_t, int t_c0, int t_ncols, float* w_eff, int ld_weff,
                 cudaStream_t stream);
@@ -176,14 +171,14 @@
   return linear_dispatch(p, (cudaStream_t)stream);
 }
 
-int nero_wgrad(const float* dY, int ldy, int n_valid, const float* X, int ldx, int k_valid,
-               const float* dY2, int ldy2, const float* X2, int ldx2,
-               float* partial, int ld_partial, int rows_partial, float* bias_partial,
-               int n_rows_pad, int k_pad, int P, const int* m_ptr, int m_cap, void* stream) {
-  WgradParams p{dY, ldy, X, ldx, dY2, ldy2, X2, ldx2, 0, n_valid, 0, k_valid, partial, ld_partial, rows_partial, bias_partial,
-                m_ptr, m_cap};
-  if (!dY || !X || !partial || (dY2 && !X2)) return NERO_ERR_ARG;
-  return wgrad_dispatch(p, n_rows_pad, k_pad, P, (cudaStream_t)stream);
+int nero_wgrad_job(void* rec, const float* dY, int ldy, const float* X, int ldx, const float* dY2, int ldy2, const float* X2, int ldx2,
+                   int n_valid, int k_valid, float* partial, int ld_partial, int rows_partial, float* bias_partial, const int* m_ptr,
+                   int m_cap, int k_pad, int n_ctas, int* units) {
+  return wgrad_job(rec, dY, ldy, X, ldx, dY2, ldy2, X2, ldx2, n_valid, k_valid, partial, ld_partial, rows_partial, bias_partial, m_ptr,
+                   m_cap, k_pad, n_ctas, units);
+}
+int nero_wgrad_group(const void* jobs_dev, int n_jobs, int n_units, int n_ctas, void* stream) {
+  return wgrad_group(jobs_dev, n_jobs, n_units, n_ctas, (cudaStream_t)stream);
 }
 
 int nero_wgrad_finish(const float* partial, int P, int rows_partial, int ld_partial, const float* bias_partial, int K,
@@ -226,6 +221,7 @@
     case 2: return int(sizeof(nero_mc_params));
     case 3: return 104;
     case 4: return 88;
+    case 5: return 112;
     default: return -1;
   }
 }
diff --git a/nero_b200/csrc/k_umma_wgrad.cu b/nero_b200/csrc/k_umma_wgrad.cu
--- a/nero_b200/csrc/k_umma_wgrad.cu
+++ b/nero_b200/csrc/k_umma_wgrad.cu
@@ -1,3 +1,5 @@
+
+#include <cstring>
 
 #include "common.cuh"
 #include "ptx.cuh"
@@ -5,27 +7,29 @@
 
 namespace nero {
 
-struct WgradParams {
-  const float* dY; int ldy; const float* X; int ldx;
-  const float* dY2; int ldy2; const float* X2; int ldx2;
-  int n0; int n_valid;
-  int k0; int k_valid;
-  float* partial; int ld_partial; int rows_partial;
-  float* bias_partial;
-  const int* m_ptr; int m_cap;
+struct WgradJob {
+  const float* dY; const float* X; const float* dY2; const float* X2;
+  float* partial; float* bias_partial;
+  const int* m_ptr;
+  int ldy, ldx, ldy2, ldx2;
+  int n_valid, k_valid;
+  int ld_partial, rows_partial;
+  int m_cap;
+  int n_tiles, k_pad, n_slices;
+  int unit0, pad_;
 };
-
-constexpr int WG_BM = 128, WG_BK = 64;
-constexpr int kWgProdWarps = 16;
-constexpr int kWgThreads = (kWgProdWarps + 1) * 32;
-constexpr uint32_t kWgABytes = WG_BM * 128;
-
-template <int NW> struct WgCfg {
-  static constexpr uint32_t b_plane = NW * 128;
-  static constexpr uint32_t stage_bytes = 2 * kWgABytes + 2 * b_plane;
-  static constexpr int stages = (stage_bytes * 3 <= 200 * 1024) ? 3 : 2;
-  static constexpr uint32_t smem_bytes = stages * stage_bytes + 1024 + 256 + 512;
-};
+static_assert(sizeof(WgradJob) == 112, "WgradJob layout is part of the C ABI (nero_wgrad_group)");
+
+constexpr int WG_BM = 128, MN_BK = 32;
+constexpr int kWgProdWarps = 16, kMnGroupWarps = kWgProdWarps / 2, kWgMmaWarp = 16, kWgEpiWarp0 = 20;
+constexpr int kWgThreads = 6 * 128;
+constexpr int kWgStages = 4;
+constexpr uint32_t kMnSbo = 1024, kMnLbo = (MN_BK / 8) * 1024;
+constexpr uint32_t kAPlane = WG_BM * MN_BK * 2, kBPlane = 256 * MN_BK * 2;
+constexpr uint32_t kStageBytes = 2 * kAPlane + 2 * kBPlane;
+constexpr int kSlabLd = 36;
+constexpr uint32_t kSlabBytes = 4 * 32 * kSlabLd * 4;
+constexpr uint32_t kWgSmemBytes = 1024 + kWgStages * kStageBytes + kSlabBytes + 2 * 128 * 4 + 256;
 
 __device__ __forceinline__ void wg_split2(float x0, float x1, uint32_t& hi, uint32_t& lo) {
   __nv_bfloat162 h = __floats2bfloat162_rn(x0, x1);
@@ -36,419 +40,288 @@
   lo = *reinterpret_cast<uint32_t*>(&l);
 }
 
-template <int NOCT>
-__device__ __forceinline__ void load_octets(const float* __restrict__ src, int ld, int col, bool col_ok, int s0, int M, uint32_t oct0,
-                                            float (&x)[NOCT][8]) {
-#pragma unroll
-  for (int o = 0; o < NOCT; ++o)
-#pragma unroll
-    for (int i = 0; i < 8; ++i) {
-      const int s = s0 + (oct0 + o) * 8 + i;
-      x[o][i] = (col_ok && s < M) ? __ldg(src + size_t(s) * ld + col) : 0.0f;
-    }
-}
-template <int NOCT>
-__device__ __forceinline__ float store_octets(const float (&x)[NOCT][8], uint8_t* plane_hi, uint8_t* plane_lo, uint32_t row, uint32_t oct0) {
-  float sum = 0.0f;
-#pragma unroll
-  for (int o = 0; o < NOCT; ++o) {
-    uint32_t hw[4], lw[4];
-#pragma unroll
-    for (int i = 0; i < 4; ++i) {
-      wg_split2(x[o][2 * i], x[o][2 * i + 1], hw[i], lw[i]);
-      sum += x[o][2 * i] + x[o][2 * i + 1];
-    }
-    const uint32_t off = row * 128u + (((oct0 + o) ^ (row & 7u)) << 4);
-    *reinterpret_cast<uint4*>(plane_hi + off) = make_uint4(hw[0], hw[1], hw[2], hw[3]);
-    *reinterpret_cast<uint4*>(plane_lo + off) = make_uint4(lw[0], lw[1], lw[2], lw[3]);
-  }
-  return sum;
-}
-
 __device__ __forceinline__ void red_add_v4(float* addr, float a, float b, float c, float d) {
   asm volatile("red.global.add.v4.f32 [%0], {%1, %2, %3, %4};" ::"l"(addr), "f"(a), "f"(b), "f"(c), "f"(d) : "memory");
 }
 
-template <int NW>
-__device__ __forceinline__ void wg_epilogue(const WgradParams& p, uint32_t tmem_base, int pw, int lane, int n0, bool any, const float* s_bias) {
-  const int orow = n0 + pw * 32 + lane;
-  float* prow = p.partial + size_t(orow) * p.ld_partial + p.k0;
-  const uint32_t taddr = tmem_base + (uint32_t(pw * 32) << 16);
-  if (any) {
-#pragma unroll 1
-    for (int cc = 0; cc < (NW + 31) / 32; ++cc) {
-      float v[32];
-      tmem_ld32(taddr + cc * 32, v);
-      tmem_ld_wait();
-      if (orow < p.rows_partial) {
-#pragma unroll
-        for (int j = 0; j < 32; j += 4)
-          if (cc * 32 + j < NW) red_add_v4(prow + cc * 32 + j, v[j], v[j + 1], v[j + 2], v[j + 3]);
-      }
-    }
-    if (p.bias_partial && p.k0 == 0 && orow < p.rows_partial) atomicAdd(&p.bias_partial[orow], s_bias[pw * 32 + lane]);
+__device__ __forceinline__ uint32_t mn_chunk_offset(uint32_t chunk, uint32_t s) {
+  const uint32_t r = s & 7u;
+  return (chunk >> 3) * kMnLbo + (s >> 3) * kMnSbo + r * 128u + (((chunk & 7u) ^ r) << 4);
+}
+
+struct WgUnit {
+  const WgradJob* j;
+  int n0, k0, width;
+  int M, c_begin, nc1, nch;
+  bool bias;
+};
+
+__device__ __forceinline__ WgUnit wg_unit(const WgradJob* __restrict__ jobs, int n_jobs, int u) {
+  int ji = 0;
+  while (ji + 1 < n_jobs && jobs[ji + 1].unit0 <= u) ++ji;
+  WgUnit w;
+  w.j = jobs + ji;
+  const int n_tiles = w.j->n_tiles, n_slices = w.j->n_slices, k_pad = w.j->k_pad;
+  const int local = u - w.j->unit0;
+  const int kt = local / (n_tiles * n_slices), r = local % (n_tiles * n_slices);
+  const int slice = r / n_tiles;
+  w.n0 = (r % n_tiles) * WG_BM;
+  int k0 = 0, width = 0;
+  for (int t = 0;; ++t) {
+    const int rem = k_pad - k0;
+    width = rem >= 256 ? 256 : rem >= 128 ? 128 : 64;
+    if (t == kt) break;
+    k0 += width;
   }
-}
-
-template <int NW>
-__global__ void __launch_bounds__(kWgThreads, 1) umma_wgrad_kernel(const WgradParams p) {
-  using Cfg = WgCfg<NW>;
-  constexpr int STAGES = Cfg::stages;
+  w.k0 = k0;
+  w.width = width;
+  int M = w.j->m_ptr ? *w.j->m_ptr : w.j->m_cap;
+  w.M = M > w.j->m_cap ? w.j->m_cap : M;
+  const int total = (w.M + MN_BK - 1) / MN_BK;
+  const int cpp = (total + n_slices - 1) / n_slices;
+  w.c_begin = min(total, slice * cpp);
+  w.nc1 = min(total, w.c_begin + cpp) - w.c_begin;
+  w.nch = w.nc1 * (w.j->dY2 ? 2 : 1);
+  w.bias = w.j->bias_partial != nullptr && k0 == 0 && w.nch > 0;
+  return w;
+}
+
+__global__ void __launch_bounds__(kWgThreads, 1) umma_wgrad_group_kernel(const WgradJob* __restrict__ jobs, int n_jobs, int n_units) {
   extern __shared__ uint8_t smem_raw[];
   uint8_t* smem = reinterpret_cast<uint8_t*>((reinterpret_cast<uintptr_t>(smem_raw) + 1023) & ~uintptr_t(1023));
-  uint64_t* bars = reinterpret_cast<uint64_t*>(smem + STAGES * Cfg::stage_bytes);
-  uint64_t* full = bars;
-  uint64_t* empty = bars + STAGES;
-  uint64_t* tfull = bars + 2 * STAGES;
-  uint32_t* tmem_slot = reinterpret_cast<uint32_t*>(bars + 2 * STAGES + 1);
-  float* s_bias = reinterpret_cast<float*>(smem + STAGES * Cfg::stage_bytes + 256);
+  float* slab = reinterpret_cast<float*>(smem + kWgStages * kStageBytes);
+  float* s_bias = slab + kSlabBytes / 4;
+  uint64_t* full = reinterpret_cast<uint64_t*>(s_bias + 2 * 128);
+  uint64_t* empty = full + kWgStages;
+  uint64_t* tfull = empty + kWgStages;
+  uint64_t* tempty = tfull + 2;
+  uint64_t* bfull = tempty + 2;
+  uint32_t* tmem_slot = reinterpret_cast<uint32_t*>(bfull + 2);
 
   const int warp = threadIdx.x >> 5, lane = threadIdx.x & 31;
-  int M = p.m_ptr ? *p.m_ptr : p.m_cap;
-  if (M > p.m_cap) M = p.m_cap;
-  const int P = gridDim.x;
-  const int n0 = p.n0 + int(blockIdx.y) * WG_BM;
-  const int total_chunks = (M + WG_BK - 1) / WG_BK;
-  const int cpp = (total_chunks + P - 1) / P;
-  const int c_begin = min(total_chunks, int(blockIdx.x) * cpp), c_end = min(total_chunks, c_begin + cpp);
-  const int npairs = p.dY2 ? 2 : 1;
-  const int nc1 = c_end - c_begin;
-  const int nchunks = nc1 * npairs;
-
   if (threadIdx.x == 0) {
-    for (int s = 0; s < STAGES; ++s) { mbar_init(&full[s], kWgProdWarps); mbar_init(&empty[s], 1); }
-    mbar_init(tfull, 1);
+    for (int s = 0; s < kWgStages; ++s) { mbar_init(&full[s], kMnGroupWarps); mbar_init(&empty[s], 1); }
+    for (int b = 0; b < 2; ++b) { mbar_init(&tfull[b], 1); mbar_init(&tempty[b], 4); mbar_init(&bfull[b], kWgProdWarps); }
     fence_mbar_init();
   }
-  if (threadIdx.x < 128) s_bias[threadIdx.x] = 0.0f;
-  if (warp == kWgProdWarps) tmem_alloc<256>(tmem_slot);
+  if (threadIdx.x < 256) s_bias[threadIdx.x] = 0.0f;
+  if (warp == kWgMmaWarp) tmem_alloc<512>(tmem_slot);
   tcgen05_fence_before();
   __syncthreads();
   tcgen05_fence_after();
   const uint32_t tmem_base = *tmem_slot;
 
   if (warp < kWgProdWarps) {
-    const bool is_a = warp < 8;
-    const int pw = warp & 3;
-    const int oh = (warp >> 2) & 1;
-    float bias_acc = 0.0f;
-    for (int g = 0; g < nchunks; ++g) {
-      const int s = g % STAGES;
-      const int pair = g / nc1;
-      const int chunk = c_begin + g % nc1;
-      const int s0 = chunk * WG_BK;
-      uint8_t* st = smem + s * Cfg::stage_bytes;
-      if (is_a) {
-        const float* src = pair ? p.dY2 : p.dY;
-        const int ld = pair ? p.ldy2 : p.ldy;
-        const uint32_t row = pw * 32 + lane;
-        const int col = n0 + int(row);
-        const bool ok = col < p.n_valid;
-        float x[4][8];
-        load_octets<4>(src, ld, col, ok, s0, M, oh * 4, x);
-        mbar_wait(&empty[s], ((g / STAGES) & 1) ^ 1);
-        const float sacc = store_octets<4>(x, st, st + kWgABytes, row, oh * 4);
-        if (pair == 0) bias_acc += sacc;
-      } else {
-        const float* src = pair ? p.X2 : p.X;
-        const int ld = pair ? p.ldx2 : p.ldx;
-        uint8_t* bh = st + 2 * kWgABytes;
-        constexpr int NJ = (NW + 127) / 128;
-        float x[NJ][4][8];
-#pragma unroll
-        for (int j = 0; j < NJ; ++j) {
-          const uint32_t row = j * 128 + pw * 32 + lane;
-          const int col = p.k0 + int(row);
-          load_octets<4>(src, ld, col, row < NW && col < p.k_valid, s0, M, oh * 4, x[j]);
-        }
-        mbar_wait(&empty[s], ((g / STAGES) & 1) ^ 1);
-#pragma unroll
-        for (int j = 0; j < NJ; ++j) {
-          const uint32_t row = j * 128 + pw * 32 + lane;
-          if (row < NW) store_octets<4>(x[j], bh, bh + Cfg::b_plane, row, oh * 4);
-        }
+    asm volatile("setmaxnreg.inc.sync.aligned.u32 96;");
+    const uint32_t a_chunk = lane & 15, a_sub = lane >> 4;
+    const int group = warp / kMnGroupWarps, wi = warp % kMnGroupWarps;
+    uint32_t gbase = 0;
+    int it = 0;
+    for (int u = blockIdx.x; u < n_units; u += gridDim.x, ++it) {
+      const WgUnit w = wg_unit(jobs, n_jobs, u);
+      const WgradJob& jb = *w.j;
+      const int lcb = w.width == 256 ? 5 : w.width == 128 ? 4 : 3;
+      const int tpw = 2 + (1 << (lcb - 3));
+      const uint32_t b_chunk = lane & ((1u << lcb) - 1), b_sub = lane >> lcb;
+      const int spw = 32 >> lcb;
+      const int a_col = w.n0 + int(a_chunk) * 8, b_col = w.k0 + int(b_chunk) * 8;
+      float bsum[8] = {0.f, 0.f, 0.f, 0.f, 0.f, 0.f, 0.f, 0.f};
+      for (int l = int((group ^ gbase) & 1); l < w.nch; l += 2) {
+        const uint32_t g = gbase + l;
+        const int s = g % kWgStages;
+        const int pair = l / w.nc1;
+        const int s0 = (w.c_begin + l % w.nc1) * MN_BK;
+        uint8_t* st = smem + s * kStageBytes;
+        const float* srcA = pair ? jb.dY2 : jb.dY;
+        const int ldA = pair ? jb.ldy2 : jb.ldy;
+        const float* srcB = pair ? jb.X2 : jb.X;
+        const int ldB = pair ? jb.ldx2 : jb.ldx;
+        float4 v[6][2];
+#pragma unroll
+        for (int i = 0; i < 6; ++i) {
+          if (i >= tpw) break;
+          const bool isA = i < 2;
+          const int sl = isA ? 2 * (wi + 8 * i) + int(a_sub) : (wi + 8 * (i - 2)) * spw + int(b_sub);
+          const int srow = s0 + sl;
+          const int col = isA ? a_col : b_col;
+          const int lim = isA ? jb.n_valid : jb.k_valid;
+          const float* rp = (isA ? srcA : srcB) + size_t(srow) * (isA ? ldA : ldB) + col;
+          const bool rok = srow < w.M;
+          v[i][0] = (rok && col < lim) ? __ldg(reinterpret_cast<const float4*>(rp)) : make_float4(0.f, 0.f, 0.f, 0.f);
+          v[i][1] = (rok && col + 4 < lim) ? __ldg(reinterpret_cast<const float4*>(rp + 4)) : make_float4(0.f, 0.f, 0.f, 0.f);
+        }
+        mbar_wait(&empty[s], ((g / kWgStages) & 1) ^ 1);
+#pragma unroll
+        for (int i = 0; i < 6; ++i) {
+          if (i >= tpw) break;
+          const bool isA = i < 2;
+          const int sl = isA ? 2 * (wi + 8 * i) + int(a_sub) : (wi + 8 * (i - 2)) * spw + int(b_sub);
+          const int col = isA ? a_col : b_col;
+          const int lim = isA ? jb.n_valid : jb.k_valid;
+          float x[8] = {v[i][0].x, v[i][0].y, v[i][0].z, v[i][0].w, v[i][1].x, v[i][1].y, v[i][1].z, v[i][1].w};
+#pragma unroll
+          for (int j = 0; j < 8; ++j) if (col + j >= lim) x[j] = 0.f;
+          uint32_t hw[4], lw[4];
+#pragma unroll
+          for (int j = 0; j < 4; ++j) wg_split2(x[2 * j], x[2 * j + 1], hw[j], lw[j]);
+          uint8_t* hi = isA ? st : st + 2 * kAPlane;
+          uint8_t* lo = isA ? st + kAPlane : st + 2 * kAPlane + kBPlane;
+          const uint32_t off = mn_chunk_offset(isA ? a_chunk : b_chunk, uint32_t(sl));
+          *reinterpret_cast<uint4*>(hi + off) = make_uint4(hw[0], hw[1], hw[2], hw[3]);
+          *reinterpret_cast<uint4*>(lo + off) = make_uint4(lw[0], lw[1], lw[2], lw[3]);
+          if (isA && pair == 0) {
+#pragma unroll
+            for (int j = 0; j < 8; ++j) bsum[j] += x[j];
+          }
+        }
+        fence_proxy_async_smem();
+        __syncwarp();
+        if (lane == 0) mbar_arrive(&full[s]);
       }
-      fence_proxy_async_smem();
+      const int buf = it & 1;
+      mbar_wait(&tempty[buf], ((it >> 1) & 1) ^ 1);
+      if (w.bias) {
+#pragma unroll
+        for (int j = 0; j < 8; ++j) {
+          bsum[j] += __shfl_xor_sync(0xffffffffu, bsum[j], 16);
+          if (lane < 16) atomicAdd(&s_bias[buf * 128 + a_chunk * 8 + j], bsum[j]);
+        }
+      }
       __syncwarp();
-      if (lane == 0) mbar_arrive(&full[s]);
+      if (lane == 0) mbar_arrive(&bfull[buf]);
+      gbase += w.nch;
     }
-    if (is_a) atomicAdd(&s_bias[pw * 32 + lane], bias_acc);
-    asm volatile("bar.sync 1, %0;" ::"n"(kWgProdWarps * 32));
-    if (warp < 4) {
-      mbar_wait(tfull, 0);
+  } else if (warp < kWgEpiWarp0) {
+    asm volatile("setmaxnreg.dec.sync.aligned.u32 40;");
+    if (warp != kWgMmaWarp) goto done;
+    uint32_t g = 0;
+    int it = 0;
+    for (int u = blockIdx.x; u < n_units; u += gridDim.x, ++it) {
+      const WgUnit w = wg_unit(jobs, n_jobs, u);
+      const int buf = it & 1;
+      mbar_wait(&tempty[buf], ((it >> 1) & 1) ^ 1);
       tcgen05_fence_after();
-      wg_epilogue<NW>(p, tmem_base, pw, lane, n0, nchunks > 0, s_bias);
+      const uint32_t tacc = tmem_base + uint32_t(buf * 256);
+      const uint32_t idesc = make_idesc_bf16_mn(WG_BM, uint32_t(w.width));
+      for (int l = 0; l < w.nch; ++l, ++g) {
+        const int s = g % kWgStages;
+        mbar_wait(&full[s], (g / kWgStages) & 1);
+        tcgen05_fence_after();
+        if (elect_one()) {
+          const uint32_t a_hi = smem_u32(smem + s * kStageBytes);
+          const uint32_t a_lo = a_hi + kAPlane;
+          const uint32_t b_hi = a_hi + 2 * kAPlane;
+          const uint32_t b_lo = b_hi + kBPlane;
+#pragma unroll
+          for (int k = 0; k < MN_BK / 16; ++k) {
+            const uint32_t ko = k * 2 * kMnSbo;
+            const uint64_t dah = make_desc_mn_sw128(a_hi + ko, kMnLbo, kMnSbo), dal = make_desc_mn_sw128(a_lo + ko, kMnLbo, kMnSbo);
+            const uint64_t dbh = make_desc_mn_sw128(b_hi + ko, kMnLbo, kMnSbo), dbl = make_desc_mn_sw128(b_lo + ko, kMnLbo, kMnSbo);
+            umma_bf16(tacc, dal, dbh, idesc, (l | k) != 0);
+            umma_bf16(tacc, dah, dbl, idesc, 1);
+            umma_bf16(tacc, dah, dbh, idesc, 1);
+          }
+          umma_commit(&empty[s]);
+          if (l == w.nch - 1) umma_commit(&tfull[buf]);
+        }
+        __syncwarp();
+      }
+      if (w.nch == 0 && elect_one()) mbar_arrive(&tfull[buf]);
+      __syncwarp();
     }
   } else {
-    constexpr uint32_t idesc = make_idesc_bf16(WG_BM, NW);
-    for (int g = 0; g < nchunks; ++g) {
-      const int s = g % STAGES;
-      mbar_wait(&full[s], (g / STAGES) & 1);
+    asm volatile("setmaxnreg.dec.sync.aligned.u32 56;");
+    const int q = warp & 3;
+    float* sl = slab + q * 32 * kSlabLd;
+    const int rr = lane >> 3, cc = (lane & 7) * 4;
+    int it = 0;
+    for (int u = blockIdx.x; u < n_units; u += gridDim.x, ++it) {
+      const WgUnit w = wg_unit(jobs, n_jobs, u);
+      const WgradJob& jb = *w.j;
+      const int buf = it & 1;
+      mbar_wait(&tfull[buf], (it >> 1) & 1);
+      mbar_wait(&bfull[buf], (it >> 1) & 1);
       tcgen05_fence_after();
-      if (elect_one()) {
-        const uint32_t a_hi = smem_u32(smem + s * Cfg::stage_bytes);
-        const uint32_t a_lo = a_hi + kWgABytes;
-        const uint32_t b_hi = a_hi + 2 * kWgABytes;
-        const uint32_t b_lo = b_hi + Cfg::b_plane;
-#pragma unroll
-        for (int k = 0; k < WG_BK / 16; ++k) {
-          const uint64_t dah = make_desc_k_sw128(a_hi + k * 32), dal = make_desc_k_sw128(a_lo + k * 32);
-          const uint64_t dbh = make_desc_k_sw128(b_hi + k * 32), dbl = make_desc_k_sw128(b_lo + k * 32);
-          umma_bf16(tmem_base, dal, dbh, idesc, (g | k) != 0);
-          umma_bf16(tmem_base, dah, dbl, idesc, 1);
-          umma_bf16(tmem_base, dah, dbh, idesc, 1);
-        }
-        umma_commit(&empty[s]);
-        if (g == nchunks - 1) umma_commit(tfull);
+      if (w.nch > 0) {
+        const uint32_t taddr = tmem_base + (uint32_t(q * 32) << 16) + uint32_t(buf * 256);
+        const int rbase = w.n0 + q * 32;
+        for (int c = 0; c < w.width; c += 32) {
+          float v[32];
+          tmem_ld32(taddr + c, v);
+          tmem_ld_wait();
+#pragma unroll
+          for (int j = 0; j < 32; j += 4) *reinterpret_cast<float4*>(sl + lane * kSlabLd + j) = make_float4(v[j], v[j + 1], v[j + 2], v[j + 3]);
+          __syncwarp();
+#pragma unroll
+          for (int i = 0; i < 8; ++i) {
+            const int r = ((i + int(blockIdx.x)) & 7) * 4 + rr;
+            const int orow = rbase + r;
+            if (orow < jb.rows_partial) {
+              const float4 x = *reinterpret_cast<const float4*>(sl + r * kSlabLd + cc);
+              red_add_v4(jb.partial + size_t(orow) * jb.ld_partial + w.k0 + c + cc, x.x, x.y, x.z, x.w);
+            }
+          }
+          __syncwarp();
+        }
+        if (w.bias) {
+          float* sb = s_bias + buf * 128 + q * 32 + lane;
+          if (rbase + lane < jb.rows_partial) atomicAdd(&jb.bias_partial[rbase + lane], *sb);
+          *sb = 0.0f;
+        }
       }
+      tcgen05_fence_before();
       __syncwarp();
+      if (lane == 0) mbar_arrive(&tempty[buf]);
     }
-    if (nchunks == 0 && elect_one()) mbar_arrive(tfull);
-    __syncwarp();
   }
+done:
   tcgen05_fence_before();
   __syncthreads();
-  if (warp == kWgProdWarps) tmem_dealloc<256>(tmem_base);
-}
-
-
-constexpr int MN_BK = 32, kMnGroupWarps = kWgProdWarps / 2;
-constexpr uint32_t kMnSbo = 1024, kMnLbo = (MN_BK / 8) * 1024;
-template <int NW> struct WgMnCfg {
-  static constexpr uint32_t a_plane = WG_BM * MN_BK * 2, b_plane = NW * MN_BK * 2;
-  static constexpr uint32_t stage_bytes = 2 * a_plane + 2 * b_plane;
-  static constexpr int stages = 4;
-  static constexpr uint32_t smem_bytes = stages * stage_bytes + 1024 + 256 + 512;
-};
-
-__device__ __forceinline__ uint32_t mn_chunk_offset(uint32_t chunk, uint32_t s) {
-  const uint32_t r = s & 7u;
-  return (chunk >> 3) * kMnLbo + (s >> 3) * kMnSbo + r * 128u + (((chunk & 7u) ^ r) << 4);
-}
-
-template <int NW>
-__device__ __forceinline__ void wg_epilogue_rows(const WgradParams& p, uint32_t tmem_base, float* tile, int warp, int lane, int n0,
-                                                 const float* s_bias) {
-  constexpr int LD = NW + 4;
-  constexpr int SLICE = NW / 4;
-  const int quarter = warp & 3, slice = warp >> 2;
-  {
-    const int row = quarter * 32 + lane;
-    const uint32_t taddr = tmem_base + (uint32_t(quarter * 32) << 16) + uint32_t(slice * SLICE);
-    float* dst = tile + row * LD + slice * SLICE;
-#pragma unroll
-    for (int c = 0; c < SLICE; c += 16) {
-      float v[16];
-      tmem_ld16(taddr + c, v);
-      tmem_ld_wait();
-#pragma unroll
-      for (int j = 0; j < 16; j += 4) *reinterpret_cast<float4*>(dst + c + j) = make_float4(v[j], v[j + 1], v[j + 2], v[j + 3]);
-    }
-  }
-  asm volatile("bar.sync 1, %0;" ::"n"(kWgProdWarps * 32));
-  const int r_first = (int(blockIdx.x) * 5) & 127;
-  for (int i = warp; i < WG_BM; i += kWgProdWarps) {
-    const int r = (i + r_first) & 127;
-    const int orow = n0 + r;
-    if (orow >= p.rows_partial) continue;
-    float* prow = p.partial + size_t(orow) * p.ld_partial + p.k0;
-#pragma unroll
-    for (int c = lane * 4; c < NW; c += 128) {
-      const float4 v = *reinterpret_cast<const float4*>(tile + r * LD + c);
-      red_add_v4(prow + c, v.x, v.y, v.z, v.w);
-    }
-    if (lane == 0 && p.bias_partial && p.k0 == 0) atomicAdd(&p.bias_partial[orow], s_bias[r]);
-  }
-}
-
-template <int NW>
-__global__ void __launch_bounds__(kWgThreads, 1) umma_wgrad_mn_kernel(const WgradParams p) {
-  using Cfg = WgMnCfg<NW>;
-  constexpr int STAGES = Cfg::stages;
-  constexpr int CB = NW / 8;
-  constexpr int SPW = 32 / CB;
-  constexpr int ATASKS = MN_BK / 2;
-  constexpr int TASKS = ATASKS + MN_BK / SPW;
-  constexpr int TPW = TASKS / kMnGroupWarps;
-  static_assert(TASKS % kMnGroupWarps == 0 && TPW >= 2 && STAGES % 2 == 0, "task split");
-  extern __shared__ uint8_t smem_raw[];
-  uint8_t* smem = reinterpret_cast<uint8_t*>((reinterpret_cast<uintptr_t>(smem_raw) + 1023) & ~uintptr_t(1023));
-  uint64_t* bars = reinterpret_cast<uint64_t*>(smem + STAGES * Cfg::stage_bytes);
-  uint64_t* full = bars;
-  uint64_t* empty = bars + STAGES;
-  uint64_t* tfull = bars + 2 * STAGES;
-  uint32_t* tmem_slot = reinterpret_cast<uint32_t*>(bars + 2 * STAGES + 1);
-  float* s_bias = reinterpret_cast<float*>(smem + STAGES * Cfg::stage_bytes + 256);
-
-  const int warp = threadIdx.x >> 5, lane = threadIdx.x & 31;
-  int M = p.m_ptr ? *p.m_ptr : p.m_cap;
-  if (M > p.m_cap) M = p.m_cap;
-  const int P = gridDim.x;
-  const int n0 = p.n0 + int(blockIdx.y) * WG_BM;
-  const int total_chunks = (M + MN_BK - 1) / MN_BK;
-  const int cpp = (total_chunks + P - 1) / P;
-  const int c_begin = min(total_chunks, int(blockIdx.x) * cpp), c_end = min(total_chunks, c_begin + cpp);
-  const int npairs = p.dY2 ? 2 : 1;
-  const int nc1 = c_end - c_begin;
-  const int nchunks = nc1 * npairs;
-
-  if (threadIdx.x == 0) {
-    for (int s = 0; s < STAGES; ++s) { mbar_init(&full[s], kMnGroupWarps); mbar_init(&empty[s], 1); }
-    mbar_init(tfull, 1);
-    fence_mbar_init();
-  }
-  if (threadIdx.x < 128) s_bias[threadIdx.x] = 0.0f;
-  if (warp == kWgProdWarps) tmem_alloc<256>(tmem_slot);
-  tcgen05_fence_before();
-  __syncthreads();
-  tcgen05_fence_after();
-  const uint32_t tmem_base = *tmem_slot;
-
-  if (warp < kWgProdWarps) {
-    float bsum[8] = {0.f, 0.f, 0.f, 0.f, 0.f, 0.f, 0.f, 0.f};
-    const uint32_t a_chunk = lane & 15, a_sub = lane >> 4;
-    const uint32_t b_chunk = lane % CB, b_sub = lane / CB;
-    const int a_col = n0 + int(a_chunk) * 8, b_col = p.k0 + int(b_chunk) * 8;
-    const int group = warp / kMnGroupWarps, wi = warp % kMnGroupWarps;
-    for (int g = group; g < nchunks; g += 2) {
-      const int s = g % STAGES;
-      const int pair = g / nc1;
-      const int chunk = c_begin + g % nc1;
-      const int s0 = chunk * MN_BK;
-      uint8_t* st = smem + s * Cfg::stage_bytes;
-      const float* srcA = pair ? p.dY2 : p.dY;
-      const int ldA = pair ? p.ldy2 : p.ldy;
-      const float* srcB = pair ? p.X2 : p.X;
-      const int ldB = pair ? p.ldx2 : p.ldx;
-      float4 v[TPW][2];
-#pragma unroll
-      for (int i = 0; i < TPW; ++i) {
-        const int t = wi + kMnGroupWarps * i;
-        const bool isA = t < ATASKS;
-        const int sl = isA ? 2 * t + int(a_sub) : (t - ATASKS) * SPW + int(b_sub);
-        const int srow = s0 + sl;
-        const int col = isA ? a_col : b_col;
-        const int lim = isA ? p.n_valid : p.k_valid;
-        const float* rp = (isA ? srcA : srcB) + size_t(srow) * (isA ? ldA : ldB) + col;
-        const bool rok = srow < M;
-        v[i][0] = (rok && col < lim) ? __ldg(reinterpret_cast<const float4*>(rp)) : make_float4(0.f, 0.f, 0.f, 0.f);
-        v[i][1] = (rok && col + 4 < lim) ? __ldg(reinterpret_cast<const float4*>(rp + 4)) : make_float4(0.f, 0.f, 0.f, 0.f);
-      }
-      mbar_wait(&empty[s], ((g / STAGES) & 1) ^ 1);
-#pragma unroll
-      for (int i = 0; i < TPW; ++i) {
-        const int t = wi + kMnGroupWarps * i;
-        const bool isA = t < ATASKS;
-        const int sl = isA ? 2 * t + int(a_sub) : (t - ATASKS) * SPW + int(b_sub);
-        const int col = isA ? a_col : b_col;
-        const int lim = isA ? p.n_valid : p.k_valid;
-        float x[8] = {v[i][0].x, v[i][0].y, v[i][0].z, v[i][0].w, v[i][1].x, v[i][1].y, v[i][1].z, v[i][1].w};
-#pragma unroll
-        for (int j = 0; j < 8; ++j) if (col + j >= lim) x[j] = 0.f;
-        uint32_t hw[4], lw[4];
-#pragma unroll
-        for (int j = 0; j < 4; ++j) wg_split2(x[2 * j], x[2 * j + 1], hw[j], lw[j]);
-        uint8_t* hi = isA ? st : st + 2 * Cfg::a_plane;
-        uint8_t* lo = isA ? st + Cfg::a_plane : st + 2 * Cfg::a_plane + Cfg::b_plane;
-        const uint32_t off = mn_chunk_offset(isA ? a_chunk : b_chunk, uint32_t(sl));
-        *reinterpret_cast<uint4*>(hi + off) = make_uint4(hw[0], hw[1], hw[2], hw[3]);
-        *reinterpret_cast<uint4*>(lo + off) = make_uint4(lw[0], lw[1], lw[2], lw[3]);
-        if (isA && pair == 0) {
-#pragma unroll
-          for (int j = 0; j < 8; ++j) bsum[j] += x[j];
-        }
-      }
-      fence_proxy_async_smem();
-      __syncwarp();
-      if (lane == 0) mbar_arrive(&full[s]);
-    }
-#pragma unroll
-    for (int j = 0; j < 8; ++j) {
-      bsum[j] += __shfl_xor_sync(0xffffffffu, bsum[j], 16);
-      if (lane < 16) atomicAdd(&s_bias[a_chunk * 8 + j], bsum[j]);
-    }
-    asm volatile("bar.sync 1, %0;" ::"n"(kWgProdWarps * 32));
-    mbar_wait(tfull, 0);
-    tcgen05_fence_after();
-    if (nchunks > 0) wg_epilogue_rows<NW>(p, tmem_base, reinterpret_cast<float*>(smem), warp, lane, n0, s_bias);
-  } else {
-    constexpr uint32_t idesc = make_idesc_bf16_mn(WG_BM, NW);
-    for (int g = 0; g < nchunks; ++g) {
-      const int s = g % STAGES;
-      mbar_wait(&full[s], (g / STAGES) & 1);
-      tcgen05_fence_after();
-      if (elect_one()) {
-        const uint32_t a_hi = smem_u32(smem + s * Cfg::stage_bytes);
-        const uint32_t a_lo = a_hi + Cfg::a_plane;
-        const uint32_t b_hi = a_hi + 2 * Cfg::a_plane;
-        const uint32_t b_lo = b_hi + Cfg::b_plane;
-#pragma unroll
-        for (int k = 0; k < MN_BK / 16; ++k) {
-          const uint32_t ko = k * 2 * kMnSbo;
-          const uint64_t dah = make_desc_mn_sw128(a_hi + ko, kMnLbo, kMnSbo), dal = make_desc_mn_sw128(a_lo + ko, kMnLbo, kMnSbo);
-          const uint64_t dbh = make_desc_mn_sw128(b_hi + ko, kMnLbo, kMnSbo), dbl = make_desc_mn_sw128(b_lo + ko, kMnLbo, kMnSbo);
-          umma_bf16(tmem_base, dal, dbh, idesc, (g | k) != 0);
-          umma_bf16(tmem_base, dah, dbl, idesc, 1);
-          umma_bf16(tmem_base, dah, dbh, idesc, 1);
-        }
-        umma_commit(&empty[s]);
-        if (g == nchunks - 1) umma_commit(tfull);
-      }
-      __syncwarp();
-    }
-    if (nchunks == 0 && elect_one()) mbar_arrive(tfull);
-    __syncwarp();
-  }
-  tcgen05_fence_before();
-  __syncthreads();
-  if (warp == kWgProdWarps) tmem_dealloc<256>(tmem_base);
-}
-
-template <int NW>
-static int launch_wgrad_mn(const WgradParams& p, int P, int n_tiles, cudaStream_t stream) {
-  using Cfg = WgMnCfg<NW>;
+  if (warp == kWgMmaWarp) tmem_dealloc<512>(tmem_base);
+}
+
+static int wg_k_tiles(int k_pad) {
+  int n = 0;
+  for (int k0 = 0; k0 < k_pad; ++n) k0 += k_pad - k0 >= 256 ? 256 : k_pad - k0 >= 128 ? 128 : 64;
+  return n;
+}
+
+int wgrad_job(void* rec, const float* dY, int ldy, const float* X, int ldx, const float* dY2, int ldy2, const float* X2, int ldx2,
+              int n_valid, int k_valid, float* partial, int ld_partial, int rows_partial, float* bias_partial, const int* m_ptr,
+              int m_cap, int k_pad, int n_ctas, int* units) {
+  auto al = [](const float* q, int ld) { return (reinterpret_cast<uintptr_t>(q) & 15) == 0 && (ld & 3) == 0; };
+  if (!rec || !dY || !X || !partial || !units || (dY2 == nullptr) != (X2 == nullptr) || n_valid <= 0 || k_valid <= 0 ||
+      k_pad <= 0 || k_pad % 64 || k_pad > ld_partial || (ld_partial & 3) || n_valid > rows_partial || m_cap < 0 || n_ctas <= 0)
+    return NERO_ERR_ARG;
+  if (!al(dY, ldy) || !al(X, ldx) || (dY2 && (!al(dY2, ldy2) || !al(X2, ldx2))) || (reinterpret_cast<uintptr_t>(partial) & 15))
+    return NERO_ERR_ARG;
+  WgradJob j{};
+  j.dY = dY; j.X = X; j.dY2 = dY2; j.X2 = X2;
+  j.partial = partial; j.bias_partial = bias_partial; j.m_ptr = m_ptr;
+  j.ldy = ldy; j.ldx = ldx; j.ldy2 = dY2 ? ldy2 : 0; j.ldx2 = X2 ? ldx2 : 0;
+  j.n_valid = n_valid; j.k_valid = k_valid; j.ld_partial = ld_partial; j.rows_partial = rows_partial; j.m_cap = m_cap;
+  j.n_tiles = (n_valid + WG_BM - 1) / WG_BM;
+  j.k_pad = k_pad;
+  j.n_slices = n_ctas / j.n_tiles > 0 ? n_ctas / j.n_tiles : 1;
+  j.unit0 = *units;
+  *units += wg_k_tiles(k_pad) * j.n_tiles * j.n_slices;
+  memcpy(rec, &j, sizeof(j));
+  return NERO_OK;
+}
+
+int wgrad_group(const void* jobs_dev, int n_jobs, int n_units, int n_ctas, cudaStream_t stream) {
+  if (!jobs_dev || n_jobs <= 0 || n_units < 0 || n_ctas <= 0) return NERO_ERR_ARG;
+  if (n_units == 0) return NERO_OK;
   static bool attr_set = false;
   if (!attr_set) {
-    if (cudaFuncSetAttribute(umma_wgrad_mn_kernel<NW>, cudaFuncAttributeMaxDynamicSharedMemorySize, Cfg::smem_bytes) != cudaSuccess)
+    if (cudaFuncSetAttribute(umma_wgrad_group_kernel, cudaFuncAttributeMaxDynamicSharedMemorySize, kWgSmemBytes) != cudaSuccess)
       return NERO_ERR_CUDA;
     attr_set = true;
   }
-  umma_wgrad_mn_kernel<NW><<<dim3(P, n_tiles), kWgThreads, Cfg::smem_bytes, stream>>>(p);
+  umma_wgrad_group_kernel<<<min(n_ctas, n_units), kWgThreads, kWgSmemBytes, stream>>>(static_cast<const WgradJob*>(jobs_dev), n_jobs,
+                                                                                      n_units);
   NERO_LAUNCH_CHECK();
   return NERO_OK;
 }
 
-template <int NW>
-static int launch_wgrad(const WgradParams& p, int P, int n_tiles, cudaStream_t stream) {
-  using Cfg = WgCfg<NW>;
-  static bool attr_set = false;
-  if (!attr_set) {
-    if (cudaFuncSetAttribute(umma_wgrad_kernel<NW>, cudaFuncAttributeMaxDynamicSharedMemorySize, Cfg::smem_bytes) != cudaSuccess)
-      return NERO_ERR_CUDA;
-    attr_set = true;
-  }
-  umma_wgrad_kernel<NW><<<dim3(P, n_tiles), kWgThreads, Cfg::smem_bytes, stream>>>(p);
-  NERO_LAUNCH_CHECK();
-  return NERO_OK;
-}
-
-int wgrad_dispatch(WgradParams p, int n_rows_pad, int k_pad, int P, cudaStream_t stream) {
-  if ((p.ld_partial & 3) || k_pad % 64 || n_rows_pad % 16 || P <= 0) return NERO_ERR_ARG;
-  const int n_tiles = (n_rows_pad + 127) / 128;
-  p.n0 = 0;
-  auto al = [](const float* q, int ld) { return q == nullptr || ((reinterpret_cast<uintptr_t>(q) & 15) == 0 && (ld & 3) == 0); };
-  const bool mn = al(p.dY, p.ldy) && al(p.X, p.ldx) && al(p.dY2, p.ldy2) && al(p.X2, p.ldx2);
-  int k0 = 0;
-  while (k0 < k_pad) {
-    const int rem = k_pad - k0;
-    p.k0 = k0;
-    int rc;
-    if (rem >= 256) { rc = mn ? launch_wgrad_mn<256>(p, P, n_tiles, stream) : launch_wgrad<256>(p, P, n_tiles, stream); k0 += 256; }
-    else if (rem >= 128) { rc = mn ? launch_wgrad_mn<128>(p, P, n_tiles, stream) : launch_wgrad<128>(p, P, n_tiles, stream); k0 += 128; }
-    else { rc = mn ? launch_wgrad_mn<64>(p, P, n_tiles, stream) : launch_wgrad<64>(p, P, n_tiles, stream); k0 += 64; }
-    if (rc != NERO_OK) return rc;
-  }
-  return NERO_OK;
-}
-
-}
+}
diff --git a/nero_b200/engine.py b/nero_b200/engine.py
--- a/nero_b200/engine.py
+++ b/nero_b200/engine.py
@@ -142,16 +142,21 @@
             wgrad(ws, Mat(dHa), 256, Mat(acts[1]), 256, L[2], *g(2), **kw)
             wgrad(ws, Mat(dHb), 256, Mat(acts[0]), 256, L[1], *g(1), **kw)
             wgrad(ws, Mat(dHc), 256, A, L[0].k_valid, L[0], *g(0), **kw)
+            ws.run()
             return
         linear(dpre, L[3], Mat(dHa), 256, transposed=True, mode=EPI_MUL_DACT, H=Mat(acts[2]), dact=ACT_RELU, **kw)
         wgrad(ws, dpre, self.n_out, Mat(acts[2]), 256, L[3], *g(3), **kw)
+        ws.run()
         linear(Mat(dHa), L[2], Mat(dHb), 256, transposed=True, mode=EPI_MUL_DACT, H=Mat(acts[1]), dact=ACT_RELU, **kw)
         wgrad(ws, Mat(dHa), 256, Mat(acts[1]), 256, L[2], *g(2), **kw)
+        ws.run()
         linear(Mat(dHb), L[1], Mat(dHa), 256, transposed=True, mode=EPI_MUL_DACT, H=Mat(acts[0]), dact=ACT_RELU, **kw)
         wgrad(ws, Mat(dHb), 256, Mat(acts[0]), 256, L[1], *g(1), **kw)
+        ws.run()
         if dX is not None:
             linear(Mat(dHa), L[0], dX, dx_ncol, transposed=True, mode=EPI_MUL_DACT, addend=dx_addend, **kw)
         wgrad(ws, Mat(dHa), 256, A, L[0].k_valid, L[0], *g(0), **kw)
+        ws.run()
 
 
 class SdfNet:
@@ -296,6 +301,7 @@
         ops.colsum(Mat(dY8, Y8_SDF), 1, self.tmp_b, m_ptr=m_ptr, m_cap=m_cap)
         K('nero_wgrad_finish', self.tmp_row, 1, 1, 256, self.tmp_b, 256, 0, 1, None, 1.0, l8.weight_v.detach(), l8.weight_g.detach(),
           l8.weight_v.grad, l8.weight_g.grad, l8.bias.grad, None, 0.0)
+        ws.run()
 
     def value_forward(self, X0, H, out, m_ptr, m_cap):
         Hs = [H[1], H[2], H[3], H[4], H[5], H[6], H[7], H[8]]
@@ -338,6 +344,7 @@
         ops.colsum(Mat(dsdf), 1, self.tmp_b, m_ptr=m_ptr, m_cap=m_cap)
         K('nero_wgrad_finish', self.tmp_row, 1, 1, 256, self.tmp_b, 256, 0, 1, None, 1.0, l8.weight_v.detach(), l8.weight_g.detach(),
           l8.weight_v.grad, l8.weight_g.grad, l8.bias.grad, None, 0.0)
+        ws.run()
 
 
 class NerfNet:
@@ -422,22 +429,31 @@
             wgrad(ws, Mat(G[2]), 256, Mat(N[2]), 256, self.P[2], *gp(pl[2]), **kw)
             wgrad(ws, Mat(G[1]), 256, Mat(N[1]), 256, self.P[1], *gp(pl[1]), **kw)
             wgrad(ws, Mat(G[0]), 256, Mat(w['XN']), self.P[0].k_valid, self.P[0], *gp(pl[0]), **kw)
+            ws.run()
             return
         linear(Mat(dA), self.P[7], Mat(dB), 256, H=Mat(N[7]), **R, **kw)
         wgrad(ws, Mat(dA), 256, Mat(N[7]), 256, self.P[7], *gp(pl[7]), **kw)
+        ws.run()
         linear(Mat(dB), self.P[6], Mat(dA), 256, H=Mat(N[6]), **R, **kw)
         wgrad(ws, Mat(dB), 256, Mat(N[6]), 256, self.P[6], *gp(pl[6]), **kw)
+        ws.run()
         linear(Mat(dA), self.P[5], Mat(dB), 256, H=Mat(w['H5'], 84), **R, **kw)
         wgrad(ws, Mat(dA), 256, Mat(w['H5']), self.P[5].k_valid, self.P[5], *gp(pl[5]), **kw)
+        ws.run()
         linear(Mat(dB), self.P[4], Mat(dA), 256, H=Mat(N[4]), **R, **kw)
         wgrad(ws, Mat(dB), 256, Mat(N[4]), 256, self.P[4], *gp(pl[4]), **kw)
+        ws.run()
         linear(Mat(dA), self.P[3], Mat(dB), 256, H=Mat(N[3]), **R, **kw)
         wgrad(ws, Mat(dA), 256, Mat(N[3]), 256, self.P[3], *gp(pl[3]), **kw)
+        ws.run()
         linear(Mat(dB), self.P[2], Mat(dA), 256, H=Mat(N[2]), **R, **kw)
         wgrad(ws, Mat(dB), 256, Mat(N[2]), 256, self.P[2], *gp(pl[2]), **kw)
+        ws.run()
         linear(Mat(dA), self.P[1], Mat(dB), 256, H=Mat(N[1]), **R, **kw)
         wgrad(ws, Mat(dA), 256, Mat(N[1]), 256, self.P[1], *gp(pl[1]), **kw)
+        ws.run()
         wgrad(ws, Mat(dB), 256, Mat(w['XN']), self.P[0].k_valid, self.P[0], *gp(pl[0]), **kw)
+        ws.run()
 
 
 class ShapeEngine:
diff --git a/nero_b200/ops.py b/nero_b200/ops.py
--- a/nero_b200/ops.py
+++ b/nero_b200/ops.py
@@ -183,13 +183,27 @@
     return _FINISH_JOB
 
 
+_WGRAD_JOB_BYTES = None
+
+
+def _wgrad_job_bytes():
+    global _WGRAD_JOB_BYTES
+    if _WGRAD_JOB_BYTES is None:
+        _WGRAD_JOB_BYTES = lib.nero_abi_sizeof(5)
+        assert _WGRAD_JOB_BYTES > 0
+    return _WGRAD_JOB_BYTES
+
+
 class WgradWorkspace:
 
     def __init__(self, device, P=74, rows=256, ld=384, max_slots=48):
         self.P, self.rows, self.ld = P, rows, ld
+        self.n_ctas = 2 * P
         self.device, self.max_slots = device, max_slots
         self.pool = torch.zeros(max_slots, rows * ld + rows, dtype=torch.float32, device=device)
         self.jobs, self.dest, self.keep = [], set(), []
+        self.gemms, self.gemm_keep = [], []
+        self.units = ctypes.c_int(0)
         self.defer = False
         self._tabs = {}
 
@@ -205,6 +219,15 @@
     @property
     def bias_partial(self):
         return self._slot()[1]
+
+    def _table(self, key, make):
+        hit = self._tabs.get(key)
+        if hit is None:
+            blob, extra = make()
+            if len(self._tabs) >= 64:
+                self._tabs.clear()
+            hit = self._tabs[key] = (torch.frombuffer(bytearray(blob), dtype=torch.uint8).to(self.device), extra)
+        return hit
 
     def enqueue(self, job, dest_key, keep):
         self.jobs.append(job)
@@ -213,22 +236,31 @@
         if len(self.jobs) >= self.max_slots:
             self.flush()
 
+    def run(self):
+        global launch_count
+        if not self.gemms:
+            return
+        blob = b''.join(self.gemms)
+        tab, _ = self._table(('gemm', blob), lambda: (blob, None))
+        rc = lib.nero_wgrad_group(_ptr(tab), len(self.gemms), self.units.value, self.n_ctas, _stream())
+        _check(rc, 'nero_wgrad_group')
+        launch_count += 1
+        self.gemms, self.gemm_keep = [], []
+        self.units.value = 0
+
     def flush(self):
         global launch_count
+        self.run()
         if not self.jobs:
             return
-        key = tuple(self.jobs)
-        hit = self._tabs.get(key)
-        if hit is None:
+
+        def make():
             import numpy as np
             arr = np.zeros(len(self.jobs), dtype=_finish_job_dtype())
             for i, j in enumerate(self.jobs):
                 arr[i] = j
-            if len(self._tabs) >= 64:
-                self._tabs.clear()
-            hit = self._tabs[key] = (torch.from_numpy(arr.view(np.uint8).copy()).to(self.device), int(arr['nrows'].max()),
-                                     int(arr['K'].max()))
-        tab, max_rows, max_k = hit
+            return arr.tobytes(), (int(arr['nrows'].max()), int(arr['K'].max()))
+        tab, (max_rows, max_k) = self._table(('finish', tuple(self.jobs)), make)
         rc = lib.nero_wgrad_finish_batch(_ptr(tab), len(self.jobs), max_rows, max_k, _stream())
         _check(rc, 'nero_wgrad_finish_batch')
         launch_count += 1
@@ -247,24 +279,25 @@
     if ws.defer and grad_w is not None and (grad_w.data_ptr(), layer.row0) in ws.dest:
         ws.flush()
     partial_t, bias_t = ws.partial, ws.bias_partial
-    P = ws.P * 2 // ceil_div(n_rows_pad, 128) if n_rows_pad <= 128 else ws.P
     if not ws.defer:
         partial_t.zero_()
         bias_t.zero_()
-    rc = lib.nero_wgrad(dY.ptr(), dY.ld, n_valid, X.ptr(), X.ld, k_valid,
-                        dY2.ptr() if dY2 else None, dY2.ld if dY2 else 0, X2.ptr() if X2 else None, X2.ld if X2 else 0,
-                        _ptr(partial_t), ws.ld, ws.rows, _ptr(bias_t), n_rows_pad, k_pad, P, _ptr(m_ptr),
-                        m_cap, _stream())
-    _check(rc, 'nero_wgrad')
-    launch_count += ceil_div(n_rows_pad, 128) * max(1, ceil_div(k_pad, 256))
+    rec = ctypes.create_string_buffer(_wgrad_job_bytes())
+    rc = lib.nero_wgrad_job(rec, dY.ptr(), dY.ld, X.ptr(), X.ld, dY2.ptr() if dY2 else None, dY2.ld if dY2 else 0,
+                            X2.ptr() if X2 else None, X2.ld if X2 else 0, n_valid, k_valid, _ptr(partial_t), ws.ld, ws.rows,
+                            _ptr(bias_t), _ptr(m_ptr), m_cap, k_pad, ws.n_ctas, ctypes.byref(ws.units))
+    _check(rc, 'nero_wgrad_job (operands need 16-byte aligned rows and column origins)')
+    ws.gemms.append(rec.raw)
+    ws.gemm_keep.append((dY, X, dY2, X2, m_ptr))
     g = None if layer.g is None else layer.g.detach()
     w_ = layer.weight.detach()
+    ptr = lambda t: 0 if t is None else t.data_ptr()
     if ws.defer:
-        ptr = lambda t: 0 if t is None else t.data_ptr()
         job = (ptr(partial_t), ptr(bias_t) if with_bias else 0, ptr(layer.kmap), ptr(w_), ptr(g), ptr(grad_w), ptr(grad_g),
                ptr(grad_b) if with_bias else 0, 0, 1, ws.rows, ws.ld, layer.K, layer.row0, layer.nrows, 1.0, 0.0)
         ws.enqueue(job, (grad_w.data_ptr(), layer.row0), (w_, g))
         return
+    ws.run()
     rc = lib.nero_wgrad_finish(_ptr(partial_t), 1, ws.rows, ws.ld, _ptr(bias_t) if with_bias else None,
                                layer.K, layer.row0, layer.nrows, _ptr(layer.kmap), ctypes.c_float(1.0),
                                _ptr(w_), _ptr(g), _ptr(grad_w), _ptr(grad_g),
```

Result: slower. 70530, median of 6 (-12.9%).
